# uci-rendering/psdr-cuda

Measured on AMD Instinct MI355X. Metric: Mpath-samples/s renderC+renderD, cbox 512x512 spp=64; grad rel-L2 vs ref, higher is better.
Workload: dtype f32; 1 GPU; cbox 512x512 spp=64/GPU PathTracer(max_depth=3): renderC + configure + renderD + enoki.forward w.r.t. diffuse albedo, through the psdr_cuda surface; triangles=12, global_spp=64, world_size=1, device=AMD Radeon Graphics, local_rank=0

## Files before the change

### __graft_entry__.py

```python
import os
import subprocess
import sys

ROOT = os.path.dirname(os.path.abspath(__file__))
PKG = os.path.join(ROOT, "psdr-cuda_amd")
for p in (PKG, os.path.join(ROOT, "oracle"), os.path.join(ROOT, "tests")):
    if p not in sys.path:
        sys.path.insert(0, p)

HIPCC_FLAGS = ["--offload-arch=gfx950", "-O3", "-std=c++17", "-fPIC", "-munsafe-fp-atomics",
               "-fno-hip-fp32-correctly-rounded-divide-sqrt", "-fgpu-flush-denormals-to-zero", "-fno-slp-vectorize",
               "-freciprocal-math", "-fapprox-func"]
VARIANTS = (0, 1, 2, 3, 4, 6, 8, 10)


def _stale(target, sources):
    return (not os.path.exists(target)) or any(os.path.getmtime(s) > os.path.getmtime(target) for s in sources)


TESTS = os.path.join(ROOT, "tests")
CSRC = os.path.join(PKG, "csrc")
HC_DIR = os.path.join(TESTS, "hostcheck")
HOST_FLAGS = ["-O2", "-std=c++17", "-pthread"]


def _product_and_harness():
    return ([os.path.join(CSRC, f) for f in sorted(os.listdir(CSRC))] + [os.path.join(ROOT, "include", "psdr_hip.h")] +
            [os.path.join(HC_DIR, f) for f in sorted(os.listdir(HC_DIR)) if f.endswith(".h")])


TEST_LIBS = {
    "hostcheck": ("hostcheck/hostcheck.cpp", "hostcheck/libhostcheck.so", _product_and_harness, HOST_FLAGS),
    "path_sedge": ("hostcheck/hostcheck_path_sedge.cpp", "hostcheck/libhostcheck_path_sedge.so", _product_and_harness, HOST_FLAGS),
    "path_guide": ("hostcheck/hostcheck_path_guide.cpp", "hostcheck/libhostcheck_path_guide.so", _product_and_harness, HOST_FLAGS),
    "collocated": ("hostcheck/hostcheck_collocated.cpp", "hostcheck/libhostcheck_collocated.so", _product_and_harness, HOST_FLAGS),
    "pointlight": ("hostcheck/hostcheck_pointlight.cpp", "hostcheck/libhostcheck_pointlight.so", _product_and_harness, HOST_FLAGS),
    "lightstage": ("hostcheck/hostcheck_lightstage.cpp", "hostcheck/libhostcheck_lightstage.so", _product_and_harness, HOST_FLAGS),
    "distantlight": ("hostcheck/hostcheck_distantlight.cpp", "hostcheck/libhostcheck_distantlight.so", _product_and_harness, HOST_FLAGS),
    "plan": ("hostcheck/hostcheck_plan.cpp", "hostcheck/libhostcheck_plan.so", _product_and_harness, HOST_FLAGS),
    "smooth": ("hostcheck/hostcheck_smooth.cpp", "hostcheck/libhostcheck_smooth.so", lambda: [os.path.join(CSRC, "psdr_smooth.h")], HOST_FLAGS),
    "poison": ("poison/poison.hip", "poison/libpoison.so", lambda: [], ["-O1"]),
}


def testlib_deps(name):
    return [os.path.join(TESTS, TEST_LIBS[name][0])] + TEST_LIBS[name][2]()


def build_testlib(name):
    so = os.path.join(TESTS, TEST_LIBS[name][1])
    if _stale(so, testlib_deps(name)):
        subprocess.check_call(["hipcc", "--offload-arch=gfx950", "-fPIC", "-shared"] + TEST_LIBS[name][3] + [os.path.join(TESTS, TEST_LIBS[name][0]), "-o", so])
    return so


def build():
    csrc = os.path.join(PKG, "csrc")
    srcs = [os.path.join(csrc, f) for f in os.listdir(csrc)] + [os.path.join(ROOT, "include", "psdr_hip.h")]
    lib = os.path.join(PKG, "lib", "libpsdr_hip.so")
    os.makedirs(os.path.dirname(lib), exist_ok=True)
    defect_job = None
    if _stale(lib, srcs):
        obj_dir = os.path.join(PKG, "lib", "obj")
        os.makedirs(obj_dir, exist_ok=True)
        jobs, objs, unit_cmds = [], [], {}
        for v in VARIANTS:
            o = os.path.join(obj_dir, "variant%d.o" % v)
            objs.append(o)
            unit_cmds[o] = ["hipcc"] + HIPCC_FLAGS + ["-DPSDR_VARIANT_FLAGS=%d" % v, "-c", os.path.join(csrc, "psdr_variant.hip"), "-o", o]
            jobs.append(subprocess.Popen(unit_cmds[o]))
            o = os.path.join(obj_dir, "path_sedge%d.o" % v)
            objs.append(o)
            unit_cmds[o] = ["hipcc"] + HIPCC_FLAGS + ["-DPSDR_VARIANT_FLAGS=%d" % v, "-c", os.path.join(csrc, "psdr_path_sedge.hip"), "-o", o]
            jobs.append(subprocess.Popen(unit_cmds[o]))
            o = os.path.join(obj_dir, "collocated%d.o" % v)
            objs.append(o)
            unit_cmds[o] = ["hipcc"] + HIPCC_FLAGS + ["-DPSDR_VARIANT_FLAGS=%d" % v, "-c", os.path.join(csrc, "psdr_collocated.hip"), "-o", o]
            jobs.append(subprocess.Popen(unit_cmds[o]))
            o = os.path.join(obj_dir, "pointlight%d.o" % v)
            objs.append(o)
            unit_cmds[o] = ["hipcc"] + HIPCC_FLAGS + ["-DPSDR_VARIANT_FLAGS=%d" % v, "-c", os.path.join(csrc, "psdr_pointlight.hip"), "-o", o]
            jobs.append(subprocess.Popen(unit_cmds[o]))
            o = os.path.join(obj_dir, "lightstage%d.o" % v)
            objs.append(o)
            unit_cmds[o] = ["hipcc"] + HIPCC_FLAGS + ["-DPSDR_VARIANT_FLAGS=%d" % v, "-c", os.path.join(csrc, "psdr_lightstage.hip"), "-o", o]
            jobs.append(subprocess.Popen(unit_cmds[o]))
        o = os.path.join(obj_dir, "logd_lean.o")
        objs.append(o)
        unit_cmds[o] = ["hipcc"] + HIPCC_FLAGS + ["-c", os.path.join(csrc, "psdr_logd_lean.hip"), "-o", o]
        jobs.append(subprocess.Popen(unit_cmds[o]))
        o = os.path.join(obj_dir, "host.o")
        objs.append(o)
        unit_cmds[o] = ["hipcc"] + HIPCC_FLAGS + ["-c", os.path.join(csrc, "psdr_hip.hip"), "-o", o]
        jobs.append(subprocess.Popen(unit_cmds[o]))
        o = os.path.join(obj_dir, "tables.o")
        objs.append(o)
        unit_cmds[o] = ["hipcc"] + HIPCC_FLAGS + ["-c", os.path.join(csrc, "psdr_tables.hip"), "-o", o]
        jobs.append(subprocess.Popen(unit_cmds[o]))
        o = os.path.join(obj_dir, "smooth.o")
        objs.append(o)
        unit_cmds[o] = ["hipcc"] + HIPCC_FLAGS + ["-c", os.path.join(csrc, "psdr_smooth.hip"), "-o", o]
        jobs.append(subprocess.Popen(unit_cmds[o]))
        defect_job = _start_defect_object(csrc, obj_dir)
        if any(j.wait() != 0 for j in jobs):
            raise RuntimeError("hipcc failed")
        sys.path.insert(0, os.path.join(ROOT, "tools"))
        import check_spill_exec
        fallbacks = (["-mllvm", "-amdgpu-opt-exec-mask-pre-ra=0"], ["-mllvm", "-amdgpu-spill-sgpr-to-vgpr=0"])
        from concurrent.futures import ThreadPoolExecutor
        with ThreadPoolExecutor(max_workers=8) as pool:
            first = dict(zip(unit_cmds, pool.map(lambda o_: check_spill_exec.check_library(o_, verbose=True, min_code_objects=1), list(unit_cmds))))
        for o, cmd in list(unit_cmds.items()):
            hits = first[o]
            for extra in fallbacks:
                if not hits:
                    break
                print("build(): %s trips the spill guard -- rebuilding it with %s" % (os.path.basename(o), " ".join(extra)))
                subprocess.check_call(cmd[:1] + cmd[1:-4] + extra + cmd[-4:])
                hits = check_spill_exec.check_library(o, verbose=True, min_code_objects=1)
            if hits:
                raise RuntimeError("%s: %d kernel(s) spill in front of an exec restore with every fallback (tools/check_spill_exec.py)" % (os.path.basename(o), len(hits)))
        subprocess.check_call(["hipcc", "--offload-arch=gfx950", "-shared", "-fPIC"] + objs + ["-o", lib])
        if len(check_spill_exec.code_objects(lib)) < len(objs):
            raise RuntimeError("the linked library holds fewer gfx code objects than translation units: the spill guard cannot see all of it")
    subprocess.check_call(["make", "-C", os.path.join(ROOT, "oracle"), "-s"])
    for name in TEST_LIBS:
        build_testlib(name)
    try:
        build_defect_lib(defect_job)
    except Exception as e:
        print("build(): tests/poison/libpsdr_hip_defect.so not built (%s) -- only tests/test_rough_rev_order_gpu.py uses it" % e)
    import psdr_cuda
    from psdr_cuda import _abi
    _abi.load_hip()
    import oracle
    oracle.load_oracle()


def _defect_object_cmd(csrc, obj_dir):
    return ["hipcc"] + HIPCC_FLAGS + ["-DPSDR_VARIANT_FLAGS=10", "-DPSDR_SINK_REG_PRIV_ROUGH=1", "-DPSDR_DPP_ALWAYS=1", "-c",
                                      os.path.join(csrc, "psdr_variant.hip"), "-o", os.path.join(obj_dir, "variant10_defect.o")]


def _start_defect_object(csrc, obj_dir):
    try:
        return subprocess.Popen(_defect_object_cmd(csrc, obj_dir), stdout=subprocess.DEVNULL, stderr=subprocess.DEVNULL)
    except Exception:
        return None


def build_defect_lib(object_job=None):
    csrc = os.path.join(PKG, "csrc")
    srcs = [os.path.join(csrc, f) for f in os.listdir(csrc)] + [os.path.join(ROOT, "include", "psdr_hip.h")]
    obj_dir = os.path.join(PKG, "lib", "obj")
    defect_lib = os.path.join(ROOT, "tests", "poison", "libpsdr_hip_defect.so")
    objs = [os.path.join(obj_dir, "%s%d.o" % (unit, v)) for v in VARIANTS for unit in ("variant", "path_sedge", "collocated", "pointlight", "lightstage")] + [os.path.join(obj_dir, "logd_lean.o"), os.path.join(obj_dir, "host.o"), os.path.join(obj_dir, "tables.o"), os.path.join(obj_dir, "smooth.o")]
    if not all(os.path.exists(o) for o in objs):
        return None
    if object_job is not None and object_job.wait() != 0:
        object_job = None
    if _stale(defect_lib, srcs + objs):
        defect_obj = os.path.join(obj_dir, "variant10_defect.o")
        if object_job is None:
            subprocess.check_call(_defect_object_cmd(csrc, obj_dir))
        subprocess.check_call(["hipcc", "--offload-arch=gfx950", "-shared", "-fPIC"] + [defect_obj if o.endswith("variant10.o") else o for o in objs] + ["-o", defect_lib])
    return defect_lib


def smoke():
    import numpy as np
    import torch
    assert torch.cuda.is_available(), "smoke() needs a GPU"
    torch.cuda.set_device(0)
    import oracle
    from helpers import GpuScene, load_scene, rel_l2, tangents_wrt
    from psdr_cuda import _abi
    sc, P = load_scene("cbox", res=32, spp=8, sppe=4, sppse=4, translate=(0, (1.0, 0.0, 0.0)))
    tb = sc.tables(0)
    g = GpuScene(tb)
    o = _abi.make_opts(integrator=_abi.INTEGRATOR_PATH, max_depth=3, spp=8)
    img = g.render_c(o)
    ref = oracle.render(tb, o)
    assert np.isfinite(img).all() and rel_l2(img, ref) < 1e-4, rel_l2(img, ref)
    o = _abi.make_opts(spp=8, sppe=4, sppse=4)
    tan = tangents_wrt(tb, P)
    img, dimg = g.render_d_fwd(o, [tan])
    rimg, rd = oracle.render(tb, o, mode=1, tangents=tan)
    assert rel_l2(img, rimg) < 1e-4 and rel_l2(dimg[0], rd) < 1e-3, (rel_l2(img, rimg), rel_l2(dimg[0], rd))
    import psdr_cuda
    from psdr_cuda.fixtures import scene_path
    s2 = psdr_cuda.Scene()
    s2.load_file(scene_path("cbox"), False)
# ... 15 lines not shown
```

### include/psdr_hip.h

```cpp
#ifndef PSDR_HIP_H
#define PSDR_HIP_H

#include <stdint.h>

#ifdef __cplusplus
extern "C" {
#endif

#define PSDR_TRI_STRIDE   24
#define PSDR_TRIUV_STRIDE  8
#define PSDR_SEDGE_STRIDE 16
#define PSDR_PEDGE_STRIDE  8
#define PSDR_BSDF_STRIDE  16
#define PSDR_EMITTER_F_STRIDE 8
#define PSDR_EMITTER_I_STRIDE 4
#define PSDR_CAM_WORDS    64
#define PSDR_ENV_WORDS    32

#define PSDR_TRI_FACE_NORMALS 0x40000000

#define PSDR_BSDF_DIFFUSE        0
#define PSDR_BSDF_ROUGHCONDUCTOR 1
#define PSDR_BSDF_MICROFACET     2
#define PSDR_BSDF_MICROFACET_NORMAL 3
// ... 70 lines not shown
    const int32_t *sec_edge_faces;
    const float   *prim_edge_z;
} psdr_scene_desc;

#define PSDR_FLAG_FUSED     1
#define PSDR_FLAG_WAVEFRONT 2
#define PSDR_FLAG_LITERAL_FORMS 4
#define PSDR_FLAG_KEEP_RECORDS 8
#define PSDR_FLAG_PATH_SEDGES 16
#define PSDR_PATH_SEDGES_MAX_DEPTH 8

typedef struct psdr_render_opts {
    int32_t integrator;
    int32_t bsdf_samples, light_samples;
    int32_t max_depth;
    int32_t hide_emitters;
    int32_t field;
    int32_t spp, sppe, sppse;
    int32_t spp_begin, spp_end;
    int32_t sppe_begin, sppe_end;
    int32_t sppse_begin, sppse_end;
    int32_t flags;
    uint64_t rng_offset[3];
} psdr_render_opts;

typedef struct psdr_tangents {
    const float *d_tri_info;
    const float *d_texels;
    const float *d_emitter_rad;
    const float *d_cam_to_world;
    const float *d_sec_edge;
    const float *d_prim_edge;
    const float *d_env_f;
} psdr_tangents;

typedef struct psdr_grads {
    float *g_tri_info;
    float *g_texels;
    float *g_emitter_rad;
    float *g_cam_to_world;
    float *g_sec_edge;
    float *g_prim_edge;
    float *g_env_f;
} psdr_grads;

typedef struct psdr_scene_s *psdr_scene_t;

const char *psdr_last_error(void);
const char *psdr_version(void);
int psdr_abi_struct_sizes(int32_t out[4]);

int psdr_scene_create(psdr_scene_t *out);
int psdr_scene_destroy(psdr_scene_t h);
int psdr_scene_set_option(psdr_scene_t h, const char *name, double value);

int psdr_scene_set_tables(psdr_scene_t h, const psdr_scene_desc *desc);

int psdr_bvh_build(psdr_scene_t h, void *stream);
int psdr_bvh_stats(psdr_scene_t h, int32_t out[4]);
int psdr_scene_info(psdr_scene_t h, int32_t out[8]);

int psdr_trace(psdr_scene_t h, int32_t m,
               const float *ox, const float *oy, const float *oz,
               const float *dx, const float *dy, const float *dz,
               const float *tmax,
               int32_t *out_shape, int32_t *out_tri, float *out_u, float *out_v,
               void *stream);

int psdr_render_c(psdr_scene_t h, const psdr_render_opts *opts,
                  float *out_img, void *stream);

int psdr_render_d_fwd(psdr_scene_t h, const psdr_render_opts *opts,
                      int32_t K, const psdr_tangents *tangents,
                      float *out_img, float *out_dimg, void *stream);

int psdr_render_d_rev(psdr_scene_t h, const psdr_render_opts *opts,
                      const float *adj_img, float *out_img,
                      const psdr_grads *grads, void *stream);

int psdr_guide_build(psdr_scene_t h, const psdr_render_opts *opts,
                     const int32_t reso[4], int32_t nrounds,
                     float *out_mass, void *stream);

int psdr_scene_set_path_guide(psdr_scene_t h, const int32_t reso[3], const float *cmf, const float *pmf, float sum);
int psdr_scene_set_point_light(psdr_scene_t h, const float pos[3], int32_t K, const float *d_pos, float *g_pos);
int psdr_scene_set_point_lights(psdr_scene_t h, int32_t L, const float *pos, int32_t K, const float *d_pos, float *g_pos);
int psdr_scene_set_light(psdr_scene_t h, int32_t kind, const float v[3], int32_t K, const float *d_v, float *g_v);
int psdr_scene_set_lights(psdr_scene_t h, int32_t L, const int32_t *kinds, const float *v, int32_t K, const float *d_v, float *g_v);
int psdr_path_guide_build(psdr_scene_t h, const psdr_render_opts *opts, int32_t segment,
                          const int32_t reso[4], int32_t nrounds,
                          float *out_mass, void *stream);

int psdr_cube_sample_reuse(int32_t ndim, const int32_t *reso, const float *cmf, const float *pmf, float sum,
                           int32_t n, int32_t m, float *samples, float *out_pdf, void *stream);
int psdr_sample_boundary_segment_direct(const psdr_scene_desc *desc, int32_t m, const float *sample3,
                                        const uint8_t *active, float *out_p0, float *out_edge_dir,
                                        float *out_edge2, float *out_p2, float *out_n, float *out_pdf,
                                        uint8_t *out_valid, int32_t *out_edge, float *out_s1, void *stream);

int psdr_geo_world_vertices_fwd(int32_t V, const float *v_raw, const int32_t *vmesh, const float *mats, float *v_world, void *stream);
int psdr_geo_world_vertices_rev(int32_t V, const float *v_raw, const int32_t *vmesh, const float *mats, const float *v_world, const float *a_world, float *a_raw,
                                void *stream);
int psdr_geo_world_vertices_jvp(int32_t V, const float *v_raw, const int32_t *vmesh, const float *mats, const float *v_world, const float *t_raw, const float *t_mats,
                                float *t_world, void *stream);
int psdr_geo_tri_rows_fwd(int32_t V, int32_t T, const float *v, const int32_t *faces, float *vsum, float *rows, int32_t row_stride, void *stream);
int psdr_geo_tri_rows_rev(int32_t V, int32_t T, const float *v, const int32_t *faces, const float *vsum, const float *a_rows, int32_t row_stride,
                          float *a_vsum , float *a_v, void *stream);
int psdr_geo_tri_rows_jvp(int32_t V, int32_t T, const float *v, const int32_t *faces, const float *vsum, const float *t_v, int32_t row_stride,
                          float *t_vsum , float *t_rows, void *stream);
int psdr_geo_sec_edges_fwd(int32_t E, const int32_t *edges, const float *v, const float *rows, int32_t row_stride, float *info, uint8_t *keep, void *stream);
int psdr_geo_sec_edges_rev(int32_t E, const int32_t *edges, const float *a_info, float *a_v, float *a_rows, int32_t row_stride, void *stream);
int psdr_geo_sec_edges_jvp(int32_t E, const int32_t *edges, const float *t_v, const float *t_rows, int32_t row_stride, float *t_info, void *stream);
int psdr_geo_prim_edges_fwd(int32_t E, const int32_t *edges, const uint8_t *face_normals, const float *v, const float *rows, int32_t row_stride,
                            const float *cam22, float *rows8, float *z4, uint8_t *keep, void *stream);
int psdr_geo_prim_edges_rev(int32_t E, const int32_t *edges, const float *v, const float *cam22, const float *a_rows8, float *a_v, float *a_w2s ,
                            void *stream);
int psdr_geo_prim_edges_jvp(int32_t E, const int32_t *edges, const float *v, const float *cam22, const float *t_v, const float *t_w2s , float *t_rows8,
                            void *stream);

int psdr_geo_compact_edges_fwd(int32_t E, const float *rows, int32_t S, const uint8_t *keep, int32_t w0, int32_t wn, const void *aux, int32_t aux_stride, int32_t A,
                               void *scratch, float *rows_out, void *aux_out, int32_t *pos, float *pmf, float *cmf, float *header, void *stream);
int psdr_geo_compact_edges_rev(int32_t E, int32_t S, const int32_t *pos, const float *a_rows_out, float *a_rows, void *stream);
int psdr_geo_compact_edges_jvp(int32_t E, int32_t S, const int32_t *pos, const float *t_rows, float *t_rows_out, void *stream);
int psdr_geo_emitter_tables(int32_t M, const float *rows, int32_t row_stride, const int32_t *face_offset, const int32_t *mesh_emitter, int32_t Ne, const int32_t *emitter_i,
                            const float *radiance, const float *env_weight, float *mesh_area, float *emitter_f, float *emitter_pmf, float *emitter_cmf, float *face_pmf,
                            float *face_cmf, void *stream);

typedef struct psdr_smooth_s *psdr_smooth_t;
typedef struct psdr_smooth_info_s {
    int32_t iterations;
    int32_t converged;
    int32_t form;
    int32_t launches;
    float rel_residual[3];
    int32_t one_workgroup_limit;
    int32_t one_workgroup_default;
    int32_t num_vertices;
    int32_t num_entries;
    int32_t long_rows;
} psdr_smooth_info_t;
int psdr_smooth_create(int32_t V, int32_t F, const int32_t *faces, psdr_smooth_t *out);
void psdr_smooth_destroy(psdr_smooth_t h);
int psdr_smooth_set_option(psdr_smooth_t h, const char *name, int value);
int psdr_smooth_apply(psdr_smooth_t h, float lambda, const float *x, float *u, void *stream);
int psdr_smooth_solve(psdr_smooth_t h, float lambda, const float *b, const float *x0, float *x, float tol, int32_t max_iter, void *stream);
int psdr_smooth_info(psdr_smooth_t h, psdr_smooth_info_t *out);

int psdr_scene_rev_layout(psdr_scene_t h, int32_t out[16]);

int psdr_scene_seed_info(psdr_scene_t h, int64_t out[4]);

int psdr_scene_logd_info(psdr_scene_t h, int64_t out[4]);

int psdr_get_counters(psdr_scene_t h, uint64_t out[4]);

#ifdef __cplusplus
}
#endif
#endif
```

### psdr-cuda_amd/csrc/psdr_hip.hip

```cpp
#define PSDR_WIDE_TREE 2
#include "psdr_host.h"
#include "psdr_bvh_build.h"

#include <cstdlib>
#include <cstring>
#include <rocprim/rocprim.hpp>

namespace {
__global__ __launch_bounds__(kBlock) void k_trace(LaunchCtx cx, int m, const float *__restrict__ ox, const float *__restrict__ oy,
                                                  const float *__restrict__ oz, const float *__restrict__ dx,
                                                  const float *__restrict__ dy, const float *__restrict__ dz,
                                                  const float *__restrict__ tmax, int32_t *__restrict__ out_shape,
                                                  int32_t *__restrict__ out_tri, float *__restrict__ out_u, float *__restrict__ out_v) {
    TraversalStack st; setup_lds(cx, st);
    const SceneView &sc = cx.sc;
    for (int i = blockIdx.x * kBlock + threadIdx.x; i < m; i += gridDim.x * kBlock) {
        const Hit h = closest_hit<false, -1>(sc, st, Vec3f{ox[i], oy[i], oz[i]}, Vec3f{dx[i], dy[i], dz[i]}, tmax[i]);
        out_tri[i] = h.tri;
        out_shape[i] = h.tri >= 0 ? (sc.d.tri_mesh[h.tri] & ~PSDR_TRI_FACE_NORMALS) : -1;
        out_u[i] = h.u; out_v[i] = h.v;
    }
}


// ... 548 lines not shown
    if (int rc = device_grow(h->d_lbvh, h->lbvh_bytes, need, 1)) return rc;
    const LbvhScratch L = lbvh_layout(h->d_lbvh, T, sort_tmp);
    if (int rc = grow_tree(h, (size_t) T, (size_t) T * 3)) return rc;
    const dim3 gT((T + kBlock - 1) / kBlock), blk(kBlock);
    HIP_TRY(hipMemsetAsync(L.info, 0, sizeof(LbvhInfo), s));
    HIP_TRY(hipMemsetAsync(L.bounds, 0xff, 3 * 4, s));
    HIP_TRY(hipMemsetAsync(L.bounds + 3, 0, 3 * 4, s));
    hipLaunchKernelGGL(k_lbvh_bounds, gT, blk, 0, s, h->desc.tri_info, T, L.bounds, L.info);
    hipLaunchKernelGGL(k_lbvh_codes, gT, blk, 0, s, h->desc.tri_info, T, L.bounds, L.keys, L.vals, L.info);
    HIP_TRY(hipGetLastError());
    size_t tmp_bytes = L.sort_tmp_bytes;
    HIP_TRY(rocprim::radix_sort_pairs(L.sort_tmp, tmp_bytes, L.keys, L.keys2, L.vals, L.vals2, (size_t) T, 0, 30, s));
    HIP_TRY(hipMemsetAsync(L.leaf_parent, 0xff, (size_t) T * 4, s));
    hipLaunchKernelGGL(k_lbvh_tris, gT, blk, 0, s, h->desc.tri_info, T, L.vals2, h->d_btris);
    hipLaunchKernelGGL(k_lbvh_hierarchy, gT, blk, 0, s, L.keys2, T, h->d_nodes, L.node_parent, L.leaf_parent);
    HIP_TRY(hipGetLastError());
    LbvhInfo info{};
    HIP_TRY(hipMemcpyAsync(&info, L.info, sizeof(info), hipMemcpyDeviceToHost, s));
    HIP_TRY(hipStreamSynchronize(s));
    if (info.bad) return fail("psdr_bvh_build: non-finite vertex");
    if (int rc = lbvh_fit(h, L, info.pad, s)) return rc;
    hipLaunchKernelGGL(k_lbvh_depth, gT, blk, 0, s, T, L.node_parent, L.leaf_parent, L.info);
    hipLaunchKernelGGL(k_lbvh_area_keys, gT, blk, 0, s, h->desc.tri_info, T, L.keys, L.vals);
    HIP_TRY(hipGetLastError());
    tmp_bytes = L.sort_tmp_bytes;
    HIP_TRY(rocprim::radix_sort_pairs_desc(L.sort_tmp, tmp_bytes, L.keys, L.keys2, L.vals, L.vals2, (size_t) T, 0, 32, s));
    float area = 0.f;
    const int top = std::min(T, kMaxHotRows);
    std::vector<int32_t> by_area((size_t) top);
    HIP_TRY(hipMemcpyAsync(&info, L.info, sizeof(info), hipMemcpyDeviceToHost, s));
    HIP_TRY(hipMemcpyAsync(&area, h->d_refit_area, sizeof(float), hipMemcpyDeviceToHost, s));
    HIP_TRY(hipMemcpyAsync(by_area.data(), L.vals2, (size_t) top * 4, hipMemcpyDeviceToHost, s));
    if (int rc = fetch_emitters(h, s)) return rc;
    HIP_TRY(hipStreamSynchronize(s));
    if (info.depth > kBvhStack - 2) { fallback = true; return 0; }
    if (int rc = upload_hot_rows(h, T, hot_row_list(T, false, h->emitter_i, h->desc.num_emitters, by_area.data(), top), s)) return rc;
    h->hot_identity = false;
    h->root = 0; h->bvh_depth = info.depth; h->num_nodes = T - 1; h->num_btris = T;
    reset_top(h);
    if (use_wide_tree(h, false)) {
        std::vector<BvhNode> host_nodes((size_t) T - 1);
        HIP_TRY(hipMemcpyAsync(host_nodes.data(), h->d_nodes, host_nodes.size() * sizeof(BvhNode), hipMemcpyDeviceToHost, s));
        HIP_TRY(hipStreamSynchronize(s));
        if (int rc = bvh4_build(h, host_nodes, std::vector<int32_t>{0}, false, s)) return rc;
    } else { h->wide = false; h->num_nodes4 = 0; h->stack_need4 = 0; }
    h->level_start.clear();
    finish_build(h, T, info.pad, area, true, true);
    return 0;
}

int bvh4_refill(psdr_scene_s *h, hipStream_t s) {
    if (h->num_nodes4 <= 0) return 0;
    hipLaunchKernelGGL(k_bvh4_fill, dim3((h->num_nodes4 + kBlock - 1) / kBlock), dim3(kBlock), 0, s, h->d_nodes4, h->d_nodes, h->d_topo4,
                       h->d_topo4 + (size_t) h->num_nodes4 * 4, h->num_nodes4);
    HIP_TRY(hipGetLastError());
    return 0;
}
int bvh4_build(psdr_scene_s *h, const std::vector<BvhNode> &nodes, const std::vector<int32_t> &roots2, bool forest, hipStream_t s) {
    h->wide = use_wide_tree(h, forest);
    if (!h->wide && !forest) { h->num_nodes4 = 0; h->stack_need4 = 0; return 0; }
    Bvh4Topology tp;
    collapse_bvh4(nodes, roots2, tp);
    h->num_nodes4 = tp.n4; h->stack_need4 = tp.stack_need;
    h->root4 = roots2.size() == 1 ? tp.roots[0] : 0;
    for (size_t k = 0; k < roots2.size() && k < (size_t) kMaxBlas; ++k) h->blas_root4[k] = tp.roots[k];
    if (tp.n4 == 0) return 0;
    if (int rc = device_grow(h->d_nodes4, h->cap_nodes4, (size_t) tp.n4, sizeof(Bvh4Node), &h->d_topo4, 8 * sizeof(int32_t))) return rc;
    HIP_TRY(hipMemcpyAsync(h->d_topo4, tp.child.data(), (size_t) tp.n4 * 4 * sizeof(int32_t), hipMemcpyHostToDevice, s));
    HIP_TRY(hipMemcpyAsync(h->d_topo4 + (size_t) tp.n4 * 4, tp.src.data(), (size_t) tp.n4 * 4 * sizeof(int32_t), hipMemcpyHostToDevice, s));
    if (int rc = bvh4_refill(h, s)) return rc;
    HIP_TRY(hipStreamSynchronize(s));
    return 0;
}

int launch_wf_trace(psdr_scene_s *h, const float4 *req, const int32_t *count, long long sub_cap, float4 *hit, hipStream_t s, bool ign) {
    TraceArgs a{};
    a.sec_edge_faces = h->desc.sec_edge_faces;
    if (ign && !a.sec_edge_faces) ign = false;
    pack_blas_boxes(h, a.blas_lo, a.blas_hi);
    a.nodes4 = h->d_nodes4; a.btris = h->d_btris; a.req = req; a.count = count; a.hit = hit; a.sub_cap = sub_cap; a.n_blas = h->n_blas;
    const TracePlan p = plan_wf_trace(h, sub_cap);
    a.n_lnodes = p.n_lnodes; a.off_stack = p.off_stack; a.stack_entries = p.stack_entries; a.ovf_stride = p.ovf_stride;
    if (p.ovf) {
        if (int rc = scratch_reserve(reinterpret_cast<void **>(&h->d_trace_ovf), &h->trace_ovf_bytes, p.ovf_bytes, s, "trace kernel's overflow stack columns")) return rc;
        a.ovf = h->d_trace_ovf;
    }
    const bool wg2 = p.wg2, ovf = p.ovf;
    const int grid = p.grid, dyn = p.dyn;
#define PSDR_LAUNCH_TRACE_I(MULTI, OVF, IGN, WPE)                                                                                                           \
    do { static bool attr_set = false;                                                                                                                      \
         if (!attr_set) { if (int rc = allow_dynamic_lds(&k_wf_trace<MULTI, OVF, IGN, WPE>, 160 * 1024 - 1024)) return rc; attr_set = true; }                     \
         hipLaunchKernelGGL(HIP_KERNEL_NAME(k_wf_trace<MULTI, OVF, IGN, WPE>), dim3(grid), dim3(kTraceBlock), dyn, s, a); } while (0)
#define PSDR_LAUNCH_TRACE(MULTI, OVF) do { if (ign) { if (wg2) PSDR_LAUNCH_TRACE_I(MULTI, OVF, true, 8); else PSDR_LAUNCH_TRACE_I(MULTI, OVF, true, 4); } else if (wg2) PSDR_LAUNCH_TRACE_I(MULTI, OVF, false, 8); else PSDR_LAUNCH_TRACE_I(MULTI, OVF, false, 4); } while (0)
    if (h->n_blas > 1) { if (ovf) PSDR_LAUNCH_TRACE(true, true); else PSDR_LAUNCH_TRACE(true, false); }
    else { if (ovf) PSDR_LAUNCH_TRACE(false, true); else PSDR_LAUNCH_TRACE(false, false); }
#undef PSDR_LAUNCH_TRACE_I
#undef PSDR_LAUNCH_TRACE
    HIP_TRY(hipGetLastError());
    return 0;
}

int probe_buffers(psdr_scene_s *h, long long slots, int rays_per_slot, ProbeBuffers &pb, hipStream_t s, int per_cu) {
    const ProbePlan pl = plan_probe_buffers(h, slots, rays_per_slot, per_cu);
    pb.sub_cap = pl.sub_cap;
    if (int rc = scratch_reserve(&h->d_probe, &h->probe_bytes, pl.total, s, "probe buffers (hit rows, masks, trace requests)")) return rc;
    char *p = reinterpret_cast<char *>(h->d_probe);
    pb.count = reinterpret_cast<int32_t *>(p); p += pl.cnt_bytes;
    pb.hit = reinterpret_cast<float4 *>(p); p += pl.hit_bytes;
    pb.mask = reinterpret_cast<uint32_t *>(p); p += pl.mask_bytes;
    pb.req = reinterpret_cast<float4 *>(p);
    HIP_TRY(hipMemsetAsync(pb.count, 0, pl.cnt_bytes, s));
    return 0;
}

#define PSDR_OPS_OF(OPS)                                                                                                              \
    switch (scene_flag_set(h)) {                                                                                                      \
        case 0: return OPS##0(); case 1: return OPS##1(); case 2: return OPS##2(); case 3: return OPS##3();                          \
        case 4: return OPS##4(); case 8: return OPS##8(); case 10: return OPS##10();                                                 \
        default: return OPS##6();                       \
    }
const VariantOps *variant_of(const psdr_scene_s *h) { PSDR_OPS_OF(variant_ops_) }
const PathSedgeOps *path_sedge_of(const psdr_scene_s *h) { PSDR_OPS_OF(path_sedge_ops_) }
const CollocatedOps *collocated_of(const psdr_scene_s *h) { PSDR_OPS_OF(collocated_ops_) }
const PointLightOps *point_light_of(const psdr_scene_s *h) { PSDR_OPS_OF(point_light_ops_) }
const LightStageOps *light_stage_of(const psdr_scene_s *h) { PSDR_OPS_OF(light_stage_ops_) }
const char *const kDistantInEnv = "a distant light cannot reach a scene inside an environment map's bounding mesh (env_emitter >= 0)";
int check_point_light(const psdr_scene_s *h, const psdr_render_opts *o) {
    if (o->integrator == PSDR_INTEGRATOR_POINT && !h->have_point) return fail("PointLightIntegrator: no light set (psdr_scene_set_point_light)");
    if (o->integrator == PSDR_INTEGRATOR_POINT_STACK && h->stack_pos.empty()) return fail("LightStageIntegrator: no lights set (psdr_scene_set_point_lights)");
    if (h->desc.env_emitter >= 0) {
        const bool distant = o->integrator == PSDR_INTEGRATOR_POINT ? h->point_kind == PSDR_LIGHT_DISTANT
                           : o->integrator == PSDR_INTEGRATOR_POINT_STACK && std::find(h->stack_kind.begin(), h->stack_kind.end(), PSDR_LIGHT_DISTANT) != h->stack_kind.end();
        if (distant) return fail(kDistantInEnv);
    }
    return 0;
}
#undef PSDR_OPS_OF
}
using namespace psdr_host;

extern "C" {

const char *psdr_last_error(void) { return g_err.c_str(); }
const char *psdr_version(void) { return "psdr-hip 0.1 gfx950"; }
int psdr_abi_struct_sizes(int32_t out[4]) {
    out[0] = (int32_t) sizeof(psdr_scene_desc); out[1] = (int32_t) sizeof(psdr_render_opts);
    out[2] = (int32_t) sizeof(psdr_tangents); out[3] = (int32_t) sizeof(psdr_grads);
    return 0;
}

int psdr_scene_create(psdr_scene_t *out) {
    if (!out) return fail("psdr_scene_create: null output");
    psdr_scene_s *h = new psdr_scene_s();
    hipError_t e = hipMalloc(&h->d_counters, sizeof(unsigned long long) * kRayCounters * kRayCounterStride);
    if (e != hipSuccess) { delete h; return fail(std::string("hipMalloc: ") + hipGetErrorString(e)); }
    int dev = 0; hipDeviceProp_t prop;
    if (hipGetDevice(&dev) == hipSuccess && hipGetDeviceProperties(&prop, dev) == hipSuccess) {
        h->num_cus = prop.multiProcessorCount;
        h->lds_limit = (int) std::min<size_t>(prop.sharedMemPerBlock, 160 * 1024);
    }
    *out = h;
    return 0;
}

int psdr_scene_set_option(psdr_scene_t h, const char *name, double value) {
    if (!h || !name) return fail("psdr_scene_set_option: null argument");
    const std::string n(name);
    const int iv = (int) value;
    if (n == "bvh_refit") h->refit_enabled = iv != 0;
    else if (n == "forest_min_inline") { h->forest_min_inline = iv; h->have_bvh = false; }
    else if (n == "scratch_plain") g_scratch_plain = iv;
    else if (n == "own_pixels") h->opt.own_pixels = iv;
    else if (n == "emitter_pretest") h->opt.emitter_pretest = iv;
    else if (n == "occ_rows") { h->opt.occ_rows = iv; h->have_bvh = false; }
    else if (n == "aa_prims") { h->aa_enabled = iv != 0; h->have_bvh = false; }
    else if (n == "tiny_scene") h->tiny_enabled = iv != 0;
    else if (n == "two_level") h->two_level_enabled = iv != 0;
    else if (n == "wf_binned") h->wf_binned = iv != 0;
    else if (n == "wf_traced") h->traced_enabled = iv != 0;
    else if (n == "bvh_build") h->bvh_device_mode = iv;
    else if (n == "sort_edges") h->sort_edges = iv != 0;
    else if (n == "blocks_per_cu") h->opt.blocks_per_cu = iv;
    else if (n == "camera_blocks") h->opt.camera_blocks = iv;
    else if (n == "tiny_variants") h->opt.tiny_variants = iv;
    else if (n == "wide") h->opt.wide = iv;
    else if (n == "lds_budget") h->opt.lds_budget = iv;
    else if (n == "sink_rep") h->opt.sink_rep = std::max(1, std::min(16, iv));
    else if (n == "sink_private") h->opt.sink_private = iv;
    else if (n == "rev_split") h->opt.rev_split = iv;
    else if (n == "tangent_live") h->opt.tangent_live = iv;
    else if (n == "wf_geo") h->opt.wf_geo = iv;
    else if (n == "logd") h->opt.logd = iv;
    else if (n == "seed_cache") h->opt.seed_cache = iv;
    else if (n == "logd_park") h->opt.logd_park = iv;
    else if (n == "seed_cache_log2") h->opt.seed_cache_log2 = std::max(0, std::min(40, iv));
    else if (n == "keep_records") h->opt.keep_records = iv;
    else if (n == "rev_sorted") h->opt.rev_sorted = iv;
    else if (n == "sedge_split") h->opt.sedge_split = iv;
    else if (n == "pt_sedge") h->opt.pt_sedge = iv & 3;
    else if (n == "pt_sedge_walk") h->opt.pt_sedge_walk = iv;
    else if (n == "probe") h->opt.probe = iv;
    else if (n == "trace_wg2") h->opt.trace_wg2 = iv;
    else if (n == "chunk_log2") h->opt.chunk_log2 = std::max(0, std::min(30, iv));
    else if (n == "bvh_maxleaf") h->opt.bvh_maxleaf = std::max(1, std::min(8, iv));
    else if (n == "bvh_tcost") h->opt.bvh_tcost = (float) value;
    else return fail("psdr_scene_set_option: unknown option '" + n + "'");
    h->kept.valid = false;
    if (n == "tiny_scene" || n == "two_level" || n == "bvh_build" || n == "wide" || n == "bvh_maxleaf" || n == "bvh_tcost" || n == "tiny_variants") h->have_bvh = false;
    return 0;
}

int psdr_scene_destroy(psdr_scene_t h) {
    if (!h) return 0;
    if (h->d_nodes) (void) hipFree(h->d_nodes);
    if (h->d_stack_lights) (void) hipFree(h->d_stack_lights);
    if (h->d_btris) (void) hipFree(h->d_btris);
    if (h->d_counters) (void) hipFree(h->d_counters);
    if (h->d_refit_area) (void) hipFree(h->d_refit_area);
    if (h->d_sort) (void) hipFree(h->d_sort);
    if (h->d_ws) (void) hipFree(h->d_ws);
    if (h->d_live) (void) hipFree(h->d_live);
    if (h->d_logd_bad) (void) hipFree(h->d_logd_bad);
    if (h->d_seed) (void) hipFree(h->d_seed);
    if (h->seed_event) (void) hipEventDestroy(h->seed_event);
    if (h->d_hot_map) (void) hipFree(h->d_hot_map);
    if (h->d_hot_tris) (void) hipFree(h->d_hot_tris);
    if (h->d_occ) (void) hipFree(h->d_occ);
    if (h->d_top) (void) hipFree(h->d_top);
    if (h->d_inline_ids) (void) hipFree(h->d_inline_ids);
    if (h->d_lbvh) (void) hipFree(h->d_lbvh);
    if (h->d_nodes4) (void) hipFree(h->d_nodes4);
    if (h->d_topo4) (void) hipFree(h->d_topo4);
    if (h->d_rev) (void) hipFree(h->d_rev);
    if (h->d_se_list) (void) hipFree(h->d_se_list);
    if (h->d_rev_deep) (void) hipFree(h->d_rev_deep);
    if (h->d_pe_rep) (void) hipFree(h->d_pe_rep);
    if (h->d_trace_ovf) (void) hipFree(h->d_trace_ovf);
    if (h->d_probe) (void) hipFree(h->d_probe);
    delete h;
    return 0;
}

int psdr_scene_set_tables(psdr_scene_t h, const psdr_scene_desc *desc) {
    if (!h || !desc) return fail("psdr_scene_set_tables: null argument");
    psdr_scene_desc d = *desc;
    if (d.num_tris <= 0 || !d.tri_info || !d.tri_mesh) return fail("Missing meshes!");
    if (!d.cam) return fail("Missing sensor!");
    if (reinterpret_cast<uintptr_t>(d.tri_info) & 15) return fail("psdr_scene_set_tables: tri_info must be 16-byte aligned");
    if (d.width <= 0 || d.height <= 0) return fail("Invalid film resolution");
    if (d.num_meshes <= 0 || !d.mesh_bsdf || !d.mesh_emitter) return fail("psdr_scene_set_tables: mesh_bsdf / mesh_emitter missing");
    if (d.num_bsdfs > 0 && (!d.bsdf_rec || !d.texels)) return fail("psdr_scene_set_tables: bsdf_rec / texels missing");
    if (d.num_emitters > 0 && (!d.emitter_f || !d.emitter_i)) return fail("psdr_scene_set_tables: emitter tables missing");
    if (d.num_emitters > 1 && (!d.emitter_cmf || !d.emitter_pmf)) return fail("psdr_scene_set_tables: emitter distribution missing");
    if (d.num_sec_edges > 0 && (!d.sec_edge || !d.sec_cmf || !d.sec_pmf)) return fail("psdr_scene_set_tables: secondary-edge tables missing");
    if (d.num_prim_edges > 0 && (!d.prim_edge || !d.prim_cmf || !d.prim_pmf)) return fail("psdr_scene_set_tables: primary-edge tables missing");
    if (d.num_prim_edges <= 0) d.prim_edge_z = nullptr;
    if (d.num_guide_cells > 0 && (!d.guide_cmf || !d.guide_pmf)) return fail("psdr_scene_set_tables: guiding tables missing");
    if (!d.env_f) d.env_emitter = -1;
    if (d.env_emitter >= 0) {
        if (d.env_emitter >= d.num_emitters || !d.env_cmf || !d.env_pmf || d.env_reso[0] <= 0 || d.env_reso[1] <= 0 || d.env_tex[1] < 2 ||
            d.env_tex[2] < 2)
            return fail("psdr_scene_set_tables: inconsistent environment-map record");
    }
    if (h->have_tables && (d.tri_info != h->desc.tri_info || d.num_tris != h->desc.num_tris)) h->have_bvh = false;
    if (h->have_tables && (d.emitter_i != h->desc.emitter_i || d.num_emitters != h->desc.num_emitters)) h->have_bvh = false;
    if (!h->have_tables || std::memcmp(&h->desc, &d, sizeof(d)) != 0) { ++h->tables_gen; h->kept.valid = false; }
    h->desc = d;
    h->has_microfacet = (d.material_mask & ((1u << PSDR_BSDF_MICROFACET) | (1u << PSDR_BSDF_MICROFACET_NORMAL) | (1u << PSDR_BSDF_MICROFACET_HEIGHT))) != 0;
    h->has_rough = d.material_mask == 0 || (d.material_mask & (1u << PSDR_BSDF_ROUGHCONDUCTOR)) != 0 || h->has_microfacet;
    h->have_tables = true;
    h->pg_cmf = h->pg_pmf = nullptr; h->pg_sum = 0.f;
    return 0;
}

int psdr_scene_set_path_guide(psdr_scene_t h, const int32_t reso[3], const float *cmf, const float *pmf, float sum) {
    if (!h) return fail("psdr_scene_set_path_guide: null argument");
    if (!cmf) { h->pg_cmf = h->pg_pmf = nullptr; h->pg_sum = 0.f; return 0; }
    if (!reso || !pmf) return fail("psdr_scene_set_path_guide: null argument");
    if (reso[0] <= 0 || reso[1] <= 0 || reso[2] <= 0 || (long long) reso[0] * reso[1] * reso[2] > 0x7fffffffLL) return fail("psdr_scene_set_path_guide: invalid resolution");
    for (int i = 0; i < 3; ++i) h->pg_reso[i] = reso[i];
    h->pg_cmf = cmf; h->pg_pmf = pmf; h->pg_sum = sum;
    return 0;
}

static hipError_t copy_on_stream(void *dst, const void *src, size_t bytes, hipMemcpyKind kind, hipStream_t s) {
    if (hipError_t e = hipMemcpyAsync(dst, src, bytes, kind, s)) return e;
    return hipStreamSynchronize(s);
}
static void update_emit_rows(psdr_scene_s *h) {
    h->emit_rows = 0;
    if (h->n_tiny > 0 && emit_rows_wanted(h))
        h->emit_rows = tiny_emitter_rows(h->tiny_meta, h->n_tiny, h->aa_cnt, emitter_triangle_mask(h->emitter_i, h->desc.num_emitters, h->desc.num_tris));
}

static void refit_done(psdr_scene_s *h) { h->refits_since_build++; h->num_refits++; h->have_bvh = true; }
static int emitters_unchanged(psdr_scene_s *h, hipStream_t s, bool &same) {
    same = (size_t) std::max(h->desc.num_emitters, 0) * PSDR_EMITTER_I_STRIDE == h->emitter_i.size();
    if (!same || h->emitter_i.empty()) return 0;
    same = h->desc.emitter_i != nullptr;
    if (!same) return 0;
    std::vector<int32_t> now(h->emitter_i.size());
    HIP_TRY(copy_on_stream(now.data(), h->desc.emitter_i, now.size() * sizeof(int32_t), hipMemcpyDeviceToHost, s));
    same = std::memcmp(now.data(), h->emitter_i.data(), now.size() * sizeof(int32_t)) == 0;
    return 0;
}
static int host_tree_refit(psdr_scene_s *h, hipStream_t s, bool &fits) {
    fits = true;
    HIP_TRY(hipMemsetAsync(h->d_refit_area, 0, sizeof(float), s));
    hipLaunchKernelGGL(k_refit_leaves, dim3((h->num_btris + kBlock - 1) / kBlock), dim3(kBlock), 0, s, h->d_btris, h->desc.tri_info, h->num_btris);
    for (int l = (int) h->level_start.size() - 2; l >= 0; --l) {
        const int first = h->level_start[l], count = h->level_start[l + 1] - first;
        hipLaunchKernelGGL(k_refit_level, dim3((count + kBlock - 1) / kBlock), dim3(kBlock), 0, s, h->d_nodes, h->d_btris, first, count, h->bvh_pad, h->d_refit_area);
    }
    HIP_TRY(hipGetLastError());
    if (int rc = bvh4_refill(h, s)) return rc;
    if (h->n_blas == 0) return 0;
    float4 top[kMaxInlineTris * 3 + 2 * kMaxBlas];
    hipLaunchKernelGGL(k_gather_top, dim3(1), dim3(64), 0, s, h->d_top, h->d_nodes, h->desc.tri_info, h->d_inline_ids, h->n_inline, h->n_blas);
    HIP_TRY(hipMemcpyAsync(top, h->d_top, sizeof(top), hipMemcpyDeviceToHost, s));
    HIP_TRY(hipStreamSynchronize(s));
    std::vector<float4> tris(top, top + 3 * (size_t) h->n_inline), prims;
    pack_tiny_prims(tris, prims);
    fits = refit_inline_fits((int) prims.size() / 3);
    if (!fits) return 0;
    h->n_tiny = tiny_plane_form(prims, h->tiny, h->tiny_meta, &h->aa_cnt, h->aa_enabled);
    update_emit_rows(h);
    for (int k = 0; k < h->n_blas; ++k) {
        const float w = h->blas_lo[k].w;
        h->blas_lo[k] = top[kMaxInlineTris * 3 + k]; h->blas_lo[k].w = w;
        h->blas_hi[k] = top[kMaxInlineTris * 3 + kMaxBlas + k];
    }
    return 0;
}
static int try_refit(psdr_scene_s *h, int T, bool tiny, hipStream_t s, bool &done) {
    done = false;
    if (!refit_candidate(h, T, tiny)) return 0;
    bool emitters_same = false;
    if (int rc = emitters_unchanged(h, s, emitters_same)) return rc;
    const bool stands = forest_stands(h);
    if (refit_choice(h, emitters_same, stands, h->built_area) == kRefitNone) return 0;
    float prev_area = h->built_area;
    if (h->refits_since_build > 0) {
        HIP_TRY(hipMemcpyAsync(&prev_area, h->d_refit_area, sizeof(float), hipMemcpyDeviceToHost, h->refit_stream));
        HIP_TRY(hipStreamSynchronize(h->refit_stream));
    }
    const RefitKind kind = refit_choice(h, emitters_same, stands, prev_area);
// ... 229 lines not shown
    if (pos == nullptr || L == 0) return 0;
    if (int rc = device_grow(h->d_stack_lights, h->cap_stack_lights, (size_t) L, sizeof(float) * 13)) return rc;
    h->stack_pos.assign(pos, pos + 3 * (size_t) L);
    h->stack_kind.assign((size_t) L, PSDR_LIGHT_POINT);
    if (d_pos != nullptr && K > 0) { h->stack_K = K; h->stack_dpos.assign(d_pos, d_pos + 3 * (size_t) L * K); }
    h->stack_gpos = g_pos;
    return 0;
}

static int check_light_vector(const char *fn, int kind, const float *v, const std::string &which) {
    if (kind != PSDR_LIGHT_POINT && kind != PSDR_LIGHT_DISTANT) return fail(std::string(fn) + ": unknown light kind " + std::to_string(kind) + which + " (PSDR_LIGHT_POINT or PSDR_LIGHT_DISTANT)");
    if (kind != PSDR_LIGHT_DISTANT || v == nullptr) return 0;
    if (!(std::isfinite(v[0]) && std::isfinite(v[1]) && std::isfinite(v[2]))) return fail(std::string(fn) + ": the direction" + which + " is not finite");
    if (v[0] == 0.f && v[1] == 0.f && v[2] == 0.f) return fail(std::string(fn) + ": the direction" + which + " is all zero");
    return 0;
}

int psdr_scene_set_light(psdr_scene_t h, int32_t kind, const float v[3], int32_t K, const float *d_v, float *g_v) {
    if (!h) return fail("psdr_scene_set_light: null handle");
    if (int rc = check_light_vector("psdr_scene_set_light", kind, v, "")) return rc;
    if (int rc = psdr_scene_set_point_light(h, v, K, d_v, g_v)) return rc;
    if (v != nullptr) h->point_kind = kind;
    return 0;
}

int psdr_scene_set_lights(psdr_scene_t h, int32_t L, const int32_t *kinds, const float *v, int32_t K, const float *d_v, float *g_v) {
    if (!h) return fail("psdr_scene_set_lights: null handle");
    const bool some = v != nullptr && L != 0;
    if (some && kinds == nullptr) return fail("psdr_scene_set_lights: null kinds");
    if (some && L >= 1 && L <= PSDR_POINT_LIGHTS_MAX)
        for (int l = 0; l < L; ++l)
            if (int rc = check_light_vector("psdr_scene_set_lights", kinds[l], v + 3 * l, " of light " + std::to_string(l))) return rc;
    if (int rc = psdr_scene_set_point_lights(h, L, v, K, d_v, g_v)) return rc;
    if (some) h->stack_kind.assign(kinds, kinds + L);
    return 0;
}

int psdr_guide_build(psdr_scene_t h, const psdr_render_opts *o, const int32_t reso[4], int32_t nrounds, float *out_mass, void *stream) {
    if (!h || !o || !reso || !out_mass) return fail("psdr_guide_build: null argument");
    if (int rc = check_microfacet(h, o)) return rc;
    if (nrounds <= 0) return fail("psdr_guide_build: nrounds must be positive");
    if (h->desc.num_sec_edges <= 0) return fail("psdr_guide_build: scene has no secondary edges");
    hipStream_t s = (hipStream_t) stream;
    if (int rc = begin_call(h, s)) return rc;
    LaunchCtx cx;
    if (int rc = make_ctx(h, o, 2, cx)) return rc;
    cx.sc.d.guide_cmf = nullptr; cx.sc.d.num_guide_cells = 0;
    const long long cells = (long long) reso[0] * reso[1] * reso[2];
    const long long n = cells * reso[3];
    if (n <= 0 || n > 0x7fffffffLL) return fail("psdr_guide_build: invalid resolution");
    HIP_TRY(hipMemsetAsync(out_mass, 0, sizeof(float) * cells, s));
    return variant_of(h)->guide(h, cx, reso, nrounds, n, out_mass, s);
}

int psdr_path_guide_build(psdr_scene_t h, const psdr_render_opts *o, int32_t segment, const int32_t reso[4], int32_t nrounds, float *out_mass, void *stream) {
    if (!h || !o || !reso || !out_mass) return fail("psdr_path_guide_build: null argument");
    if (int rc = check_microfacet(h, o)) return rc;
    if (nrounds <= 0) return fail("psdr_path_guide_build: nrounds must be positive");
    if (o->integrator != PSDR_INTEGRATOR_PATH) return fail("psdr_path_guide_build: the integrator must be PSDR_INTEGRATOR_PATH");
    if (o->max_depth < 1) return fail("psdr_path_guide_build: max_depth must be at least 1");
    if (o->max_depth > PSDR_PATH_SEDGES_MAX_DEPTH) return fail("psdr_path_guide_build: PathTracer max_depth > 8 is not supported for the secondary-edge term");
    if (segment != 1 && segment != 2) return fail("psdr_path_guide_build: segment must be 1 (direct source) or 2 (indirect source)");
    if (segment == 2 && o->max_depth < 2) return fail("psdr_path_guide_build: segment 2 needs max_depth >= 2");
    if (!h->have_tables) return fail("Scene not loaded yet!");
    if (h->desc.num_sec_edges <= 0) return fail("psdr_path_guide_build: scene has no secondary edges");
    if (reso[0] <= 0 || reso[1] <= 0 || reso[2] <= 0 || reso[3] <= 0) return fail("psdr_path_guide_build: invalid resolution");
    const long long cells = (long long) reso[0] * reso[1] * reso[2];
    if (cells > 0x7fffffffLL || cells * reso[3] > 0x7fffffffLL || cells * reso[3] * (long long) nrounds > 0x7fffffffLL)
        return fail("psdr_path_guide_build: more than 2^31 (stream, round) slots");
    hipStream_t s = (hipStream_t) stream;
    if (int rc = begin_call(h, s)) return rc;
    HIP_TRY(hipMemsetAsync(out_mass, 0, sizeof(float) * cells, s));
    return path_sedge_of(h)->guide(h, o, segment, reso, nrounds, out_mass, s);
}

int psdr_cube_sample_reuse(int32_t ndim, const int32_t *reso, const float *cmf, const float *pmf, float sum, int32_t n, int32_t m, float *samples,
                           float *out_pdf, void *stream) {
    if (!reso || !cmf || !pmf || !samples || !out_pdf) return fail("psdr_cube_sample_reuse: null argument");
    if (ndim != 2 && ndim != 3) return fail("psdr_cube_sample_reuse: ndim must be 2 or 3");
    long long cells = 1;
    for (int d = 0; d < ndim; ++d) {
        if (reso[d] <= 0) return fail("psdr_cube_sample_reuse: invalid resolution");
        cells *= reso[d];
    }
    if (cells != (long long) n) return fail("psdr_cube_sample_reuse: n must be the product of the resolution");
    if (m < 0) return fail("psdr_cube_sample_reuse: negative sample count");
    if (m == 0) return 0;
    const dim3 grid((unsigned) ((m + kBlock - 1) / kBlock));
    hipStream_t s = (hipStream_t) stream;
    if (ndim == 2)
        hipLaunchKernelGGL(k_cube_sample_reuse<2>, grid, dim3(kBlock), 0, s, m, cmf, pmf, sum, n, reso[0], reso[1], 1, samples, out_pdf);
    else
        hipLaunchKernelGGL(k_cube_sample_reuse<3>, grid, dim3(kBlock), 0, s, m, cmf, pmf, sum, n, reso[0], reso[1], reso[2], samples, out_pdf);
    HIP_TRY(hipGetLastError());
    return 0;
}

int psdr_sample_boundary_segment_direct(const psdr_scene_desc *desc, int32_t m, const float *sample3, const uint8_t *active, float *out_p0,
                                        float *out_edge_dir, float *out_edge2, float *out_p2, float *out_n, float *out_pdf, uint8_t *out_valid,
                                        int32_t *out_edge, float *out_s1, void *stream) {
    if (!desc || !sample3 || !out_p0 || !out_edge_dir || !out_edge2 || !out_p2 || !out_n || !out_pdf || !out_valid || !out_edge || !out_s1)
        return fail("psdr_sample_boundary_segment_direct: null argument");
    const psdr_scene_desc &d = *desc;
    if (d.num_sec_edges <= 0 || !d.sec_edge || !d.sec_cmf || !d.sec_pmf) return fail("Scene has no secondary edges");
    if (d.num_emitters <= 0 || !d.emitter_f || !d.emitter_i) return fail("No Emitter!");
    if (d.num_emitters > 1 && (!d.emitter_cmf || !d.emitter_pmf)) return fail("psdr_sample_boundary_segment_direct: emitter distribution missing");
    const bool env = d.env_f != nullptr && d.env_emitter >= 0;
    if (env && (d.env_emitter >= d.num_emitters || !d.env_cmf || !d.env_pmf || d.env_reso[0] <= 0 || d.env_reso[1] <= 0))
        return fail("psdr_sample_boundary_segment_direct: inconsistent environment-map record");
    if (d.num_emitters > (env ? 1 : 0) && (d.num_tris <= 0 || !d.tri_info || !d.face_cmf || !d.face_pmf))
        return fail("psdr_sample_boundary_segment_direct: area-light tables missing");
    if (m < 0) return fail("psdr_sample_boundary_segment_direct: negative sample count");
    if (m == 0) return 0;
    SceneView sc{};
    sc.d = d;
    if (!env) sc.d.env_emitter = -1;
    const dim3 grid((unsigned) ((m + kBlock - 1) / kBlock));
    hipStream_t s = (hipStream_t) stream;
    if (env)
        hipLaunchKernelGGL(k_boundary_segment_direct<kSceneEnv>, grid, dim3(kBlock), 0, s, sc, m, sample3, active, out_p0, out_edge_dir, out_edge2, out_p2, out_n,
                           out_pdf, out_valid, out_edge, out_s1);
    else
        hipLaunchKernelGGL(k_boundary_segment_direct<0>, grid, dim3(kBlock), 0, s, sc, m, sample3, active, out_p0, out_edge_dir, out_edge2, out_p2, out_n,
                           out_pdf, out_valid, out_edge, out_s1);
    HIP_TRY(hipGetLastError());
    return 0;
}

int psdr_bvh_stats(psdr_scene_t h, int32_t out[4]) {
    if (!h || !out) return fail("psdr_bvh_stats: null argument");
    out[0] = h->num_builds; out[1] = h->num_refits; out[2] = h->num_nodes; out[3] = h->bvh_depth;
    return 0;
}

int psdr_scene_info(psdr_scene_t h, int32_t out[8]) {
    if (!h || !out) return fail("psdr_scene_info: null argument");
    const int n_slab = (h->aa_cnt & 255) + ((h->aa_cnt >> 8) & 255) + (h->aa_cnt >> 16);
    out[0] = h->n_tiny - (h->aa_cnt != 0 ? kAaSlots - n_slab : 0); out[1] = h->n_blas; out[2] = h->n_inline; out[3] = h->num_btris; out[4] = h->lbvh ? 1 : 0;
    out[5] = n_slab; out[6] = h->have_occ ? 1 : 0; out[7] = h->have_occ ? h->occ_max_rows : 0;
    return 0;
}

int psdr_scene_rev_layout(psdr_scene_t h, int32_t out[16]) {
    if (!h || !out) return fail("psdr_scene_rev_layout: null argument");
    std::copy(std::begin(h->rev_layout), std::end(h->rev_layout), out);
    return 0;
}

int psdr_scene_logd_info(psdr_scene_t h, int64_t out[4]) {
    if (!h || !out) return fail("psdr_scene_logd_info: null argument");
    out[0] = h->logd_launches; out[1] = h->logd_lean_launches; out[2] = h->logd_lean_seeded; out[3] = (int64_t) h->logd_lean_lds + h->logd_lean_park;
    return 0;
}
int psdr_scene_seed_info(psdr_scene_t h, int64_t out[4]) {
    if (!h || !out) return fail("psdr_scene_seed_info: null argument");
    out[0] = h->seed_valid ? h->seed_key[0] * h->seed_key[3] : 0; out[1] = (int64_t) (h->seed_cap * sizeof(ulonglong2)); out[2] = h->seed_fills; out[3] = h->seed_launches;
    return 0;
}

int psdr_get_counters(psdr_scene_t h, uint64_t out[4]) {
    if (!h || !out) return fail("psdr_get_counters: null argument");
    unsigned long long all[kRayCounters * kRayCounterStride], c[1] = {0};
    HIP_TRY(hipMemcpyAsync(all, h->d_counters, sizeof(all), hipMemcpyDeviceToHost, h->last_stream));
    HIP_TRY(hipStreamSynchronize(h->last_stream));
    for (int i = 0; i < kRayCounters; ++i) c[0] += all[i * kRayCounterStride];
#ifdef PSDR_STAGE_CLOCKS
    {
        unsigned long long ph[12] = {0};
        for (int i = 0; i < kRayCounters; ++i) for (int k = 0; k < 12; ++k) ph[k] += all[i * kRayCounterStride + 1 + k];
        std::fprintf(stderr, "stage clocks:");
        for (int k = 0; k < 12; ++k) std::fprintf(stderr, " %llu", ph[k]);
        std::fprintf(stderr, "\n");
    }
#endif
    out[0] = c[0]; out[1] = h->slots[0]; out[2] = h->slots[1]; out[3] = h->slots[2];
    return 0;
}

}
```

### psdr-cuda_amd/csrc/psdr_host.h

```cpp
#pragma once
#include "psdr_device.h"
#include "psdr_reverse.h"

#include <algorithm>
#include <type_traits>
#include <cmath>
#include <cstdio>
#include <cstdlib>
#include <cstring>
#include <string>
#include <vector>

using namespace psdr;

struct LaunchCtx {
    SceneView sc;
    LiParams lp;
    RngJump jump;
    int32_t off_stack;
    int32_t off_pathrec;
    int32_t off_sink;
    int32_t off_park;
};

static_assert(offsetof(LaunchCtx, sc) == 0, "closest_hit reads SceneView::tiny through the kernel-argument segment pointer: LaunchCtx (SceneView first) must be the first kernel argument");

__device__ __forceinline__ void setup_lds(const LaunchCtx &cx, TraversalStack &st) {
#if defined(__HIP_DEVICE_COMPILE__)
    const SceneView &sc = cx.sc;
    float4 *dst = reinterpret_cast<float4 *>(psdr_dyn_lds);
    const float4 *src = sc.nodes4 != nullptr ? reinterpret_cast<const float4 *>(sc.nodes4) : reinterpret_cast<const float4 *>(sc.nodes);
    for (int i = threadIdx.x; i < sc.n_lnodes * 4; i += kBlock) dst[sc.off_lnodes / 16 + (i >> 2) * (kLdsNodeStride / 16) + (i & 3)] = src[i];
    for (int i = threadIdx.x; i < sc.n_lbtris * 3; i += kBlock) dst[sc.off_lbtris / 16 + i] = sc.btris[i];
    src = reinterpret_cast<const float4 *>(sc.d.tri_info);
    for (int i = threadIdx.x; i < sc.n_ltri * 6; i += kBlock) dst[sc.off_ltri / 16 + i] = src[i];
    {
        float *m = reinterpret_cast<float *>(psdr_dyn_lds + sc.off_lprim);
#pragma unroll 1
        for (int i = 0; i < sc.n_tiny; ++i) {
            int32_t tri; float k[6];
            const int w = threadIdx.x & 7;
            const float4 Sm = sc.tiny[i * 4 + 2];
            const float S[4] = {Sm.x, Sm.y, Sm.z, Sm.w};
            tiny_hit_row(sc.tiny_meta + i * 4, (threadIdx.x >> 3) & 1, tri, k, (sc.aa_cnt != 0 && i < kAaSlots) ? S : nullptr);
            const float val = w == 0 ? __int_as_float(tri) : (w == 1 ? k[0] : w == 2 ? k[1] : w == 3 ? k[2] : w == 4 ? k[3] : w == 5 ? k[4] : w == 6 ? k[5] : 0.f);
            if (threadIdx.x < kTinyHitWords) m[i * kTinyHitWords + threadIdx.x] = val;
        }
    }
    if (sc.lt_meshbsdf >= 0) {
        auto stage = [&](int off, const void *table, int words) {
            if (off < 0 || table == nullptr) return;
            const uint32_t *g = static_cast<const uint32_t *>(table);
            uint32_t *l = reinterpret_cast<uint32_t *>(psdr_dyn_lds + off);
#pragma unroll 1
            for (int i = threadIdx.x; i < words; i += kBlock) l[i] = g[i];
        };
        stage(sc.lt_trimesh, sc.d.tri_mesh, sc.d.num_tris);
        stage(sc.lt_meshbsdf, sc.d.mesh_bsdf, sc.d.num_meshes);
        stage(sc.lt_meshemitter, sc.d.mesh_emitter, sc.d.num_meshes);
        stage(sc.lt_bsdf, sc.d.bsdf_rec, sc.d.num_bsdfs * PSDR_BSDF_STRIDE);
        stage(sc.lt_emf, sc.d.emitter_f, sc.d.num_emitters * PSDR_EMITTER_F_STRIDE);
        stage(sc.lt_emi, sc.d.emitter_i, sc.d.num_emitters * PSDR_EMITTER_I_STRIDE);
        stage(sc.lt_ecmf, sc.d.emitter_cmf, sc.d.num_emitters);
        stage(sc.lt_epmf, sc.d.emitter_pmf, sc.d.num_emitters);
        stage(sc.lt_fcmf, sc.d.face_cmf, sc.lt_nfaces);
        stage(sc.lt_fpmf, sc.d.face_pmf, sc.lt_nfaces);
        stage(sc.lt_uv, sc.d.tri_uv, sc.d.num_tris * PSDR_TRIUV_STRIDE);
        stage(sc.lt_tex, sc.d.texels, sc.d.num_texels);
        stage(sc.lt_occ, sc.occ, sc.d.num_tris * sc.d.num_tris);
    }
    st.base = reinterpret_cast<int32_t *>(psdr_dyn_lds + cx.off_stack) + threadIdx.x;
    __syncthreads();
#else
    (void) cx; (void) st;
#endif
}
template <class TVT> __device__ __forceinline__ void setup_lds(const LaunchCtx &cx, TraversalStack &st, const TVT &tv) {
    setup_lds(cx, st);
#if defined(__HIP_DEVICE_COMPILE__)
    if constexpr (Tab<TVT::flags>::lds_small && TVT::k > 0) {
        constexpr int K = TVT::k;
        static_assert(K <= 3, "plan_lds reserves three tangent texel pools");
        if (cx.sc.lt_tex >= 0) {
            float *l = reinterpret_cast<float *>(psdr_dyn_lds + cx.sc.lt_tex);
            const int nt = cx.sc.d.num_texels;
            for (int k = 0; k < K; ++k) {
                const float *g = tv.t[k].d_texels;
                for (int i = threadIdx.x; i < nt; i += kBlock) l[(k + 1) * nt + i] = g ? g[i] : 0.f;
            }
            __syncthreads();
        }
    }
#endif
}

constexpr int kSinkCacheWords = 6144;
struct SinkLayout {
    int tex_off, tex_n;
    int rad_off, rad_n;
    int cam_off;
    int env_off, env_n;
    int hot_off, hot_rows;
    const int32_t *hot_map, *hot_tris;
    int total;
    int rep, stride;
    int priv_off, priv_rows;
    int priv_tri[2], priv_slot[2], priv_emitter;
    int priv_regs;
    int pend_off, pend_rows;
};
constexpr int kPendWords = 10;
constexpr int kPrivRowWords = 13;
constexpr int kPrivWords = 2 * kPrivRowWords + 3;

struct psdr_scene_options {
    int blocks_per_cu = 0;
    int camera_blocks = 0;
    int tiny_variants = 1;
    int wide = -1;
    int lds_budget = 0;
    int sink_rep = 4;
    int sink_private = 1;
    int rev_split = -1;
    int tangent_live = 1;
    int wf_geo = 1;
    int own_pixels = 1;
    int emitter_pretest = 1;
    int occ_rows = 1;
    int logd = 1;
    int keep_records = 1;
    int rev_sorted = 1;
    int pt_sedge = 3;
    int pt_sedge_walk = 1;
    int sedge_split = -1;
    int chunk_log2 = 0;
    int probe = 1;
    int trace_wg2 = -1;
    int seed_cache = 1;
    int seed_cache_log2 = 25;
    int logd_park = 1;
    int bvh_maxleaf = 4;
    float bvh_tcost = 2.0f;
};

struct psdr_scene_s {
    psdr_scene_options opt;
    psdr_scene_desc desc{};
    bool have_tables = false;
    bool has_rough = true;
    int num_cus = 256;
    int lds_limit = 64 * 1024;

    BvhNode *d_nodes = nullptr;
    float4 *d_btris = nullptr;
    size_t cap_nodes = 0, cap_btris = 0;
    int32_t root = 0;
    bool have_bvh = false;
    int bvh_depth = 0, num_nodes = 0, num_btris = 0;
    Bvh4Node *d_nodes4 = nullptr;
    int32_t *d_topo4 = nullptr;
    size_t cap_nodes4 = 0;
    int num_nodes4 = 0, stack_need4 = 0;
    bool wide = false;
    int32_t *d_trace_ovf = nullptr;
    size_t trace_ovf_bytes = 0;
    bool traced_enabled = true;
    int32_t root4 = 0, blas_root4[kMaxBlas] = {};
    bool refit_enabled = true;
    int tree_tris = -1, refits_since_build = 0, num_builds = 0, num_refits = 0;
    std::vector<int> level_start;
    float bvh_pad = 0.f, built_area = 0.f;
    float *d_refit_area = nullptr;

    int bvh_device_mode = -1;
    bool lbvh = false;
    int lbvh_leaves = 0;
    void *d_lbvh = nullptr;
    size_t lbvh_bytes = 0;

    bool tiny_enabled = true, aa_enabled = true;
    int n_tiny = 0, aa_cnt = 0;
    float4 tiny[kTinyRows * 4] = {};
    int32_t tiny_meta[kTinyRows * 4] = {};
    bool two_level_enabled = true, refit_ok = true, wf_binned = true;
    int n_blas = 0, n_inline = 0;
    float4 blas_lo[kMaxBlas] = {}, blas_hi[kMaxBlas] = {};
    float4 *d_top = nullptr;
    int32_t *d_inline_ids = nullptr;

    unsigned long long *d_counters = nullptr;
    hipStream_t last_stream = nullptr;
    hipStream_t refit_stream = nullptr;
    uint64_t slots[3] = {0, 0, 0};
    int last_path_depth = 0;
    int32_t rev_layout[16] = {};

    std::vector<int32_t> emitter_i;
    int32_t *d_hot_map = nullptr, *d_hot_tris = nullptr;
    uint32_t *d_occ = nullptr; size_t occ_cap = 0; bool have_occ = false; int occ_max_rows = 0;
    int hot_rows = 0;
    bool hot_identity = false;
    size_t hot_cap = 0;

    bool sort_edges = true;
    void *d_sort = nullptr;
    size_t sort_bytes = 0;

    void *d_pe_rep = nullptr;
    size_t pe_rep_bytes = 0;

    void *d_rev_deep = nullptr;
    size_t rev_deep_bytes = 0;

    void *d_se_list = nullptr;
    size_t se_list_bytes = 0;

    void *d_rev = nullptr;
    size_t rev_bytes = 0;
    void *d_logd_bad = nullptr; size_t logd_bad_bytes = 0;
    struct KeptRecords { bool valid = false; psdr_render_opts o{}; uint64_t gen = 0; long long n = 0; int kind = 0; } kept;
    uint64_t tables_gen = 0;

    void *d_seed = nullptr;
    size_t seed_cap = 0;
    long long seed_key[4] = {0, 0, 0, 0};
    bool seed_valid = false;
    hipStream_t seed_stream = nullptr;
    hipEvent_t seed_event = nullptr;
    long long seed_fills = 0, seed_launches = 0;
    long long logd_launches = 0, logd_lean_launches = 0, logd_lean_seeded = 0;
    int logd_lean_lds = 0, logd_lean_park = 0;
    void *d_ws = nullptr;
    size_t ws_bytes = 0;
    void *d_live = nullptr;
    size_t live_bytes = 0;
    void *d_probe = nullptr;
    size_t probe_bytes = 0;
    uint32_t emit_rows = 0;
    int forest_min_inline = 0;
    int32_t pg_reso[3] = {1, 1, 1};
    const float *pg_cmf = nullptr, *pg_pmf = nullptr;
    float pg_sum = 0.f;
    bool has_microfacet = false;
    bool have_point = false;
    float point_pos[3] = {0.f, 0.f, 0.f}, point_dpos[3][3] = {};
    int point_K = 0;
    float *point_gpos = nullptr;
    int point_kind = PSDR_LIGHT_POINT;
    std::vector<float> stack_pos, stack_dpos;
    int stack_K = 0;
    float *stack_gpos = nullptr;
    std::vector<int32_t> stack_kind;
    float *d_stack_lights = nullptr;
    size_t cap_stack_lights = 0;
};

constexpr int kRayCounters = 64, kRayCounterStride = 16;
constexpr int kWfSub = 64, kWfCountStride = 32;
constexpr int kTraceBlock = 1024, kTraceNodeStride = 80, kTraceStackMax = 16;

#define HIP_TRY(expr)                                                                              \
    do { hipError_t e_ = (expr); if (e_ != hipSuccess) return psdr_host::fail(std::string(#expr) + ": " + hipGetErrorString(e_)); } while (0)
namespace psdr_host {
int fail(const std::string &m);
template <class Kernel> int allow_dynamic_lds(Kernel *kernel, int bytes) {
    if (bytes > 48 * 1024) HIP_TRY(hipFuncSetAttribute(reinterpret_cast<const void *>(kernel), hipFuncAttributeMaxDynamicSharedMemorySize, bytes));
    return 0;
}
int scratch_reserve(void **buf, size_t *have, size_t need, hipStream_t s, const char *what);
long long fit_chunk(long long chunk, size_t bytes_per_slot, size_t fixed_bytes, size_t have);
inline int workspace_reserve(psdr_scene_s *h, size_t need, hipStream_t s) { return scratch_reserve(&h->d_ws, &h->ws_bytes, need, s, "wavefront workspace (path-state streams + trace requests)"); }
void fill_top(const psdr_scene_s *h, SceneView &sc);
constexpr int kMaxInlineTris = 2 * kTinyTris;
int make_ctx(psdr_scene_s *h, const psdr_render_opts *o, int sampler, LaunchCtx &cx);
int launch_wf_trace(psdr_scene_s *h, const float4 *req, const int32_t *count, long long sub_cap, float4 *hit, hipStream_t s, bool ign = false);
struct ProbeBuffers { float4 *hit; uint32_t *mask; float4 *req; int32_t *count; long long sub_cap; };
int probe_buffers(psdr_scene_s *h, long long slots, int rays_per_slot, ProbeBuffers &pb, hipStream_t s, int per_cu = 16);
inline int sink_bytes_base(const SinkLayout &L) { return (L.priv_rows > 0 && !L.priv_regs) ? (L.priv_off + kPrivWords * kBlock) * 4 : (L.rep * L.stride * 4 + 15) / 16 * 16; }
inline int sink_bytes(const SinkLayout &L) { return L.pend_rows > 0 ? (L.pend_off + L.pend_rows * kPendWords * kBlock) * 4 : sink_bytes_base(L); }
inline void sink_reserve_pending(SinkLayout &L, int rows) { L.pend_rows = 0; L.pend_off = (sink_bytes_base(L) / 4 + 3) / 4 * 4; L.pend_rows = rows; }
int check_counts(const psdr_scene_s *h, const psdr_render_opts *o);
int check_microfacet(const psdr_scene_s *h, const psdr_render_opts *o);
int begin_call(psdr_scene_s *h, hipStream_t s);
int primary_edge_order(psdr_scene_s *h, const LaunchCtx &cx, long long i0, long long n, const uint32_t **order, hipStream_t s);
constexpr int kMaxRefits = 64;
constexpr float kRefitAreaGrowth = 1.3f;
constexpr int kLbvhAutoTris = 1 << 18;

struct VariantOps {
    int (*render_c)(psdr_scene_s *h, const psdr_render_opts *o, float *img, hipStream_t s);
    int (*render_fwd)(psdr_scene_s *h, const psdr_render_opts *o, int K, const psdr_tangents *tangents, float *img, float *dimg, hipStream_t s);
    int (*render_rev)(psdr_scene_s *h, const psdr_render_opts *o, const float *adj_img, float *out_img, const psdr_grads *grads, hipStream_t s);
    int (*guide)(psdr_scene_s *h, LaunchCtx &cx, const int32_t reso[4], int nrounds, long long n, float *out_mass, hipStream_t s);
};
struct PathSedgeOps {
    int (*fwd)(psdr_scene_s *h, const psdr_render_opts *o, int K, const psdr_tangents *tangents, float *dimg, hipStream_t s);
    int (*rev)(psdr_scene_s *h, const psdr_render_opts *o, const float *adj_img, const psdr_grads *grads, hipStream_t s);
    int (*guide)(psdr_scene_s *h, const psdr_render_opts *o, int segment, const int32_t reso[4], int nrounds, float *out_mass, hipStream_t s);
};
const PathSedgeOps *path_sedge_ops_0();
const PathSedgeOps *path_sedge_ops_1();
const PathSedgeOps *path_sedge_ops_2();
const PathSedgeOps *path_sedge_ops_3();
const PathSedgeOps *path_sedge_ops_4();
const PathSedgeOps *path_sedge_ops_6();
const PathSedgeOps *path_sedge_ops_8();
const PathSedgeOps *path_sedge_ops_10();
struct CollocatedOps {
    int (*render_c)(psdr_scene_s *h, const psdr_render_opts *o, float *img, hipStream_t s);
    int (*render_fwd)(psdr_scene_s *h, const psdr_render_opts *o, int K, const psdr_tangents *tangents, float *img, float *dimg, hipStream_t s);
    int (*render_rev)(psdr_scene_s *h, const psdr_render_opts *o, const float *adj_img, float *out_img, const psdr_grads *grads, hipStream_t s);
};
const CollocatedOps *collocated_ops_0();
const CollocatedOps *collocated_ops_1();
const CollocatedOps *collocated_ops_2();
const CollocatedOps *collocated_ops_3();
const CollocatedOps *collocated_ops_4();
const CollocatedOps *collocated_ops_6();
const CollocatedOps *collocated_ops_8();
const CollocatedOps *collocated_ops_10();
struct PointLightOps {
    int (*render_c)(psdr_scene_s *h, const psdr_render_opts *o, float *img, hipStream_t s);
    int (*render_fwd)(psdr_scene_s *h, const psdr_render_opts *o, int K, const psdr_tangents *tangents, float *img, float *dimg, hipStream_t s);
    int (*render_rev)(psdr_scene_s *h, const psdr_render_opts *o, const float *adj_img, float *out_img, const psdr_grads *grads, hipStream_t s);
    int (*edges_fwd)(psdr_scene_s *h, const psdr_render_opts *o, int K, const psdr_tangents *tangents, int kind, const float *pos, const float *d_pos, float *dimg, long long plane, hipStream_t s);
    int (*edges_rev)(psdr_scene_s *h, const psdr_render_opts *o, const float *adj_img, const psdr_grads *grads, int kind, const float *pos, float *g_pos, hipStream_t s);
};
const PointLightOps *point_light_ops_0();
const PointLightOps *point_light_ops_1();
const PointLightOps *point_light_ops_2();
const PointLightOps *point_light_ops_3();
const PointLightOps *point_light_ops_4();
const PointLightOps *point_light_ops_6();
const PointLightOps *point_light_ops_8();
const PointLightOps *point_light_ops_10();
struct LightStageOps {
    int (*render_c)(psdr_scene_s *h, const psdr_render_opts *o, float *img, hipStream_t s);
    int (*render_fwd)(psdr_scene_s *h, const psdr_render_opts *o, int K, const psdr_tangents *tangents, float *img, float *dimg, const PointLightOps *point, hipStream_t s);
    int (*render_rev)(psdr_scene_s *h, const psdr_render_opts *o, const float *adj_img, float *out_img, const psdr_grads *grads, const PointLightOps *point, hipStream_t s);
};
const LightStageOps *light_stage_ops_0();
const LightStageOps *light_stage_ops_1();
const LightStageOps *light_stage_ops_2();
const LightStageOps *light_stage_ops_3();
const LightStageOps *light_stage_ops_4();
const LightStageOps *light_stage_ops_6();
const LightStageOps *light_stage_ops_8();
const LightStageOps *light_stage_ops_10();
int logd_lean_launch_8(psdr_scene_s *h, const psdr_render_opts *o, const LaunchCtx &cx, const psdr::TangentView<1, psdr::kSceneTiny> &tv, float *img, float *dimg, hipStream_t s, bool *ran);
const VariantOps *variant_ops_0();
const VariantOps *variant_ops_1();
const VariantOps *variant_ops_2();
const VariantOps *variant_ops_3();
const VariantOps *variant_ops_4();
const VariantOps *variant_ops_6();
const VariantOps *variant_ops_8();
const VariantOps *variant_ops_10();
}

#include "psdr_plan.h"
#include "psdr_tree_plan.h"
```

### psdr-cuda_amd/csrc/psdr_kernels.h

```cpp
#pragma once
#include "psdr_host.h"

namespace {
using namespace psdr_host;

__device__ __forceinline__ float wave_shfl_down(float v, int off) { return __shfl_down(v, off, 64); }

template <int CTRL, int ROW_MASK> __device__ __forceinline__ float dpp_add(float v) {
    return v + __int_as_float(__builtin_amdgcn_update_dpp(0, __float_as_int(v), CTRL, ROW_MASK, 0xf, true));
}
__device__ __forceinline__ float wave_total(float v) {
    v = dpp_add<0x111, 0xf>(v); v = dpp_add<0x112, 0xf>(v); v = dpp_add<0x114, 0xf>(v); v = dpp_add<0x118, 0xf>(v);
    v = dpp_add<0x142, 0xa>(v); v = dpp_add<0x143, 0xc>(v);
    return __int_as_float(__builtin_amdgcn_readlane(__float_as_int(v), 63));
}
#ifndef PSDR_DPP_ALWAYS
#define PSDR_DPP_ALWAYS 0
#endif
template <int N, bool DPP = (N <= 6 || PSDR_DPP_ALWAYS)> __device__ __forceinline__ bool wave_segmented_sum(int key, float (&v)[N]) {
    const int lane = threadIdx.x & 63;
    if (DPP && __ballot(key != __builtin_amdgcn_readfirstlane(key)) == 0ull) {
#pragma unroll
        for (int i = 0; i < N; ++i) v[i] = wave_total(v[i]);
        return lane == 0;
    }
#pragma unroll
    for (int off = 1; off < 64; off <<= 1) {
        const int okey = __shfl_down(key, off, 64);
        const bool take = (lane + off < 64) && (okey == key);
#pragma unroll
        for (int i = 0; i < N; ++i) {
            const float o = wave_shfl_down(v[i], off);
            if (take) v[i] += o;
        }
    }
    const int pkey = __shfl_up(key, 1, 64);
    return lane == 0 || pkey != key;
}

template <int N, bool DPP = (N <= 6 || PSDR_DPP_ALWAYS)> __device__ __forceinline__ bool wave_run_sum(int key, float (&v)[N]) {
    const int lane = threadIdx.x & 63;
    const int prev = __shfl_up(key, 1, 64);
    const bool head = lane == 0 || prev != key;
    const unsigned long long heads = __ballot(head);
    const int seg = __popcll(heads & (~0ull >> (63 - lane)));
    wave_segmented_sum<N, DPP>(seg, v);
    return head;
}

__device__ __forceinline__ float *dyn_lds_floats(int byte_offset) {
#if defined(__HIP_DEVICE_COMPILE__)
    return reinterpret_cast<float *>(psdr_dyn_lds + byte_offset);
#else
    (void) byte_offset; return nullptr;
#endif
}
__device__ __forceinline__ void count_rays(unsigned long long *counters, uint32_t nrays) {
    uint32_t s = nrays;
#pragma unroll
    for (int off = 32; off > 0; off >>= 1) s += __shfl_down(s, off, 64);
    if ((threadIdx.x & 63) == 0 && s) atomicAdd(counters + (blockIdx.x % kRayCounters) * kRayCounterStride, (unsigned long long) s);
}

struct ProbeView { const float4 *hit; const uint32_t *mask; };
template <int NR>
__device__ __forceinline__ void probe_load(TraversalStack &st, const ProbeView &pv, long long slot, uint32_t m) {
#pragma unroll
    for (int r = 0; r < NR; ++r) {
        st.pre[r].tri = -1;
        if ((m >> r) & 1u) { const float4 h = pv.hit[slot * NR + r]; st.pre[r] = Hit{__float_as_int(h.x), h.y, h.z, h.w}; }
    }
}

struct SlotDiv {
    uint32_t d, m; int sh;
    SlotDiv() = default;
    SlotDiv(int nsp) : d((uint32_t) nsp) {
        int l = 0;
        while ((1u << l) < d) ++l;
        m = (uint32_t) ((1ull << (31 + l)) / d + 1ull); sh = 31 + l;
    }
};
PSDR_HD void slot_to_pixel(long long j, const SlotDiv &nsp, int &pixel, int &s) {
    const uint32_t ju = (uint32_t) j, q = (uint32_t) (((uint64_t) ju * nsp.m) >> nsp.sh);
    pixel = (int) q; s = (int) (ju - q * nsp.d);
}
#ifndef PSDR_WAVES_C
#define PSDR_WAVES_C 4
#endif
#ifndef PSDR_WAVES_DM
#define PSDR_WAVES_DM 3
#endif
#ifndef PSDR_WAVES_C_NOTREE
#define PSDR_WAVES_C_NOTREE 6
#endif
#ifndef PSDR_WAVES_DG
#define PSDR_WAVES_DG 2
#endif
#ifndef PSDR_LOGD
#define PSDR_LOGD 1
#endif
#ifndef PSDR_LOGD_WAVES_K1
#define PSDR_LOGD_WAVES_K1 6
#endif
template <class G, class R, int INTEG, int FL, bool NOTREE = false> constexpr int camera_waves() {
    constexpr bool lean = (FL & (kSceneEnv | kSceneRough)) == 0;
    if (!is_ad<R>()) return lean ? ((NOTREE && INTEG == PSDR_INTEGRATOR_PATH) ? PSDR_WAVES_C_NOTREE : PSDR_WAVES_C + 1) : PSDR_WAVES_C;
    constexpr bool rough_path_notree = NOTREE && (FL & kSceneRough) != 0 && INTEG == PSDR_INTEGRATOR_PATH;
    if (is_ad<G>()) return ad_traits<G>::K == 1 ? (rough_path_notree ? 2 : 3) : PSDR_WAVES_DG;
    if (rough_path_notree && ad_traits<R>::K == 3) return 2;
    if (lean && NOTREE && INTEG == PSDR_INTEGRATOR_PATH) return ad_traits<R>::K == 1 ? PSDR_WAVES_DM + 2 : PSDR_WAVES_DM + 1;
    return (lean && INTEG == PSDR_INTEGRATOR_PATH && ad_traits<R>::K == 1) ? PSDR_WAVES_DM + 1 : PSDR_WAVES_DM;
}
constexpr int kLogdGateWord = kRayCounterStride - 1;
template <class G, class R, int INTEG, int FL> constexpr bool logd_instance() {
    return PSDR_LOGD && !is_ad<G>() && is_ad<R>() && INTEG == PSDR_INTEGRATOR_PATH && (FL & (kSceneRough | kSceneEnv | kScenePre)) == 0;
}
__global__ __launch_bounds__(kBlock) void k_seed_fill(ulonglong2 *__restrict__ seed, long long n, int spp, int s_begin, SlotDiv nsp) {
    const long long j = (long long) blockIdx.x * kBlock + threadIdx.x;
    if (j >= n) return;
    int pixel, s_in;
    slot_to_pixel(j, nsp, pixel, s_in);
    Rng rng; rng.seed((uint64_t) pixel * (uint64_t) spp + (uint64_t) (s_begin + s_in));
    seed[j] = ulonglong2{rng.state, rng.inc};
}
__device__ __forceinline__ Rng seeded_rng(const ulonglong2 &sd, const RngJump &jump) { Rng rng; rng.init_seeded(sd.x, sd.y, jump); return rng; }
#define PSDR_CAMERA_KERNEL_BODY(SEED_LOAD, SAMPLE) \
    constexpr int K = ad_traits<R>::K; \
    constexpr int NV = 3 * (1 + K); \
    if constexpr (logd_instance<G, R, INTEG, FL>()) { if (counters[kLogdGateWord] == 1ull) return; } \
    TraversalStack st; setup_lds(cx, st, tv); \
    uint32_t nrays = 0; \
    const long long nceil = (n + kBlock - 1) / kBlock * kBlock; \
    for (long long j = (long long) blockIdx.x * kBlock + threadIdx.x; j < nceil; j += (long long) gridDim.x * kBlock) { \
        const bool in = j < n; \
        SEED_LOAD \
        int pixel = 0x7fffffff, s_in = 0; \
        if (in) slot_to_pixel(j0 + j, nsp, pixel, s_in); \
        float v[NV]; \
_Pragma("unroll") \
        for (int i = 0; i < NV; ++i) v[i] = 0.f; \
        if constexpr ((FL & kScenePre) != 0) { if (in) probe_load<3>(st, pv, j, pv.mask[j]); } \
        if (in) { \
            const int s = s_begin + s_in; \
            const uint64_t slot = (uint64_t) pixel * (uint64_t) spp + (uint64_t) s; \
            const Vec3<R> r = SAMPLE; \
            v[0] = val(r.x) * inv_spp; v[1] = val(r.y) * inv_spp; v[2] = val(r.z) * inv_spp; \
_Pragma("unroll") \
            for (int k = 0; k < K; ++k) { \
                v[3 + 3 * k] = tangent(r.x, k) * inv_spp; v[4 + 3 * k] = tangent(r.y, k) * inv_spp; v[5 + 3 * k] = tangent(r.z, k) * inv_spp; \
            } \
        } \
        const bool head = wave_segmented_sum<NV>(pixel, v); \
        if (head && in) { \
            float *p = img + (size_t) pixel * 3; \
            if (own) { \
                p[0] = v[0]; p[1] = v[1]; p[2] = v[2]; \
_Pragma("unroll") \
                for (int k = 0; k < K; ++k) { float *q = dimg + (size_t) k * plane + (size_t) pixel * 3; q[0] = v[3 + 3 * k]; q[1] = v[4 + 3 * k]; q[2] = v[5 + 3 * k]; } \
            } else { \
                if (v[0] != 0.f) atomicAdd(p, v[0]); \
                if (v[1] != 0.f) atomicAdd(p + 1, v[1]); \
                if (v[2] != 0.f) atomicAdd(p + 2, v[2]); \
_Pragma("unroll") \
                for (int k = 0; k < K; ++k) { \
                    float *q = dimg + (size_t) k * plane + (size_t) pixel * 3; \
                    if (v[3 + 3 * k] != 0.f) atomicAdd(q, v[3 + 3 * k]); \
                    if (v[4 + 3 * k] != 0.f) atomicAdd(q + 1, v[4 + 3 * k]); \
                    if (v[5 + 3 * k] != 0.f) atomicAdd(q + 2, v[5 + 3 * k]); \
                } \
            } \
        } \
    } \
    count_rays(counters, nrays);
#define PSDR_SEED_LOAD_NONE
#define PSDR_SEED_LOAD const ulonglong2 sd = in ? seed[j] : ulonglong2{0ull, 0ull};
template <class G, class R, int INTEG, int FL, bool NOTREE = false>
__global__ __launch_bounds__(kBlock, (camera_waves<G, R, INTEG, FL, NOTREE>())) void k_camera(LaunchCtx cx, TV<R, FL> tv, int spp, int s_begin, SlotDiv nsp, long long n, float inv_spp,
                                                   float *__restrict__ img, float *__restrict__ dimg, long long plane,
                                                   unsigned long long *counters, long long j0, ProbeView pv, int own) {
    PSDR_CAMERA_KERNEL_BODY(PSDR_SEED_LOAD_NONE, (camera_sample<G, R, INTEG>(cx.sc, tv, st, cx.lp, cx.jump, pixel, slot, nrays)))
}
template <class G, class R, int INTEG, int FL, bool NOTREE = false>
__global__ __launch_bounds__(kBlock, (camera_waves<G, R, INTEG, FL, NOTREE>())) void k_camera_seeded(LaunchCtx cx, TV<R, FL> tv, int spp, int s_begin, SlotDiv nsp, long long n, float inv_spp,
                                                   float *__restrict__ img, float *__restrict__ dimg, long long plane,
                                                   unsigned long long *counters, int own, const ulonglong2 *__restrict__ seed) {
    static_assert((FL & kScenePre) == 0, "seeded launches have no probe rows");
    constexpr long long j0 = 0;
    const ProbeView pv{nullptr, nullptr};
    PSDR_CAMERA_KERNEL_BODY(PSDR_SEED_LOAD, (((void) slot), camera_sample<G, R, INTEG>(cx.sc, tv, st, cx.lp, seeded_rng(sd, cx.jump), pixel, nrays)))
}
#undef PSDR_CAMERA_KERNEL_BODY
#undef PSDR_SEED_LOAD
#undef PSDR_SEED_LOAD_NONE

template <int K>
__global__ __launch_bounds__(kBlock) void k_logd_check(const float *__restrict__ texels, TangentView<K, 0> tv, int n, unsigned long long *counters, int *bad) {
    const int i = blockIdx.x * kBlock + threadIdx.x;
    bool b = false;
    if (i < n) {
        bool moved = false;
#pragma unroll
        for (int k = 0; k < K; ++k) moved = moved || tv.t[k].d_texels[i] != 0.f;
        b = moved && !(fabsf(texels[i]) > 1e-20f);
    }
    if (__ballot(b) != 0ull && (threadIdx.x & 63) == 0) atomicOr(bad, 1);
}
__global__ void k_logd_gate(unsigned long long *counters, const int *bad) { if (threadIdx.x == 0 && blockIdx.x == 0) counters[kLogdGateWord] = *bad ? 0ull : 1ull; }
template <int K, int FL, bool NOTREE>
__global__ __launch_bounds__(kBlock, ((PSDR_LOGD_WAVES_K1 > 0 && K == 1 && NOTREE) ? PSDR_LOGD_WAVES_K1 : camera_waves<float, Dual<K>, PSDR_INTEGRATOR_PATH, FL, NOTREE>())) void k_camera_logd(LaunchCtx cx, TV<Dual<K>, FL> tv, int spp, int s_begin, SlotDiv nsp,
                                                   long long n, float inv_spp, float *__restrict__ img, float *__restrict__ dimg, long long plane, unsigned long long *counters, int own) {
    constexpr int NV = 3 * (1 + K);
    if (counters[kLogdGateWord] != 1ull) return;
    TraversalStack st; setup_lds(cx, st, tv);
    uint32_t nrays = 0;
    const long long nceil = (n + kBlock - 1) / kBlock * kBlock;
    for (long long j = (long long) blockIdx.x * kBlock + threadIdx.x; j < nceil; j += (long long) gridDim.x * kBlock) {
        const bool in = j < n;
        int pixel = 0x7fffffff, s_in = 0;
        if (in) slot_to_pixel(j, nsp, pixel, s_in);
        float v[NV];
#pragma unroll
        for (int i = 0; i < NV; ++i) v[i] = 0.f;
        if (in) {
            const uint64_t slot = (uint64_t) pixel * (uint64_t) spp + (uint64_t) (s_begin + s_in);
            const Vec3<Dual<K>> r = camera_sample_logd<K>(cx.sc, tv, st, cx.lp, cx.jump, pixel, slot, nrays);
            v[0] = r.x.v * inv_spp; v[1] = r.y.v * inv_spp; v[2] = r.z.v * inv_spp;
#pragma unroll
            for (int k = 0; k < K; ++k) { v[3 + 3 * k] = r.x.d[k] * inv_spp; v[4 + 3 * k] = r.y.d[k] * inv_spp; v[5 + 3 * k] = r.z.d[k] * inv_spp; }
        }
        const bool head = wave_segmented_sum<NV>(pixel, v);
        if (head && in) {
            float *p = img + (size_t) pixel * 3;
            if (own) {
                p[0] = v[0]; p[1] = v[1]; p[2] = v[2];
#pragma unroll
                for (int k = 0; k < K; ++k) { float *q = dimg + (size_t) k * plane + (size_t) pixel * 3; q[0] = v[3 + 3 * k]; q[1] = v[4 + 3 * k]; q[2] = v[5 + 3 * k]; }
            } else {
                if (v[0] != 0.f) atomicAdd(p, v[0]);
                if (v[1] != 0.f) atomicAdd(p + 1, v[1]);
                if (v[2] != 0.f) atomicAdd(p + 2, v[2]);
#pragma unroll
                for (int k = 0; k < K; ++k) {
                    float *q = dimg + (size_t) k * plane + (size_t) pixel * 3;
                    if (v[3 + 3 * k] != 0.f) atomicAdd(q, v[3 + 3 * k]);
                    if (v[4 + 3 * k] != 0.f) atomicAdd(q + 1, v[4 + 3 * k]);
                    if (v[5 + 3 * k] != 0.f) atomicAdd(q + 2, v[5 + 3 * k]);
                }
            }
        }
    }
    count_rays(counters, nrays);
}

constexpr int kWfGroups = 16, kWfClasses = 4, kWfGrab = 8;
constexpr int kWfStageInts = (kWfSub + 1) * kWfCountStride;
struct PathStream {
    int32_t *pixel; uint32_t *slot; int32_t *tri; float *hu, *hv; float *dir; float *beta;
    float *acc;
    long long cap;
    int32_t *count;
    long long sub_cap;
    int32_t binned;
    float4 *hit;
    float *prev_t;
};
constexpr int kWfClsShift = 29;
constexpr int32_t kWfTriMask = (1 << kWfClsShift) - 1;
struct TraceQueue {
    float4 *req;
    int32_t *count;
    long long sub_cap;
};
struct WfRec {
    float *disk; long long stride;
    int spp, s_begin, nsp; long long j0;
    int stage;
    __device__ __forceinline__ long long column(int pixel, uint32_t slot) const {
        return (long long) pixel * nsp + (long long) (slot - (uint32_t) pixel * (uint32_t) spp - (uint32_t) s_begin) - j0;
    }
};

template <class M>
__device__ __forceinline__ void stream_write(const PathStream &out, long long i, int pixel, uint32_t slot, const Its<float> &next, const Vec3f &dir, const Vec3<M> &beta,
                                             const Vec3<M> &acc, int cls = 0) {
    constexpr int K = ad_traits<M>::K;
    out.pixel[i] = pixel; out.slot[i] = slot; out.tri[i] = next.tri | (cls << kWfClsShift); out.hu[i] = next.hu; out.hv[i] = next.hv;
    out.dir[i] = dir.x; out.dir[out.cap + i] = dir.y; out.dir[2 * out.cap + i] = dir.z;
    out.beta[i] = val(beta.x); out.beta[out.cap + i] = val(beta.y); out.beta[2 * out.cap + i] = val(beta.z);
    out.acc[i] = val(acc.x); out.acc[out.cap + i] = val(acc.y); out.acc[2 * out.cap + i] = val(acc.z);
#pragma unroll
    for (int k = 0; k < K; ++k) {
        out.beta[(3 + 3 * k) * out.cap + i] = tangent(beta.x, k); out.beta[(4 + 3 * k) * out.cap + i] = tangent(beta.y, k);
        out.beta[(5 + 3 * k) * out.cap + i] = tangent(beta.z, k);
        out.acc[(3 + 3 * k) * out.cap + i] = tangent(acc.x, k); out.acc[(4 + 3 * k) * out.cap + i] = tangent(acc.y, k);
        out.acc[(5 + 3 * k) * out.cap + i] = tangent(acc.z, k);
    }
}

template <class M>
__device__ __forceinline__ void stream_push(const PathStream &out, bool alive, int pixel, uint32_t slot, const Its<float> &next,
                                            const Vec3f &dir, const Vec3<M> &beta, const Vec3<M> &acc) {
    const unsigned long long mask = __ballot(alive);
    if (mask == 0ull) return;
    const int lane = threadIdx.x & 63, sub = blockIdx.x % kWfSub;
    int base = 0;
    if (lane == __ffsll((long long) mask) - 1) base = atomicAdd(out.count + sub * kWfCountStride, (int) __popcll(mask));
    base = __shfl(base, __ffsll((long long) mask) - 1, 64);
    if (!alive) return;
    const long long i = (long long) sub * out.sub_cap + base + __popcll(mask & ((1ull << lane) - 1ull));
    stream_write<M>(out, i, pixel, slot, next, dir, beta, acc);
}

template <bool TRACED = false, class TVT>
__device__ __forceinline__ int classify_next(const SceneView &sc, const TVT &, Rng rng, const Its<float> &next, const Vec3f &,
                                             Vec3f *d_bsdf = nullptr, Vec3f *d_light = nullptr, bool emitter_only = false, TraversalStack *stp = nullptr) {
    const TangentView<0, TVT::flags> tv0{};
    const Its<float> &its = next;
    const int bsdf_id = Tab<TVT::flags>::mesh_bsdf(sc, its.mesh);
    if (bsdf_id < 0) return 0;
    auto enters = [&](const Vec3f &o, const Vec3f &d, float tmax) {
        const Vec3f inv{1.f / d.x, 1.f / d.y, 1.f / d.z};
        bool any = false;
        for (int k = 0; k < sc.n_blas; ++k) { float te; any = any || blas_box(sc, k, o, inv, tmax, te); }
        return any;
    };
    const float s[3] = {rng.next(), rng.next(), rng.next()};
    const float s0 = rng.next(), s1 = rng.next();
    int cls = 0;
    const Bsdf<float, float> bsdf(sc, tv0, bsdf_id);
    Vec3f wo_s; float pdf_s;
    if (bsdf.sample(sc, tv0, its, s, true, wo_s, pdf_s)) {
        const Vec3f d1 = its.sh.s * wo_s.x + its.sh.t * wo_s.y + its.sh.n * wo_s.z;
        bool wanted = true;
        if constexpr (!TVT::has_env && TVT::forest && PSDR_EMITTER_PRETEST) {
            if (emitter_only && sc.emit_rows != 0u && stp != nullptr) wanted = closest_hit<false, 2, true>(sc, *stp, its.p, d1, INFINITY, -1, -1, 0, sc.emit_rows).tri >= 0;
        }
        if (wanted && enters(its.p, d1, INFINITY)) cls |= 1;
        if (TRACED) *d_bsdf = d1;
    }
    const PosSample<float> ps = sample_emitter_position<float>(sc, tv0, its.p, s0, s1, false);
    if (ps.valid) {
        Vec3f wo = ps.p - its.p;
        const float dist = sqrtf(fmaxf(dot(wo, wo), 0.f));
        wo = wo / dist;
        const bool lit = PSDR_SKIP_UNLIT ? (its.sh.to_local(wo).z > 0.f && its.wi.z > 0.f) : true;
        if (lit && enters(its.p, wo, TRACED ? INFINITY : dist)) cls |= 2;
// ... 1100 lines not shown
__global__ __launch_bounds__(kBlock) void k_sum_replicas(float *__restrict__ dst, const float *__restrict__ rep, long long n, int reps) {
    const long long i = (long long) blockIdx.x * kBlock + threadIdx.x;
    if (i >= n) return;
    float s = 0.f;
    for (int r = 0; r < reps; ++r) s += rep[(size_t) r * n + i];
    if (s != 0.f) dst[i] += s;
}
template <int FL, int INTEG>
__global__ __launch_bounds__(kBlock, PSDR_WAVES_PE) void k_primary_edge_rev(LaunchCtx cx, PrimaryEdgeSink<FL> sink, long long i0, long long n, float inv_sppe,
                                                                            const float *__restrict__ adj_img, unsigned long long *counters,
                                                                            const uint32_t *__restrict__ order) {
    TraversalStack st; setup_lds(cx, st);
    uint32_t nrays = 0;
    const long long nceil = (n + kBlock - 1) / kBlock * kBlock;
    for (long long j = (long long) blockIdx.x * kBlock + threadIdx.x; j < nceil; j += (long long) gridDim.x * kBlock) {
        float w[4] = {0.f, 0.f, 0.f, 0.f};
        int edge = -1;
        if (j < n)
            edge = primary_edge_reverse_values<INTEG, FL>(cx.sc, st, cx.lp, cx.jump, (uint64_t) (i0 + (order ? (long long) order[j] : j)), inv_sppe, adj_img,
                                                          nrays, w);
        const bool head = wave_run_sum<4>(edge, w);
        if (head && edge >= 0) {
#pragma unroll
            for (int i = 0; i < 4; ++i) sink.add_pedge(edge, i, w[i]);
        }
    }
    count_rays(counters, nrays);
}

template <int FL>
__global__ __launch_bounds__(kBlock) void k_secondary_edge_rev(LaunchCtx cx, DeviceSink<FL> sink, long long i0, long long n, float inv_sppse,
                                                               const float *__restrict__ adj_img, unsigned long long *counters,
                                                               const uint32_t *__restrict__ list, const int *__restrict__ list_n) {
    TraversalStack st; setup_lds(cx, st);
    sink.begin(dyn_lds_floats(cx.off_sink));
    uint32_t nrays = 0;
    const bool guided = cx.sc.d.guide_cmf != nullptr && cx.sc.d.num_guide_cells > 0;
    if (list != nullptr) n = *list_n;
    for (long long jj = (long long) blockIdx.x * kBlock + threadIdx.x; jj < n; jj += (long long) gridDim.x * kBlock) {
        const long long j = list != nullptr ? (long long) list[jj] : jj;
        Rng rng; rng.init((uint64_t) (i0 + j), cx.jump);
        float s3[3] = {rng.next(), rng.next(), rng.next()};
        const float pdf0 = guided ? guide_sample_reuse(cx.sc, s3) : 1.f;
        secondary_edge_reverse(sink, cx.sc, st, s3, (pdf0 > kEpsilon ? 1.f / pdf0 : 1.f) * inv_sppse, adj_img, nrays, list == nullptr);
    }
    sink.end();
    count_rays(counters, nrays);
}


template <int FL> int make_device_sink(const psdr_scene_s *h, const psdr_grads *grads, DeviceSink<FL> &sink) {
    sink.g = *grads; sink.L = make_sink_layout(h, grads);
    if ((FL & kSceneTiny) != 0 && PSDR_TINY_DIRECT_ROWS && grads->g_tri_info != nullptr && !(h->hot_identity && sink.L.hot_rows == h->desc.num_tris))
        return fail("psdr_render_d_rev: the gradient cache of a scene without a tree does not hold every triangle row");
    return 0;
}
inline bool tangents_move_geometry(const psdr_tangents *tangents, int K) {
    bool geo = false;
    for (int k = 0; k < K; ++k) geo = geo || tangents[k].d_tri_info || tangents[k].d_cam_to_world;
    return geo;
}
struct EdgeLaunch { LaunchCtx cx; long long i0, n; const uint32_t *order; };
inline int begin_edge_term(psdr_scene_s *h, const psdr_render_opts *o, int sampler, EdgeLaunch &e, hipStream_t s) {
    if (int rc = make_ctx(h, o, sampler, e.cx)) return rc;
    const long long WH = (long long) h->desc.width * h->desc.height;
    const int begin = sampler == 1 ? o->sppe_begin : o->sppse_begin, end = sampler == 1 ? o->sppe_end : o->sppse_end;
    e.i0 = WH * begin; e.n = WH * (end - begin);
    h->slots[sampler] += (uint64_t) e.n;
    e.order = nullptr;
    return sampler == 1 ? primary_edge_order(h, e.cx, e.i0, e.n, &e.order, s) : 0;
}
template <int FL> int begin_pe_replicas(psdr_scene_s *h, const psdr_grads *grads, const EdgeLaunch &e, PrimaryEdgeSink<FL> &pe_sink, hipStream_t s) {
    const long long pe_words = (long long) h->desc.num_prim_edges * PSDR_PEDGE_STRIDE;
    const int reps = primary_edge_replicas(pe_words, e.n);
    if (reps > 1) {
        const size_t need = (size_t) reps * pe_words * sizeof(float);
        if (int rc = scratch_reserve(&h->d_pe_rep, &h->pe_rep_bytes, need, s, "primary-edge gradient replicas")) return rc;
        HIP_TRY(hipMemsetAsync(h->d_pe_rep, 0, need, s));
    }
    pe_sink = PrimaryEdgeSink<FL>{reps > 1 ? reinterpret_cast<float *>(h->d_pe_rep) : grads->g_prim_edge, pe_words, reps};
    h->rev_layout[9] = reps; h->rev_layout[15] = e.order != nullptr ? 1 : 0;
    return 0;
}
template <int FL> int end_pe_replicas(psdr_scene_s *h, const psdr_grads *grads, const PrimaryEdgeSink<FL> &pe_sink, hipStream_t s) {
    if (pe_sink.reps > 1) {
        hipLaunchKernelGGL(k_sum_replicas, dim3((unsigned) ((pe_sink.rep_stride + kBlock - 1) / kBlock)), dim3(kBlock), 0, s, grads->g_prim_edge,
                           reinterpret_cast<const float *>(h->d_pe_rep), pe_sink.rep_stride, pe_sink.reps);
        HIP_TRY(hipGetLastError());
    }
    return 0;
}
template <int FL> int probe_and_trace(psdr_scene_s *h, const psdr_render_opts *o, const LaunchCtx &cx, long long c0, long long nc, ProbeBuffers &pb, hipStream_t s) {
    const int probe_per_cu = big_launch_per_cu(h, nc);
    if (int rc = probe_buffers(h, nc, 3, pb, s, probe_per_cu)) return rc;
    const TraceQueue tq{pb.req, pb.count, pb.sub_cap};
    const int blocks = (launch_blocks(h, nc, probe_per_cu) + kWfSub - 1) / kWfSub * kWfSub;
    hipLaunchKernelGGL(k_direct_probe<FL>, dim3(blocks), dim3(kBlock), lds_bytes(cx, h), s, cx, TangentView<0, FL>{}, o->spp, o->spp_begin, SlotDiv(o->spp_end - o->spp_begin), c0, nc, tq,
                       pb.hit, pb.mask, make_rng_jump(o->rng_offset[0] + 2));
    HIP_TRY(hipGetLastError());
    return launch_wf_trace(h, pb.req, pb.count, pb.sub_cap, pb.hit, s);
}
inline const ulonglong2 *seed_table(psdr_scene_s *h, const psdr_render_opts *o, long long WH, int nsp, long long n, hipStream_t s) {
    if (h->opt.seed_cache == 0 || n <= 0 || n > (1ll << std::max(0, std::min(40, h->opt.seed_cache_log2)))) return nullptr;
    const long long key[4] = {WH, (long long) o->spp, (long long) o->spp_begin, (long long) nsp};
    if (h->d_seed != nullptr && h->seed_valid && std::equal(key, key + 4, h->seed_key)) {
        if (s != h->seed_stream && h->seed_event != nullptr && hipStreamWaitEvent(s, h->seed_event, 0) != hipSuccess) { (void) hipGetLastError(); return nullptr; }
        return reinterpret_cast<const ulonglong2 *>(h->d_seed);
    }
    h->seed_valid = false;
    if ((size_t) n > h->seed_cap) {
        if (h->d_seed) { (void) hipFreeAsync(h->d_seed, s); h->d_seed = nullptr; h->seed_cap = 0; }
        void *nb = nullptr;
        if (hipMallocAsync(&nb, (size_t) n * sizeof(ulonglong2), s) != hipSuccess) { (void) hipGetLastError(); return nullptr; }
        h->d_seed = nb; h->seed_cap = (size_t) n;
    }
    if (h->seed_event == nullptr && hipEventCreateWithFlags(&h->seed_event, hipEventDisableTiming) != hipSuccess) { (void) hipGetLastError(); h->seed_event = nullptr; return nullptr; }
    hipLaunchKernelGGL(k_seed_fill, dim3((unsigned) ((n + kBlock - 1) / kBlock)), dim3(kBlock), 0, s, reinterpret_cast<ulonglong2 *>(h->d_seed), n, o->spp, o->spp_begin, SlotDiv(nsp));
    if (hipGetLastError() != hipSuccess || hipEventRecord(h->seed_event, s) != hipSuccess) { (void) hipGetLastError(); return nullptr; }
    std::copy(key, key + 4, h->seed_key);
    h->seed_valid = true; h->seed_stream = s; h->seed_fills++;
    return reinterpret_cast<const ulonglong2 *>(h->d_seed);
}
template <class G, class R, int FL> constexpr bool seeded_render_c() { return (FL & kSceneTiny) != 0 && (FL & kScenePre) == 0 && std::is_same<G, float>::value && std::is_same<R, float>::value; }
template <class G, class R, int FL>
int run_camera(psdr_scene_s *h, const psdr_render_opts *o, const TV<R, FL> &tv, float *img, float *dimg, hipStream_t s) {
    const long long WH = (long long) h->desc.width * h->desc.height;
    const int nsp = o->spp_end - o->spp_begin;
    if (o->spp <= 0 || nsp <= 0) return 0;
    LaunchCtx cx;
    if (int rc = make_ctx(h, o, 0, cx)) return rc;
    const long long n = WH * nsp;
    h->slots[0] += (uint64_t) n;
    if constexpr ((FL & kSceneForest) != 0) {
        if (o->integrator == PSDR_INTEGRATOR_DIRECT && probe_direct(h, o, n)) {
            TV<R, FL | kScenePre> tvp;
            for (int k = 0; k < (ad_traits<R>::K > 0 ? ad_traits<R>::K : 1); ++k) tvp.t[k] = tv.t[k];
            tvp.live = tv.live;
            LaunchCtx cxp = cx;
            plan_lds_no_walk(h, cxp);
            const long long chunk = std::min<long long>(n, launch_chunk(h, 25));
            const int own = wave_owns_pixels(h, nsp, chunk);
            for (long long c0 = 0; c0 < n; c0 += chunk) {
                const long long nc = std::min(chunk, n - c0);
                ProbeBuffers pb;
                if (int rc = probe_and_trace<FL>(h, o, cx, c0, nc, pb, s)) return rc;
                hipLaunchKernelGGL(HIP_KERNEL_NAME(k_camera<G, R, PSDR_INTEGRATOR_DIRECT, FL | kScenePre, false>), dim3(launch_blocks(h, nc, camera_blocks_per_cu(h, nc))), dim3(kBlock), cxp.off_stack, s,
                                   cxp, tvp, o->spp, o->spp_begin, SlotDiv(nsp), nc, 1.f / (float) o->spp, img, dimg, WH * 3, h->d_counters, c0, ProbeView{pb.hit, pb.mask}, own);
                HIP_TRY(hipGetLastError());
            }
            return 0;
        }
    }
    const int own = wave_owns_pixels(h, nsp, n);
    bool gated = false;
    if constexpr (logd_instance<G, R, PSDR_INTEGRATOR_PATH, FL>()) {
        constexpr int K = ad_traits<R>::K;
        bool texels_only = o->integrator == PSDR_INTEGRATOR_PATH && h->opt.logd != 0 && h->desc.num_texels > 0 && h->desc.texels != nullptr;
        for (int k = 0; k < K && texels_only; ++k) {
            const psdr_tangents &t = tv.t[k];
            texels_only = t.d_texels != nullptr && !t.d_tri_info && !t.d_emitter_rad && !t.d_cam_to_world && !t.d_sec_edge && !t.d_prim_edge && !t.d_env_f;
        }
        if (texels_only) {
            if (int rc = scratch_reserve(&h->d_logd_bad, &h->logd_bad_bytes, sizeof(int), s, "log-derivative gate")) return rc;
            int *bad = reinterpret_cast<int *>(h->d_logd_bad);
            HIP_TRY(hipMemsetAsync(bad, 0, sizeof(int), s));
            TangentView<K, 0> tvk;
            for (int k = 0; k < K; ++k) tvk.t[k] = tv.t[k];
            hipLaunchKernelGGL(k_logd_check<K>, dim3((unsigned) ((h->desc.num_texels + kBlock - 1) / kBlock)), dim3(kBlock), 0, s, h->desc.texels, tvk, h->desc.num_texels, h->d_counters, bad);
            hipLaunchKernelGGL(k_logd_gate, dim3(1), dim3(64), 0, s, h->d_counters, bad);
            bool lean = false;
            if constexpr (K == 1 && FL == kSceneTiny) { if (int rc = logd_lean_launch_8(h, o, cx, tv, img, dimg, s, &lean)) return rc; }
            if (!lean)
                hipLaunchKernelGGL(HIP_KERNEL_NAME(k_camera_logd<K, FL, ((FL & kSceneTiny) != 0)>), dim3(launch_blocks(h, n, camera_blocks_per_cu(h, n))), dim3(kBlock), lds_bytes(cx, h), s, cx, tv,
                                   o->spp, o->spp_begin, SlotDiv(nsp), n, 1.f / (float) o->spp, img, dimg, WH * 3, h->d_counters, own);
            HIP_TRY(hipGetLastError());
            h->logd_launches++;
            gated = true;
        }
    }
#define PSDR_LAUNCH_CAMERA_T(INTEG, NOTREE)                                                                                        \
    hipLaunchKernelGGL(HIP_KERNEL_NAME(k_camera<G, R, INTEG, FL, NOTREE>), dim3(launch_blocks(h, n, camera_blocks_per_cu(h, n))), dim3(kBlock), lds_bytes(cx, h), s, cx, tv, o->spp, \
                       o->spp_begin, nsp, n, 1.f / (float) o->spp, img, dimg, WH * 3, h->d_counters, 0ll, ProbeView{nullptr, nullptr}, own)
#define PSDR_LAUNCH_CAMERA(INTEG) PSDR_LAUNCH_CAMERA_T(INTEG, ((FL & kSceneTiny) != 0))
    if constexpr (seeded_render_c<G, R, FL>()) {
        if (o->integrator == PSDR_INTEGRATOR_PATH) {
            if (const ulonglong2 *seed = seed_table(h, o, WH, nsp, n, s)) {
                hipLaunchKernelGGL(HIP_KERNEL_NAME(k_camera_seeded<G, R, PSDR_INTEGRATOR_PATH, FL, true>), dim3(launch_blocks(h, n, camera_blocks_per_cu(h, n))), dim3(kBlock), lds_bytes(cx, h), s, cx, tv,
                                   o->spp, o->spp_begin, SlotDiv(nsp), n, 1.f / (float) o->spp, img, dimg, WH * 3, h->d_counters, own, seed);
                HIP_TRY(hipGetLastError());
                h->seed_launches++;
                return 0;
            }
        }
    }
    switch (o->integrator) {
        case PSDR_INTEGRATOR_DIRECT: PSDR_LAUNCH_CAMERA(PSDR_INTEGRATOR_DIRECT); break;
        case PSDR_INTEGRATOR_PATH: PSDR_LAUNCH_CAMERA(PSDR_INTEGRATOR_PATH); break;
        case PSDR_INTEGRATOR_FIELD: PSDR_LAUNCH_CAMERA(PSDR_INTEGRATOR_FIELD); break;
        default: return fail("Unknown integrator");
    }
#undef PSDR_LAUNCH_CAMERA
#undef PSDR_LAUNCH_CAMERA_T
    HIP_TRY(hipGetLastError());
    if (gated) HIP_TRY(hipMemsetAsync(h->d_counters + kLogdGateWord, 0, sizeof(unsigned long long), s));
    return 0;
}


constexpr int kWfMaxDepth = 256;
struct WfRecArgs { float *disk; long long stride, c0, nc; };
template <class M, int FL>
int run_camera_wavefront(psdr_scene_s *h, const psdr_render_opts *o, const TV<M, FL> &tv, float *img, float *dimg, hipStream_t s, const WfRecArgs *rec = nullptr) {
    constexpr int K = ad_traits<M>::K;
    const long long WH = (long long) h->desc.width * h->desc.height;
    const int nsp = o->spp_end - o->spp_begin;
    if (o->spp <= 0 || nsp <= 0) return 0;
    const long long n_all = WH * nsp;
    const long long n = rec ? rec->nc : n_all;
    bool traced = false;
    if constexpr ((FL & kSceneForest) != 0) traced = traced_wavefront(h);
    const bool binned = !traced && (FL & kSceneForest) != 0 && h->n_blas > 0 && h->wf_binned;
    const int depth = o->max_depth;
    const size_t words = 8 + 6 * (1 + K) + (traced ? 8 : 0);
    const long long cap = rec ? n : std::min(n, fit_chunk(binned ? launch_chunk(h, 24) : launch_chunk(h, traced ? 26 : 25), 2 * words * 4 * 5 / 4 + (traced ? 80 : 0), 64u << 20, h->ws_bytes));
    const auto wf_per_cu = [&](long long slots) { return traced ? big_launch_per_cu(h, slots) : 16; };
    const long long max_blocks = ((long long) launch_blocks(h, cap, wf_per_cu(cap)) + kWfSub - 1) / kWfSub * kWfSub;
    const long long binned_sub_cap = (((cap + kBlock - 1) / kBlock + kWfSub) / kWfGroups + 2) * kBlock;
    const long long cap_alloc = ((binned ? binned_sub_cap * kWfSub : cap + max_blocks * kBlock) + 63) / 64 * 64;
    const size_t cnt_ints = (size_t) (kWfMaxDepth + 1) * kWfStageInts + (traced ? (size_t) (kWfMaxDepth + 1) * kWfSub * kWfCountStride : 0);
    const size_t cnt_bytes = cnt_ints * sizeof(int32_t);
    const size_t req_bytes = traced ? (size_t) 2 * cap_alloc * 2 * sizeof(float4) : 0;
    const size_t need = 2 * words * 4 * (size_t) cap_alloc + cnt_bytes + req_bytes;
    if (int rc = workspace_reserve(h, need, s)) return rc;
    int32_t *cnt = reinterpret_cast<int32_t *>(h->d_ws);
    int32_t *req_cnt = cnt + (size_t) (kWfMaxDepth + 1) * kWfStageInts;
    PathStream st[2];
    for (int i = 0; i < 2; ++i) {
        float *b = reinterpret_cast<float *>(reinterpret_cast<char *>(h->d_ws) + cnt_bytes) + (size_t) i * words * cap_alloc;
        const long long c = cap_alloc;
        st[i].cap = c;
        st[i].pixel = reinterpret_cast<int32_t *>(b); st[i].slot = reinterpret_cast<uint32_t *>(b + c); st[i].tri = reinterpret_cast<int32_t *>(b + 2 * c);
        st[i].hu = b + 3 * c; st[i].hv = b + 4 * c; st[i].dir = b + 5 * c; st[i].beta = b + 8 * c; st[i].acc = b + (8 + 3 * (1 + K)) * c;
        st[i].hit = traced ? reinterpret_cast<float4 *>(b + (8 + 6 * (1 + K)) * c) : nullptr;
        st[i].prev_t = nullptr;
        st[i].binned = binned ? 1 : 0;
    }
    TraceQueue tq{};
    tq.req = traced ? reinterpret_cast<float4 *>(reinterpret_cast<char *>(h->d_ws) + cnt_bytes + 2 * words * 4 * (size_t) cap_alloc) : nullptr;
    if (!rec) h->slots[0] += (uint64_t) n;
    const float inv_spp = 1.f / (float) o->spp;
    const long long j_first = rec ? rec->c0 : 0;
    for (long long j0 = j_first; j0 < j_first + n; j0 += cap) {
        const long long cn = std::min(cap, j_first + n - j0);
        LaunchCtx cx;
        if (int rc = make_ctx(h, o, 0, cx)) return rc;
        HIP_TRY(hipMemsetAsync(cnt, 0, (size_t) (std::min(depth, kWfMaxDepth) + 1) * kWfStageInts * sizeof(int32_t), s));
        if (traced) HIP_TRY(hipMemsetAsync(req_cnt, 0, (size_t) (std::min(depth, kWfMaxDepth) + 1) * kWfSub * kWfCountStride * sizeof(int32_t), s));
        const int blocks = (launch_blocks(h, cn, wf_per_cu(cn)) + kWfSub - 1) / kWfSub * kWfSub;
        const long long trips = (cn + (long long) blocks * kBlock - 1) / ((long long) blocks * kBlock);
        st[0].sub_cap = st[1].sub_cap = binned ? binned_sub_cap : (blocks / kWfSub) * trips * kBlock;
        st[0].count = cnt;
        if constexpr ((FL & kSceneForest) != 0) {
            if (traced) {
                tq.sub_cap = 2 * st[0].sub_cap;
                tq.count = req_cnt;
                LaunchCtx cxp = cx;
                plan_lds(h, cxp, 1 << 30);
                cxp.sc.n_lnodes = cxp.sc.n_lbtris = cxp.sc.n_ltri = 0;
                const int dyn_p = cxp.off_stack;
                WfRec wr{};
                bool recording = false;
                if constexpr (K == 0) {
                    if (rec) { recording = true; wr = WfRec{rec->disk + (j0 - rec->c0), rec->stride, o->spp, o->spp_begin, nsp, j0, 0}; }
                }
                if (recording) {
                    if constexpr (K == 0)
                        hipLaunchKernelGGL(HIP_KERNEL_NAME(k_wf_camera<M, FL, true, true>), dim3(blocks), dim3(kBlock), lds_bytes(cx, h), s, cx, tv, o->spp, o->spp_begin, nsp, j0, cn,
                                           inv_spp, img, dimg, WH * 3, st[0], 1 | (depth == 1 ? 2 : 0), h->d_counters, make_rng_jump(o->rng_offset[0] + 2), tq, wr);
                } else
                hipLaunchKernelGGL(HIP_KERNEL_NAME(k_wf_camera<M, FL, true>), dim3(blocks), dim3(kBlock), lds_bytes(cx, h), s, cx, tv, o->spp, o->spp_begin, nsp, j0, cn,
                                   inv_spp, img, dimg, WH * 3, st[0], 1 | (depth == 1 ? 2 : 0), h->d_counters, make_rng_jump(o->rng_offset[0] + 2), tq, wr);
                HIP_TRY(hipGetLastError());
                for (int k = 0; k < depth; ++k) {
                    if (int rc = launch_wf_trace(h, tq.req, tq.count, tq.sub_cap, st[k & 1].hit, s)) return rc;
                    st[(k + 1) & 1].count = cnt + (size_t) (k + 1) * kWfStageInts;
                    tq.count = req_cnt + (size_t) (k + 1) * kWfSub * kWfCountStride;
                    cxp.jump = make_rng_jump(o->rng_offset[0] + 2 + 5 * (uint64_t) k);
                    wr.stage = k;
                    if (recording) {
                        if constexpr (K == 0)
                            hipLaunchKernelGGL(HIP_KERNEL_NAME(k_wf_bounce<M, FL, true, true>), dim3(blocks), dim3(kBlock), dyn_p, s, cxp, tv, inv_spp, img, dimg, WH * 3,
                                               st[k & 1], st[(k + 1) & 1], (k + 1 < depth ? 1 : 0) | (k + 2 == depth ? 2 : 0), h->d_counters, make_rng_jump(o->rng_offset[0] + 2 + 5 * (uint64_t) (k + 1)), tq, wr);
                    } else
                    hipLaunchKernelGGL(HIP_KERNEL_NAME(k_wf_bounce<M, FL, true>), dim3(blocks), dim3(kBlock), dyn_p, s, cxp, tv, inv_spp, img, dimg, WH * 3,
                                       st[k & 1], st[(k + 1) & 1], (k + 1 < depth ? 1 : 0) | (k + 2 == depth ? 2 : 0), h->d_counters, make_rng_jump(o->rng_offset[0] + 2 + 5 * (uint64_t) (k + 1)), tq, wr);
                    HIP_TRY(hipGetLastError());
                }
                continue;
            }
        }
        if (binned) {
            hipLaunchKernelGGL(HIP_KERNEL_NAME(k_wf_camera<M, FL>), dim3(blocks), dim3(kBlock), lds_bytes(cx, h), s, cx, tv, o->spp, o->spp_begin, nsp, j0, cn,
                               inv_spp, img, dimg, WH * 3, st[0], 1 | (depth == 1 ? 2 : 0), h->d_counters, make_rng_jump(o->rng_offset[0] + 2), tq, WfRec{});
            HIP_TRY(hipGetLastError());
            for (int k = 0; k < depth; ++k) {
                st[(k + 1) & 1].count = cnt + (size_t) (k + 1) * kWfStageInts;
                cx.jump = make_rng_jump(o->rng_offset[0] + 2 + 5 * (uint64_t) k);
                hipLaunchKernelGGL(HIP_KERNEL_NAME(k_wf_bounce<M, FL>), dim3(blocks), dim3(kBlock), lds_bytes(cx, h), s, cx, tv, inv_spp, img, dimg, WH * 3,
                                   st[k & 1], st[(k + 1) & 1], (k + 1 < depth ? 1 : 0) | (k + 2 == depth ? 2 : 0), h->d_counters, make_rng_jump(o->rng_offset[0] + 2 + 5 * (uint64_t) (k + 1)), tq, WfRec{});
                HIP_TRY(hipGetLastError());
            }
            continue;
        }
        hipLaunchKernelGGL(HIP_KERNEL_NAME(k_wf_camera<M, FL>), dim3(blocks), dim3(kBlock), lds_bytes(cx, h), s, cx, tv, o->spp, o->spp_begin, nsp, j0, cn,
                           inv_spp, img, dimg, WH * 3, st[0], (depth > 1 ? 1 : 0) | (depth == 2 ? 2 : 0), h->d_counters, make_rng_jump(o->rng_offset[0] + 2 + 5), tq, WfRec{});
        HIP_TRY(hipGetLastError());
        for (int k = 1; k < depth; ++k) {
            st[k & 1].count = cnt + (size_t) k * kWfStageInts;
            cx.jump = make_rng_jump(o->rng_offset[0] + 2 + 5 * (uint64_t) k);
            hipLaunchKernelGGL(HIP_KERNEL_NAME(k_wf_bounce<M, FL>), dim3(blocks), dim3(kBlock), lds_bytes(cx, h), s, cx, tv, inv_spp, img, dimg, WH * 3,
                               st[(k - 1) & 1], st[k & 1], (k + 1 < depth ? 1 : 0) | (k + 2 == depth ? 2 : 0), h->d_counters, make_rng_jump(o->rng_offset[0] + 2 + 5 * (uint64_t) (k + 1)), tq, WfRec{});
            HIP_TRY(hipGetLastError());
        }
    }
    return 0;
}

template <int K, int FL>
int run_camera_wavefront_geo(psdr_scene_s *h, const psdr_render_opts *o, const TangentView<K, FL> &tv, float *img, float *dimg, hipStream_t s) {
    const long long WH = (long long) h->desc.width * h->desc.height;
    const int nsp = o->spp_end - o->spp_begin;
    if (o->spp <= 0 || nsp <= 0) return 0;
    const long long n = WH * nsp;
    const int depth = o->max_depth;
    const size_t words = 8 + 6 * (1 + K) + 3 * K + 8;
    const long long cap = std::min(n, fit_chunk(launch_chunk(h, 26), 2 * words * 4 * 5 / 4 + 80, 64u << 20, h->ws_bytes));
    const auto wf_per_cu = [&](long long slots) { return big_launch_per_cu(h, slots); };
    const long long max_blocks = ((long long) launch_blocks(h, cap, wf_per_cu(cap)) + kWfSub - 1) / kWfSub * kWfSub;
    const long long cap_alloc = ((cap + max_blocks * kBlock) + 63) / 64 * 64;
    const size_t cnt_ints = (size_t) (kWfMaxDepth + 1) * kWfStageInts + (size_t) (kWfMaxDepth + 1) * kWfSub * kWfCountStride;
    const size_t cnt_bytes = cnt_ints * sizeof(int32_t);
    const size_t req_bytes = (size_t) 2 * cap_alloc * 2 * sizeof(float4);
    const size_t need = 2 * words * 4 * (size_t) cap_alloc + cnt_bytes + req_bytes;
// ... 350 lines not shown
```

### psdr-cuda_amd/csrc/psdr_logd_lean.hip

```cpp
#define PSDR_WIDE_TREE 0
#define PSDR_LEAF_PAIR 0
#include "psdr_kernels.h"
#include "psdr_logd_lean.h"

namespace {

constexpr int kLeanFlags = kSceneTiny;

template <int K, int FL, bool SEEDED>
__global__ __launch_bounds__(kBlock, PSDR_LOGD_WAVES_K1) void k_camera_logd_lean(LaunchCtx cx, TV<Dual<K>, FL> tv, int spp, int s_begin, SlotDiv nsp, long long n, float inv_spp,
                                                                                  float *__restrict__ img, float *__restrict__ dimg, long long plane, unsigned long long *counters, int own,
                                                                                  const ulonglong2 *__restrict__ seed) {
    constexpr int NV = 3 * (1 + K);
    if (counters[kLogdGateWord] != 1ull) return;
    TraversalStack st; setup_lds(cx, st, tv);
    Park pk{nullptr};
#if defined(__HIP_DEVICE_COMPILE__)
    pk.base = reinterpret_cast<float *>(psdr_dyn_lds + cx.off_park) + threadIdx.x;
#endif
    uint32_t nrays = 0;
    const long long nceil = (n + kBlock - 1) / kBlock * kBlock;
    for (long long jb = (long long) blockIdx.x * kBlock; jb < nceil; jb += (long long) gridDim.x * kBlock) {
        const long long j = jb + threadIdx.x;
        const bool in = j < n;
        int pixel = 0x7fffffff, s_in = 0;
        if (in) slot_to_pixel(j, nsp, pixel, s_in);
        Rng rng;
        if constexpr (SEEDED) {
            const ulonglong2 sd = in ? seed[j] : ulonglong2{0ull, 0ull};
            rng.init_seeded(sd.x, sd.y, cx.jump);
        } else {
            rng.init((uint64_t) pixel * (uint64_t) spp + (uint64_t) (s_begin + s_in), cx.jump);
        }
        const float j0 = rng.next(), j1 = rng.next();
        const int W = cx.sc.d.width;
        const float sx = ((float) (pixel % W) + j0) / (float) W, sy = ((float) (pixel / W) + j1) / (float) cx.sc.d.height;
        const TangentView<0, FL> tv0{};
        const RayT<float> ray = primary_ray<float>(cx.sc, tv0, sx, sy);
        const Vec3<Dual<K>> r = zero_nonfinite(li_path_logd_lean<K>(cx.sc, tv, st, cx.lp, rng, ray, in, nrays, pk));
        float v[NV];
        v[0] = in ? r.x.v * inv_spp : 0.f; v[1] = in ? r.y.v * inv_spp : 0.f; v[2] = in ? r.z.v * inv_spp : 0.f;
#pragma unroll
        for (int k = 0; k < K; ++k) { v[3 + 3 * k] = in ? r.x.d[k] * inv_spp : 0.f; v[4 + 3 * k] = in ? r.y.d[k] * inv_spp : 0.f; v[5 + 3 * k] = in ? r.z.d[k] * inv_spp : 0.f; }
        const bool head = wave_segmented_sum<NV>(pixel, v);
        if (head && in) {
            float *p = img + (size_t) pixel * 3;
            if (own) {
                p[0] = v[0]; p[1] = v[1]; p[2] = v[2];
#pragma unroll
                for (int k = 0; k < K; ++k) { float *q = dimg + (size_t) k * plane + (size_t) pixel * 3; q[0] = v[3 + 3 * k]; q[1] = v[4 + 3 * k]; q[2] = v[5 + 3 * k]; }
            } else {
                if (v[0] != 0.f) atomicAdd(p, v[0]);
                if (v[1] != 0.f) atomicAdd(p + 1, v[1]);
                if (v[2] != 0.f) atomicAdd(p + 2, v[2]);
#pragma unroll
                for (int k = 0; k < K; ++k) {
                    float *q = dimg + (size_t) k * plane + (size_t) pixel * 3;
                    if (v[3 + 3 * k] != 0.f) atomicAdd(q, v[3 + 3 * k]);
                    if (v[4 + 3 * k] != 0.f) atomicAdd(q + 1, v[4 + 3 * k]);
                    if (v[5 + 3 * k] != 0.f) atomicAdd(q + 2, v[5 + 3 * k]);
                }
            }
        }
    }
    count_rays(counters, nrays);
}

}

namespace psdr_host {
int logd_lean_launch_8(psdr_scene_s *h, const psdr_render_opts *o, const LaunchCtx &cx0, const psdr::TangentView<1, psdr::kSceneTiny> &tv, float *img, float *dimg, hipStream_t s, bool *ran) {
    *ran = false;
    if (h->opt.logd_park == 0) return 0;
    constexpr int kCuLds = 160 * 1024, park = ParkLayout<1>::cols * kBlock * 4;
    const int lds = (lds_bytes(cx0, h) + 15) / 16 * 16;
    const int limit = h->opt.lds_budget > 0 ? std::min(h->opt.lds_budget, kCuLds / PSDR_LOGD_WAVES_K1) : kCuLds / PSDR_LOGD_WAVES_K1;
    if (lds + park > limit) return 0;
    LaunchCtx cx = cx0;
    cx.off_park = lds;
    const long long WH = (long long) h->desc.width * h->desc.height;
    const int nsp = o->spp_end - o->spp_begin;
    const long long n = WH * nsp;
    const int own = wave_owns_pixels(h, nsp, n);
    const dim3 grid(launch_blocks(h, n, camera_blocks_per_cu(h, n)));
    const ulonglong2 *seed = seed_table(h, o, WH, nsp, n, s);
    if (seed != nullptr)
        hipLaunchKernelGGL(HIP_KERNEL_NAME(k_camera_logd_lean<1, kLeanFlags, true>), grid, dim3(kBlock), lds + park, s, cx, tv, o->spp, o->spp_begin, SlotDiv(nsp), n, 1.f / (float) o->spp, img, dimg,
                           WH * 3, h->d_counters, own, seed);
    else
        hipLaunchKernelGGL(HIP_KERNEL_NAME(k_camera_logd_lean<1, kLeanFlags, false>), grid, dim3(kBlock), lds + park, s, cx, tv, o->spp, o->spp_begin, SlotDiv(nsp), n, 1.f / (float) o->spp, img, dimg,
                           WH * 3, h->d_counters, own, seed);
    h->logd_lean_launches++;
    if (seed != nullptr) { h->logd_lean_seeded++; h->seed_launches++; }
    h->logd_lean_lds = lds; h->logd_lean_park = park;
    *ran = true;
    return 0;
}
}
```

### psdr-cuda_amd/csrc/psdr_plan.h

```cpp
#pragma once

namespace psdr_host {
inline int launch_blocks(const psdr_scene_s *h, long long n, int per_cu = 16) {
    const int forced = h->opt.blocks_per_cu;
    const long long need = (n + kBlock - 1) / kBlock;
    const long long cap = (long long) h->num_cus * (forced ? forced : per_cu);
    return (int) std::max(1LL, std::min(need, cap));
}

constexpr int kLdsBudget = 40 * 1024;
inline bool tiny_only(const psdr_scene_s *h) { return h->n_tiny > 0 && h->n_blas == 0; }
inline int emitter_faces(const psdr_scene_s *h) {
    int n = 0;
    for (int e = 0; e < h->desc.num_emitters && (size_t) (e + 1) * PSDR_EMITTER_I_STRIDE <= h->emitter_i.size(); ++e)
        n = std::max(n, h->emitter_i[(size_t) e * PSDR_EMITTER_I_STRIDE + 3] + h->emitter_i[(size_t) e * PSDR_EMITTER_I_STRIDE + 2]);
    return n;
}
constexpr int kLdsTexels = 256, kLdsTexelTangents = 3;
inline bool small_tables_fit(const psdr_scene_s *h) {
    const psdr_scene_desc &d = h->desc;
    return d.env_emitter < 0 && d.num_meshes <= 64 && d.num_bsdfs <= 32 && d.num_emitters >= 0 && d.num_emitters <= 8 &&
           (d.num_emitters == 0 || (d.face_cmf && d.face_pmf)) && emitter_faces(h) <= 64;
}
inline bool tiny_tables_ok(const psdr_scene_s *h) {
    return h->opt.tiny_variants != 0 && tiny_only(h) && small_tables_fit(h);
}
inline int scene_flag_set(const psdr_scene_s *h) {
    return (h->desc.env_emitter >= 0 ? kSceneEnv : 0) | (h->has_rough ? kSceneRough : 0) | (h->n_blas > 0 ? kSceneForest : 0) | (tiny_tables_ok(h) ? kSceneTiny : 0);
}
inline bool forest_tables(const psdr_scene_s *h) { return PSDR_FOREST_LDS_TABLES && h->n_blas > 0; }

inline int stack_entries_of(const psdr_scene_s *h) { return tiny_only(h) ? 0 : (h->wide ? h->stack_need4 + 1 : std::min(kBvhStack, h->bvh_depth + 2)); }
inline int staged_nodes_of(const psdr_scene_s *h) { return h->wide ? h->num_nodes4 : h->num_nodes; }
inline int plan_lds(const psdr_scene_s *h, LaunchCtx &cx, int reserved = 0) {
    const int forced = h->opt.lds_budget;
    const bool lean = !h->has_rough && h->desc.env_emitter < 0;
    const int budget = forced ? forced : (lean ? 28 * 1024 : kLdsBudget);
    const int stack_bytes = stack_entries_of(h) * kBlock * 4;
    int room = std::max(0, budget - reserved - stack_bytes);
    if (tiny_only(h)) room = std::max(room, staged_nodes_of(h) * kLdsNodeStride + h->num_btris * 48 + h->desc.num_tris * 96);
    SceneView &sc = cx.sc;
    int off = 0;
    sc.n_lnodes = std::min(staged_nodes_of(h), room / kLdsNodeStride); sc.off_lnodes = off; off += sc.n_lnodes * kLdsNodeStride; room -= sc.n_lnodes * kLdsNodeStride;
    sc.n_lbtris = (sc.n_lnodes == staged_nodes_of(h)) ? std::min(h->num_btris, room / 48) : 0;
    sc.off_lbtris = off; off += sc.n_lbtris * 48; room -= sc.n_lbtris * 48;
    sc.n_ltri = (sc.n_lbtris == h->num_btris) ? std::min(h->desc.num_tris, room / 96) : 0;
    sc.off_ltri = off; off += sc.n_ltri * 96;
    sc.off_lprim = off; off += h->n_tiny * kTinyHitWords * 4;
    sc.lt_trimesh = sc.lt_meshbsdf = sc.lt_meshemitter = sc.lt_bsdf = sc.lt_emf = sc.lt_emi = sc.lt_fcmf = sc.lt_fpmf = sc.lt_uv = sc.lt_tex = sc.lt_ecmf = sc.lt_epmf = -1;
    sc.lt_nfaces = 0; sc.lt_occ = -1; sc.occ = nullptr;
    const bool all_tables = tiny_tables_ok(h);
    if (all_tables || forest_tables(h)) {
        auto take = [&](int words) { const int o = off; off += (words * 4 + 15) / 16 * 16; return o; };
        const psdr_scene_desc &d = h->desc;
        sc.lt_nfaces = emitter_faces(h);
        if (all_tables) sc.lt_trimesh = take(d.num_tris);
        sc.lt_meshbsdf = take(d.num_meshes); sc.lt_meshemitter = take(d.num_meshes);
        sc.lt_bsdf = take(std::max(d.num_bsdfs, 1) * PSDR_BSDF_STRIDE);
        sc.lt_emf = take(d.num_emitters * PSDR_EMITTER_F_STRIDE); sc.lt_emi = take(d.num_emitters * PSDR_EMITTER_I_STRIDE);
        sc.lt_fcmf = take(sc.lt_nfaces); sc.lt_fpmf = take(sc.lt_nfaces);
        if (d.num_emitters > 1 && d.emitter_cmf && d.emitter_pmf) { sc.lt_ecmf = take(d.num_emitters); sc.lt_epmf = take(d.num_emitters); }
        if (all_tables && d.tri_uv) sc.lt_uv = take(d.num_tris * PSDR_TRIUV_STRIDE);
        if (d.num_texels > 0 && d.num_texels <= kLdsTexels) sc.lt_tex = take(d.num_texels * (1 + kLdsTexelTangents));
        if (all_tables && h->have_occ && h->d_occ != nullptr) { sc.occ = h->d_occ; sc.lt_occ = take(d.num_tris * d.num_tris); }
    }
    sc.lt_end = off;
    cx.off_stack = off;
    return off + stack_bytes;
}
inline int lds_bytes(const LaunchCtx &cx, const psdr_scene_s *h) { return cx.off_stack + stack_entries_of(h) * kBlock * 4; }
inline int plan_lds_no_walk(const psdr_scene_s *h, LaunchCtx &cx) {
    const int with_stacks = plan_lds(h, cx, 1 << 30);
    cx.sc.n_lnodes = cx.sc.n_lbtris = cx.sc.n_ltri = 0;
    return with_stacks;
}

inline bool open_scene(const psdr_scene_s *h) { return !(h->n_blas > 0 || (h->n_tiny > 0 && h->n_blas == 0)); }
inline bool traced_wavefront(const psdr_scene_s *h) { return h->traced_enabled && h->n_blas > 0 && h->num_nodes4 > 0 && h->d_nodes4 != nullptr; }
inline bool use_wavefront(const psdr_scene_s *h, const psdr_render_opts *o) {
    if (o->integrator != PSDR_INTEGRATOR_PATH || o->max_depth > 250) return false;
    if (h->desc.num_tris >= (1 << 29)) return false;
    if (o->flags & PSDR_FLAG_FUSED) return false;
    if (o->flags & PSDR_FLAG_WAVEFRONT) return true;
    if (o->max_depth < 2) return false;
    if (open_scene(h)) return true;
    const long long n = (long long) h->desc.width * h->desc.height * (o->spp_end - o->spp_begin);
    if (traced_wavefront(h)) return n >= (1ll << 16);
    return h->n_blas > 0 && h->wf_binned && n >= (1ll << 25);
}

inline SinkLayout make_sink_layout(const psdr_scene_s *h, const psdr_grads *g) {
    SinkLayout L{};
    int off = 0;
    L.cam_off = off; off += 16;
    if (g->g_env_f && h->desc.env_emitter >= 0) { L.env_off = off; L.env_n = PSDR_ENV_WORDS; off += PSDR_ENV_WORDS; }
    const int nt = h->desc.num_texels, nr = h->desc.num_emitters * 3;
    if (g->g_texels && nt > 0 && nt <= 2048) { L.tex_off = off; L.tex_n = nt; off += nt; }
    if (g->g_emitter_rad && nr > 0 && nr <= 256) { L.rad_off = off; L.rad_n = nr; off += nr; }
    if (g->g_tri_info && h->hot_rows > 0) {
        const int rows = std::min(h->hot_rows, (kSinkCacheWords - off) / PSDR_TRI_STRIDE);
        if (rows > 0) { L.hot_off = off; L.hot_rows = rows; L.hot_map = h->d_hot_map; L.hot_tris = h->d_hot_tris; off += rows * PSDR_TRI_STRIDE; }
    }
    L.total = off;
    L.stride = off | 1;
    L.rep = 1;
    const int max_rep = h->opt.sink_rep;
    while (L.rep * 2 <= max_rep && L.rep * 2 * L.stride <= kSinkCacheWords) L.rep *= 2;
    const bool priv_on = h->opt.sink_private != 0;
    L.priv_tri[0] = L.priv_tri[1] = -1; L.priv_slot[0] = L.priv_slot[1] = 0; L.priv_emitter = -1;
    if (priv_on && L.hot_rows > 0 && h->desc.num_emitters > 0 && h->desc.env_emitter != 0) {
        const int32_t *ei = h->emitter_i.data();
        const int n = std::min(std::min(ei[2], 2), L.hot_rows);
        for (int r = 0; r < n; ++r) { L.priv_tri[r] = ei[1] + r; L.priv_slot[r] = h->hot_identity ? ei[1] + r : r; }
        L.priv_rows = n;
        if (n > 0) { L.priv_off = (L.rep * L.stride + 3) / 4 * 4; if (L.rad_n) L.priv_emitter = 0; }
    }
    return L;
}

inline int camera_blocks_per_cu(const psdr_scene_s *h, long long n) {
    if (h->opt.camera_blocks > 0) return h->opt.camera_blocks;
    if (h->has_rough) return 16;
    if (h->n_tiny > 0 && h->n_blas == 0) return 40;
    const long long fit = n / ((long long) kBlock * h->num_cus * 2);
    return (int) std::max(16LL, std::min(64LL, fit));
}
inline int big_launch_per_cu(const psdr_scene_s *h, long long n) { return (int) std::max(16LL, std::min(40LL, n / ((long long) kBlock * h->num_cus * 8))); }
inline long long launch_chunk(const psdr_scene_s *h, int log2_default) { return 1ll << (h->opt.chunk_log2 > 0 ? h->opt.chunk_log2 : log2_default); }
inline bool probe_direct(const psdr_scene_s *h, const psdr_render_opts *o, long long n) {
    return traced_wavefront(h) && h->opt.probe != 0 && o->bsdf_samples == 1 && o->light_samples == 1 && !(o->flags & PSDR_FLAG_FUSED) && n >= (1ll << 16);
}
inline bool wave_owns_pixels(const psdr_scene_s *h, int nsp, long long chunk) {
    return h->opt.own_pixels != 0 && nsp <= 64 && 64 % nsp == 0 && chunk % nsp == 0;
}
inline bool path_sedge_split(const psdr_scene_s *h, long long n) {
    const int split_env = h->opt.sedge_split;
    return !(split_env == 0 || (split_env < 0 && n < (1ll << 18))) && n <= 0x7fffffffLL;
}
inline long long filter_grid_slots(long long n, int divisor) { return std::max(n / divisor, 1ll << 16); }
inline int primary_edge_replicas(long long pe_words, long long n) {
    int reps = 1;
    while (reps < 64 && (long long) (reps * 2) * pe_words * 4 <= (64ll << 20)) reps *= 2;
    return n < (1ll << 18) ? 1 : reps;
}

inline bool same_camera_samples(const psdr_render_opts &a, const psdr_render_opts &b) {
    return a.integrator == b.integrator && a.max_depth == b.max_depth && a.hide_emitters == b.hide_emitters && a.spp == b.spp && a.spp_begin == b.spp_begin &&
           a.spp_end == b.spp_end && a.rng_offset[0] == b.rng_offset[0] && ((a.flags ^ b.flags) & (PSDR_FLAG_FUSED | PSDR_FLAG_WAVEFRONT)) == 0;
}
inline int rev_record_words(int depth, bool wavefront) { return kRevDiskHead + (wavefront ? kRevDiskPerVertexCf : kRevDiskPerVertex) * depth; }
inline bool rev_launch_splits(const psdr_scene_s *h, const psdr_render_opts *o, long long n) {
    const int split_env = h->opt.rev_split;
    const bool replayable = o->integrator == PSDR_INTEGRATOR_PATH || (o->integrator == PSDR_INTEGRATOR_DIRECT && o->bsdf_samples <= 1 && o->light_samples <= 1);
    const bool has_tree = h->num_nodes > 0 && (h->n_tiny == 0 || h->n_blas > 0);
    const bool worth = o->integrator == PSDR_INTEGRATOR_PATH ? o->max_depth >= 2 : h->num_nodes >= 16384;
    return replayable && split_env != 0 && (split_env == 1 || (has_tree && worth && n >= (1ll << 20)));
}
inline bool rev_wavefront_sweep(const psdr_scene_s *h, const psdr_render_opts *o) {
    return o->integrator == PSDR_INTEGRATOR_PATH && std::min(o->max_depth, kMaxRevDepthDeep) <= kMaxRevDepth && traced_wavefront(h) && use_wavefront(h, o);
}
inline bool rev_value_sweep_is_wavefront(const psdr_scene_s *h, const psdr_render_opts *o, long long n) { return rev_launch_splits(h, o, n) && rev_wavefront_sweep(h, o); }

inline void rev_layout_of_sink(psdr_scene_s *h, const SinkLayout &L, bool deep_rec) {
    int32_t *r = h->rev_layout;
    r[0] = L.tex_n; r[1] = L.rad_n; r[2] = L.env_n; r[3] = L.hot_rows; r[4] = L.rep;
    r[5] = L.priv_rows; r[6] = L.priv_regs; r[7] = L.pend_rows;
    r[10] = h->hot_identity ? 1 : 0; r[11] = deep_rec ? 1 : 0; r[12] = L.priv_slot[0]; r[13] = L.priv_slot[1]; r[14] = h->hot_rows;
}

inline int plan_rev_one_vertex(const psdr_scene_s *h, LaunchCtx &cx, SinkLayout &L, int *dyn_bytes) {
    L.priv_rows = 0; L.priv_emitter = -1; L.priv_regs = 0;
    L.pend_rows = 0; L.pend_off = 0;
    const int cache_bytes = sink_bytes(L);
    plan_lds(h, cx, cache_bytes);
    cx.off_sink = lds_bytes(cx, h);
    *dyn_bytes = cx.off_sink + cache_bytes;
    if (*dyn_bytes > h->lds_limit) return fail("psdr_render_d_rev: the launch needs " + std::to_string(*dyn_bytes) + " bytes of LDS per workgroup (traversal stacks + gradient cache), the device offers " +
                                               std::to_string(h->lds_limit));
    return 0;
}

enum RevCameraForm { kRevFused = 0, kRevSplit = 1, kRevSplitWavefront = 2, kRevKeptRecords = 3, kRevProbe = 4 };
struct RevCameraPlan {
    int form, depth, rec_bytes, cache_bytes, dyn1, dyn_bytes;
    bool geo, deep_rec, split, kept_fused, no_tree;
};
inline int plan_rev_camera(psdr_scene_s *h, const psdr_render_opts *o, const psdr_grads *grads, long long n, int fl, bool reg_priv, bool value_only, bool has_out_img,
                           SinkLayout &L, LaunchCtx &cx, LaunchCtx &cx2, RevCameraPlan &p) {
    p.depth = o->integrator == PSDR_INTEGRATOR_PATH ? std::min(o->max_depth, kMaxRevDepthDeep) : 1;
    p.deep_rec = p.depth > kMaxRevDepth;
    p.rec_bytes = p.deep_rec ? 0 : p.depth * kPathRecWords * kBlock * 4;
    p.geo = value_only || grads->g_tri_info != nullptr || grads->g_cam_to_world != nullptr;
    const int wg_per_cu = (o->integrator == PSDR_INTEGRATOR_DIRECT && !(fl & kSceneRough)) ? 3 : 2;
    p.kept_fused = !value_only && p.geo && o->integrator == PSDR_INTEGRATOR_PATH && !p.deep_rec && h->opt.rev_split != 0 && h->kept.valid && h->kept.kind == 0 &&
                   h->kept.gen == h->tables_gen && h->kept.n == n && !has_out_img && same_camera_samples(h->kept.o, *o) && n <= launch_chunk(h, 26);
    p.split = value_only || p.kept_fused || (p.geo && rev_launch_splits(h, o, n));
    L.priv_regs = (p.geo && o->integrator == PSDR_INTEGRATOR_PATH && reg_priv) ? 1 : 0;
    cx2 = cx;
    const int stacks_only = plan_lds_no_walk(h, cx2);
    const int base2 = cx2.off_stack;
    const int floor_bytes = (p.split ? base2 : stacks_only) + p.rec_bytes;
    if (!L.priv_regs && L.priv_rows > 0 && floor_bytes + sink_bytes(L) > h->lds_limit / wg_per_cu) { L.priv_rows = 0; L.priv_emitter = -1; }
    L.pend_rows = 0; L.pend_off = 0;
    if (p.geo && h->opt.rev_sorted != 0 && grads->g_tri_info != nullptr && o->integrator == PSDR_INTEGRATOR_PATH) {
        for (int rows = std::min(p.depth, 4); rows >= 1; --rows) {
            SinkLayout t = L;
            sink_reserve_pending(t, rows);
            if (floor_bytes + sink_bytes(t) <= h->lds_limit / wg_per_cu) { L = t; break; }
        }
    }
    p.cache_bytes = sink_bytes(L);
    rev_layout_of_sink(h, L, p.deep_rec);
    plan_lds(h, cx, p.split ? p.rec_bytes : p.rec_bytes + p.cache_bytes);
    cx.off_pathrec = lds_bytes(cx, h);
    cx.off_sink = cx.off_pathrec + p.rec_bytes;
    cx2.off_pathrec = base2; cx2.off_sink = base2 + p.rec_bytes;
    p.no_tree = lds_bytes(cx, h) == cx.off_stack;
    if (p.split && p.no_tree) cx2 = cx;
    p.dyn1 = cx.off_pathrec + p.rec_bytes;
    p.dyn_bytes = (p.split ? cx2.off_sink : cx.off_sink) + p.cache_bytes;
    if (std::max(p.dyn_bytes, p.split ? p.dyn1 : 0) > h->lds_limit) return fail("psdr_render_d_rev: the launch needs " + std::to_string(p.dyn_bytes) + " bytes of LDS per workgroup (path record of " +
                                              std::to_string(p.depth) + " levels + traversal stacks + gradient cache), the device offers " + std::to_string(h->lds_limit));
    const bool forest = (fl & kSceneForest) != 0;
    const bool wf_value = forest && p.split && !value_only && !p.kept_fused && !p.no_tree && rev_wavefront_sweep(h, o);
    const bool direct_probe = forest && !p.split && !p.no_tree && o->integrator == PSDR_INTEGRATOR_DIRECT && probe_direct(h, o, n);
    p.form = p.split ? (wf_value ? kRevSplitWavefront : kRevSplit) : direct_probe ? kRevProbe : kRevFused;
    if (direct_probe) p.dyn_bytes = cx2.off_sink + p.cache_bytes;
    h->rev_layout[8] = p.form;
    return 0;
}
}
```

### psdr-cuda_amd/psdr_cuda/_abi.py

```python
import ctypes as C
import os

_HERE = os.path.dirname(os.path.abspath(__file__))
PKG_ROOT = os.path.dirname(_HERE)
REPO_ROOT = os.path.dirname(PKG_ROOT)

TRI_STRIDE = 24
TRIUV_STRIDE = 8
SEDGE_STRIDE = 16
PEDGE_STRIDE = 8
BSDF_STRIDE = 16
EMITTER_F_STRIDE = 8
EMITTER_I_STRIDE = 4
CAM_WORDS = 64
ENV_WORDS = 32
TRI_FACE_NORMALS = 0x40000000

BSDF_DIFFUSE, BSDF_ROUGHCONDUCTOR, BSDF_MICROFACET, BSDF_MICROFACET_NORMAL, BSDF_MICROFACET_HEIGHT = 0, 1, 2, 3, 4
SLOT_REFLECTANCE, SLOT_ALPHA_U, SLOT_ALPHA_V, SLOT_ETA, SLOT_K = range(5)
CAM_SAMPLE_TO_CAMERA, CAM_TO_WORLD, CAM_WORLD_TO_SAMPLE, CAM_POS, CAM_DIR, CAM_INV_AREA = 0, 16, 32, 48, 51, 54
INTEGRATOR_DIRECT, INTEGRATOR_PATH, INTEGRATOR_FIELD, INTEGRATOR_COLLOCATED, INTEGRATOR_POINT, INTEGRATOR_POINT_STACK = 0, 1, 2, 3, 4, 5
POINT_LIGHTS_MAX = 256
LIGHT_POINT, LIGHT_DISTANT = 0, 1
DISTANT_IN_ENV = "a distant light cannot reach a scene inside an environment map's bounding mesh (env_emitter >= 0)"
FLAG_FUSED, FLAG_WAVEFRONT, FLAG_LITERAL_FORMS, FLAG_KEEP_RECORDS, FLAG_PATH_SEDGES = 1, 2, 4, 8, 16
MAX_PATH_SEDGE_DEPTH = 8
FIELDS = {"silhouette": 0, "position": 1, "depth": 2, "geoNormal": 3, "shNormal": 4, "uv": 5}

_fp = C.c_void_p


class SceneDesc(C.Structure):
    _fields_ = [
        ("width", C.c_int32), ("height", C.c_int32),
        ("num_tris", C.c_int32), ("num_meshes", C.c_int32), ("num_bsdfs", C.c_int32), ("num_emitters", C.c_int32),
        ("num_sec_edges", C.c_int32), ("num_prim_edges", C.c_int32), ("num_texels", C.c_int32),
        ("num_guide_cells", C.c_int32),
        ("tri_info", _fp), ("tri_uv", _fp), ("tri_mesh", _fp), ("mesh_bsdf", _fp), ("mesh_emitter", _fp),
        ("bsdf_rec", _fp), ("texels", _fp), ("emitter_f", _fp), ("emitter_i", _fp),
        ("face_cmf", _fp), ("face_pmf", _fp), ("emitter_cmf", _fp), ("emitter_pmf", _fp),
        ("emitter_sum", C.c_float),
        ("cam", _fp),
        ("sec_edge", _fp), ("sec_cmf", _fp), ("sec_pmf", _fp), ("sec_sum", C.c_float),
        ("prim_edge", _fp), ("prim_cmf", _fp), ("prim_pmf", _fp), ("prim_sum", C.c_float),
        ("guide_reso", C.c_int32 * 3),
        ("guide_cmf", _fp), ("guide_pmf", _fp), ("guide_sum", C.c_float),
        ("env_emitter", C.c_int32), ("env_tex", C.c_int32 * 3), ("env_reso", C.c_int32 * 2),
        ("env_f", _fp), ("env_cmf", _fp), ("env_pmf", _fp), ("env_sum", C.c_float),
        ("material_mask", C.c_uint32),
        ("sec_edge_faces", _fp),
        ("prim_edge_z", _fp),
    ]


class RenderOpts(C.Structure):
    _fields_ = [
        ("integrator", C.c_int32), ("bsdf_samples", C.c_int32), ("light_samples", C.c_int32),
        ("max_depth", C.c_int32), ("hide_emitters", C.c_int32), ("field", C.c_int32),
        ("spp", C.c_int32), ("sppe", C.c_int32), ("sppse", C.c_int32),
        ("spp_begin", C.c_int32), ("spp_end", C.c_int32),
        ("sppe_begin", C.c_int32), ("sppe_end", C.c_int32),
        ("sppse_begin", C.c_int32), ("sppse_end", C.c_int32),
        ("flags", C.c_int32),
        ("rng_offset", C.c_uint64 * 3),
    ]


class Tangents(C.Structure):
    _fields_ = [("d_tri_info", _fp), ("d_texels", _fp), ("d_emitter_rad", _fp), ("d_cam_to_world", _fp),
                ("d_sec_edge", _fp), ("d_prim_edge", _fp), ("d_env_f", _fp)]


class Grads(C.Structure):
    _fields_ = [("g_tri_info", _fp), ("g_texels", _fp), ("g_emitter_rad", _fp), ("g_cam_to_world", _fp),
                ("g_sec_edge", _fp), ("g_prim_edge", _fp), ("g_env_f", _fp)]


class SmoothInfo(C.Structure):
    _fields_ = [("iterations", C.c_int32), ("converged", C.c_int32), ("form", C.c_int32), ("launches", C.c_int32), ("rel_residual", C.c_float * 3),
                ("one_workgroup_limit", C.c_int32), ("one_workgroup_default", C.c_int32), ("num_vertices", C.c_int32), ("num_entries", C.c_int32),
                ("long_rows", C.c_int32)]


SMOOTH_FORMS = {-1: "none", 0: "multi_launch", 1: "one_workgroup"}

TANGENT_FIELDS = ("tri_info", "texels", "emitter_rad", "cam_to_world", "sec_edge", "prim_edge", "env_f")

HIP_SYMBOLS = (
    "psdr_last_error", "psdr_version", "psdr_abi_struct_sizes", "psdr_scene_create", "psdr_scene_destroy", "psdr_scene_set_option", "psdr_scene_set_tables",
    "psdr_bvh_build", "psdr_bvh_stats", "psdr_scene_info", "psdr_trace", "psdr_render_c", "psdr_render_d_fwd", "psdr_render_d_rev",
    "psdr_guide_build", "psdr_scene_set_point_light", "psdr_scene_set_point_lights", "psdr_scene_set_light", "psdr_scene_set_lights", "psdr_scene_set_path_guide", "psdr_path_guide_build", "psdr_get_counters", "psdr_scene_rev_layout", "psdr_scene_seed_info", "psdr_scene_logd_info",
    "psdr_geo_world_vertices_fwd", "psdr_geo_world_vertices_rev", "psdr_geo_tri_rows_fwd", "psdr_geo_tri_rows_rev", "psdr_geo_sec_edges_fwd", "psdr_geo_sec_edges_rev", "psdr_geo_prim_edges_fwd", "psdr_geo_prim_edges_rev",
    "psdr_geo_compact_edges_fwd", "psdr_geo_compact_edges_rev", "psdr_geo_emitter_tables",
    "psdr_geo_world_vertices_jvp", "psdr_geo_tri_rows_jvp", "psdr_geo_sec_edges_jvp", "psdr_geo_prim_edges_jvp", "psdr_geo_compact_edges_jvp",
    "psdr_cube_sample_reuse", "psdr_sample_boundary_segment_direct",
    "psdr_smooth_create", "psdr_smooth_destroy", "psdr_smooth_set_option", "psdr_smooth_apply", "psdr_smooth_solve", "psdr_smooth_info",
)

HIP_LIB_PATH = os.path.join(PKG_ROOT, "lib", "libpsdr_hip.so")


def use_library(path):
    global HIP_LIB_PATH
    if _hip is not None:
        raise RuntimeError("psdr_cuda._abi.use_library: the library is already loaded (%s)" % HIP_LIB_PATH)
    HIP_LIB_PATH = os.path.abspath(path)


_hip = None


def load_hip():
    global _hip
    if _hip is not None:
        return _hip
    if not os.path.exists(HIP_LIB_PATH):
        raise RuntimeError("libpsdr_hip.so not built (%s): run `python -c 'import __graft_entry__ as g; g.build()'`"
                           % HIP_LIB_PATH)
    lib = C.CDLL(HIP_LIB_PATH)
    lib.psdr_last_error.restype = C.c_char_p
    lib.psdr_version.restype = C.c_char_p
    vp, i32 = C.c_void_p, C.c_int32
    lib.psdr_scene_create.argtypes = [C.POINTER(vp)]
    lib.psdr_scene_destroy.argtypes = [vp]
    lib.psdr_scene_set_option.argtypes = [vp, C.c_char_p, C.c_double]
    lib.psdr_scene_set_tables.argtypes = [vp, C.POINTER(SceneDesc)]
    lib.psdr_bvh_build.argtypes = [vp, vp]
    lib.psdr_trace.argtypes = [vp, i32] + [vp] * 7 + [vp] * 4 + [vp]
    lib.psdr_render_c.argtypes = [vp, C.POINTER(RenderOpts), vp, vp]
    lib.psdr_render_d_fwd.argtypes = [vp, C.POINTER(RenderOpts), i32, C.POINTER(Tangents), vp, vp, vp]
    lib.psdr_render_d_rev.argtypes = [vp, C.POINTER(RenderOpts), vp, vp, C.POINTER(Grads), vp]
    lib.psdr_guide_build.argtypes = [vp, C.POINTER(RenderOpts), C.POINTER(i32), i32, vp, vp]
    lib.psdr_scene_set_point_light.argtypes = [vp, C.POINTER(C.c_float), i32, C.POINTER(C.c_float), vp]
    lib.psdr_scene_set_point_lights.argtypes = [vp, i32, C.POINTER(C.c_float), i32, C.POINTER(C.c_float), vp]
    lib.psdr_scene_set_light.argtypes = [vp, i32, C.POINTER(C.c_float), i32, C.POINTER(C.c_float), vp]
    lib.psdr_scene_set_lights.argtypes = [vp, i32, C.POINTER(C.c_int32), C.POINTER(C.c_float), i32, C.POINTER(C.c_float), vp]
    lib.psdr_scene_set_path_guide.argtypes = [vp, C.POINTER(i32), vp, vp, C.c_float]
    lib.psdr_path_guide_build.argtypes = [vp, C.POINTER(RenderOpts), i32, C.POINTER(i32), i32, vp, vp]
    lib.psdr_get_counters.argtypes = [vp, C.POINTER(C.c_uint64)]
    lib.psdr_scene_info.argtypes = [vp, C.POINTER(i32)]
    lib.psdr_scene_rev_layout.argtypes = [vp, C.POINTER(i32)]
    lib.psdr_scene_seed_info.argtypes = [vp, C.POINTER(C.c_int64)]
    lib.psdr_scene_logd_info.argtypes = [vp, C.POINTER(C.c_int64)]
    lib.psdr_geo_world_vertices_fwd.argtypes = [i32, vp, vp, vp, vp, vp]
    lib.psdr_geo_world_vertices_rev.argtypes = [i32, vp, vp, vp, vp, vp, vp, vp]
    lib.psdr_geo_tri_rows_fwd.argtypes = [i32, i32, vp, vp, vp, vp, i32, vp]
    lib.psdr_geo_tri_rows_rev.argtypes = [i32, i32, vp, vp, vp, vp, i32, vp, vp, vp]
    lib.psdr_geo_sec_edges_fwd.argtypes = [i32, vp, vp, vp, i32, vp, vp, vp]
    lib.psdr_geo_sec_edges_rev.argtypes = [i32, vp, vp, vp, vp, i32, vp]
    lib.psdr_geo_prim_edges_fwd.argtypes = [i32, vp, vp, vp, vp, i32, vp, vp, vp, vp, vp]
    lib.psdr_geo_prim_edges_rev.argtypes = [i32, vp, vp, vp, vp, vp, vp, vp]
    lib.psdr_geo_compact_edges_fwd.argtypes = [i32, vp, i32, vp, i32, i32, vp, i32, i32, vp, vp, vp, vp, vp, vp, vp, vp]
    lib.psdr_geo_compact_edges_rev.argtypes = [i32, i32, vp, vp, vp, vp]
    lib.psdr_geo_world_vertices_jvp.argtypes = [i32, vp, vp, vp, vp, vp, vp, vp, vp]
    lib.psdr_geo_tri_rows_jvp.argtypes = [i32, i32, vp, vp, vp, vp, i32, vp, vp, vp]
    lib.psdr_geo_sec_edges_jvp.argtypes = [i32, vp, vp, vp, i32, vp, vp]
    lib.psdr_geo_prim_edges_jvp.argtypes = [i32, vp, vp, vp, vp, vp, vp, vp]
    lib.psdr_geo_compact_edges_jvp.argtypes = [i32, i32, vp, vp, vp, vp]
    lib.psdr_geo_emitter_tables.argtypes = [i32, vp, i32, vp, vp, i32, vp, vp, vp, vp, vp, vp, vp, vp, vp, vp]
    lib.psdr_cube_sample_reuse.argtypes = [i32, C.POINTER(i32), vp, vp, C.c_float, i32, i32, vp, vp, vp]
    lib.psdr_sample_boundary_segment_direct.argtypes = [C.POINTER(SceneDesc), i32] + [vp] * 12
    lib.psdr_smooth_create.argtypes = [i32, i32, vp, C.POINTER(vp)]
    lib.psdr_smooth_destroy.argtypes = [vp]
    lib.psdr_smooth_destroy.restype = None
    lib.psdr_smooth_set_option.argtypes = [vp, C.c_char_p, C.c_int]
    lib.psdr_smooth_apply.argtypes = [vp, C.c_float, vp, vp, vp]
    lib.psdr_smooth_solve.argtypes = [vp, C.c_float, vp, vp, vp, C.c_float, i32, vp]
    lib.psdr_smooth_info.argtypes = [vp, C.POINTER(SmoothInfo)]
    for name in HIP_SYMBOLS:
        if name not in ("psdr_last_error", "psdr_version", "psdr_smooth_destroy"):
            getattr(lib, name).restype = C.c_int
    sizes = (C.c_int32 * 4)()
    lib.psdr_abi_struct_sizes(sizes)
    mine = (C.sizeof(SceneDesc), C.sizeof(RenderOpts), C.sizeof(Tangents), C.sizeof(Grads))
    if tuple(sizes) != mine:
        raise RuntimeError("psdr_cuda/_abi.py is out of sync with include/psdr_hip.h: %s vs %s" % (tuple(sizes), mine))
    _hip = lib
    return lib


def check(lib, rc):
    if rc != 0:
        msg = lib.psdr_last_error()
        raise RuntimeError(msg.decode() if msg else "psdr_hip call failed (rc=%d)" % rc)


def scene_stats(handle):
    lib = load_hip()
    out = (C.c_int32 * 8)()
    check(lib, lib.psdr_scene_info(handle, out))
    return {"n_tiny": out[0], "n_blas": out[1], "n_inline": out[2], "leaf_tris": out[3], "device_built": out[4], "n_slab": out[5], "occ_rows": out[6], "occ_max_rows": out[7]}


REV_LAUNCH_KINDS = {-1: "none", 0: "fused", 1: "split", 2: "split_wavefront", 3: "kept_records", 4: "probe"}


def rev_layout(handle):
    lib = load_hip()
    out = (C.c_int32 * 16)()
    check(lib, lib.psdr_scene_rev_layout(handle, out))
    return {"tex_n": out[0], "rad_n": out[1], "env_n": out[2], "hot_rows": out[3], "rep": out[4], "priv_rows": out[5], "priv_regs": out[6],
            "pend_rows": out[7], "launch": REV_LAUNCH_KINDS[out[8]], "pe_reps": out[9], "hot_identity": out[10], "deep_rec": out[11],
            "priv_slot": (out[12], out[13]), "tree_hot_rows": out[14], "pe_sorted": out[15]}


def seed_cache_info(handle):
    lib = load_hip()
    out = (C.c_int64 * 4)()
    check(lib, lib.psdr_scene_seed_info(handle, out))
    return {"slots": int(out[0]), "bytes": int(out[1]), "fills": int(out[2]), "launches": int(out[3])}


def logd_info(handle):
    lib = load_hip()
    out = (C.c_int64 * 4)()
    check(lib, lib.psdr_scene_logd_info(handle, out))
    return {"launches": int(out[0]), "lean": int(out[1]), "lean_seeded": int(out[2]), "lean_lds_bytes": int(out[3])}


def make_opts(integrator=INTEGRATOR_DIRECT, bsdf_samples=1, light_samples=1, max_depth=1, hide_emitters=False,
              field=0, spp=1, sppe=0, sppse=0, spp_range=None, sppe_range=None, sppse_range=None,
              rng_offset=(0, 0, 0), flags=0):
    o = RenderOpts()
    o.flags = flags
    o.integrator, o.bsdf_samples, o.light_samples = integrator, bsdf_samples, light_samples
    o.max_depth, o.hide_emitters, o.field = max_depth, int(bool(hide_emitters)), field
    o.spp, o.sppe, o.sppse = spp, sppe, sppse
    o.spp_begin, o.spp_end = spp_range if spp_range is not None else (0, spp)
    o.sppe_begin, o.sppe_end = sppe_range if sppe_range is not None else (0, sppe)
    o.sppse_begin, o.sppse_end = sppse_range if sppse_range is not None else (0, sppse)
    for i in range(3):
        o.rng_offset[i] = int(rng_offset[i])
    return o


def draws_per_slot(opts):
    if opts.integrator == INTEGRATOR_DIRECT:
        li = 3 * opts.bsdf_samples + 2 * opts.light_samples
    elif opts.integrator == INTEGRATOR_PATH:
        li = 5 * opts.max_depth
    else:
        li = 0
    se = 3
    if opts.integrator == INTEGRATOR_PATH and (opts.flags & FLAG_PATH_SEDGES) and opts.max_depth >= 2:
        se = 11 * opts.max_depth - 9
    return (2 + li, 1 + 2 * li, se)
```

Measured before the change: 20850 Mpath-samples/s.

## Taper camera-kernel work distribution with shrinking tail segments to cut straggler imbalance

```diff
diff --git a/__graft_entry__.py b/__graft_entry__.py
--- a/__graft_entry__.py
+++ b/__graft_entry__.py
@@ -38,6 +38,7 @@
     "lightstage": ("hostcheck/hostcheck_lightstage.cpp", "hostcheck/libhostcheck_lightstage.so", _product_and_harness, HOST_FLAGS),
     "distantlight": ("hostcheck/hostcheck_distantlight.cpp", "hostcheck/libhostcheck_distantlight.so", _product_and_harness, HOST_FLAGS),
     "plan": ("hostcheck/hostcheck_plan.cpp", "hostcheck/libhostcheck_plan.so", _product_and_harness, HOST_FLAGS),
+    "taper": ("hostcheck/hostcheck_taper.cpp", "hostcheck/libhostcheck_taper.so", _product_and_harness, HOST_FLAGS),
     "smooth": ("hostcheck/hostcheck_smooth.cpp", "hostcheck/libhostcheck_smooth.so", lambda: [os.path.join(CSRC, "psdr_smooth.h")], HOST_FLAGS),
     "poison": ("poison/poison.hip", "poison/libpoison.so", lambda: [], ["-O1"]),
 }
diff --git a/include/psdr_hip.h b/include/psdr_hip.h
--- a/include/psdr_hip.h
+++ b/include/psdr_hip.h
@@ -246,6 +246,8 @@
 
 int psdr_scene_logd_info(psdr_scene_t h, int64_t out[4]);
 
+int psdr_scene_taper_info(psdr_scene_t h, int32_t which, int32_t out[42]);
+
 int psdr_get_counters(psdr_scene_t h, uint64_t out[4]);
 
 #ifdef __cplusplus
diff --git a/psdr-cuda_amd/csrc/psdr_hip.hip b/psdr-cuda_amd/csrc/psdr_hip.hip
--- a/psdr-cuda_amd/csrc/psdr_hip.hip
+++ b/psdr-cuda_amd/csrc/psdr_hip.hip
@@ -724,8 +724,9 @@
 int psdr_scene_create(psdr_scene_t *out) {
     if (!out) return fail("psdr_scene_create: null output");
     psdr_scene_s *h = new psdr_scene_s();
-    hipError_t e = hipMalloc(&h->d_counters, sizeof(unsigned long long) * kRayCounters * kRayCounterStride);
+    hipError_t e = hipMalloc(&h->d_counters, sizeof(unsigned long long) * (kRayCounters * kRayCounterStride + kTimelineWords));
     if (e != hipSuccess) { delete h; return fail(std::string("hipMalloc: ") + hipGetErrorString(e)); }
+    if (kTimelineWords > 0) (void) hipMemset(h->d_counters, 0, sizeof(unsigned long long) * (kRayCounters * kRayCounterStride + kTimelineWords));
     int dev = 0; hipDeviceProp_t prop;
     if (hipGetDevice(&dev) == hipSuccess && hipGetDeviceProperties(&prop, dev) == hipSuccess) {
         h->num_cus = prop.multiProcessorCount;
@@ -764,6 +765,8 @@
     else if (n == "wf_geo") h->opt.wf_geo = iv;
     else if (n == "logd") h->opt.logd = iv;
     else if (n == "seed_cache") h->opt.seed_cache = iv;
+    else if (n == "taper_rounds") h->opt.taper = std::max(0, std::min(8, iv));
+    else if (n == "taper_places") h->opt.taper_places = std::max(0, iv);
     else if (n == "logd_park") h->opt.logd_park = iv;
     else if (n == "seed_cache_log2") h->opt.seed_cache_log2 = std::max(0, std::min(40, iv));
     else if (n == "keep_records") h->opt.keep_records = iv;
@@ -1299,6 +1302,25 @@
     out[0] = h->logd_launches; out[1] = h->logd_lean_launches; out[2] = h->logd_lean_seeded; out[3] = (int64_t) h->logd_lean_lds + h->logd_lean_park;
     return 0;
 }
+int psdr_scene_taper_info(psdr_scene_t h, int32_t which, int32_t out[42]) {
+    if (!h || !out || which < 0 || which > 1) return fail("psdr_scene_taper_info: null argument or unknown launch");
+    const TaperPlan &p = h->taper_last[which];
+    out[0] = p.nseg; out[1] = p.grid;
+    for (int s = 0; s < kTaperSegs; ++s) {
+        const TaperSeg &g = p.seg[s];
+        const int32_t v[5] = {g.wg0, g.wgs, g.trips, g.block0, g.stride};
+        std::copy(v, v + 5, out + 2 + 5 * s);
+    }
+    return 0;
+}
+#if PSDR_WG_TIMELINE
+extern "C" int psdr_scene_wg_timeline(psdr_scene_t h, uint64_t *out, int n_wg) {
+    if (!h || !out || n_wg < 0 || n_wg > kTimelineGrid) return fail("psdr_scene_wg_timeline: bad argument");
+    HIP_TRY(hipMemcpyAsync(out, h->d_counters + kRayCounters * kRayCounterStride, sizeof(uint64_t) * 4 * (size_t) n_wg, hipMemcpyDeviceToHost, h->last_stream));
+    HIP_TRY(hipStreamSynchronize(h->last_stream));
+    return 0;
+}
+#endif
 int psdr_scene_seed_info(psdr_scene_t h, int64_t out[4]) {
     if (!h || !out) return fail("psdr_scene_seed_info: null argument");
     out[0] = h->seed_valid ? h->seed_key[0] * h->seed_key[3] : 0; out[1] = (int64_t) (h->seed_cap * sizeof(ulonglong2)); out[2] = h->seed_fills; out[3] = h->seed_launches;
diff --git a/psdr-cuda_amd/csrc/psdr_host.h b/psdr-cuda_amd/csrc/psdr_host.h
--- a/psdr-cuda_amd/csrc/psdr_host.h
+++ b/psdr-cuda_amd/csrc/psdr_host.h
@@ -113,6 +113,10 @@
 constexpr int kPrivRowWords = 13;
 constexpr int kPrivWords = 2 * kPrivRowWords + 3;
 
+constexpr int kTaperSegs = 8;
+struct TaperSeg { int32_t wg0, wgs, trips, block0, stride; };
+struct TaperPlan { int32_t nseg, grid; TaperSeg seg[kTaperSegs]; };
+
 struct psdr_scene_options {
     int blocks_per_cu = 0;
     int camera_blocks = 0;
@@ -139,6 +143,8 @@
     int seed_cache = 1;
     int seed_cache_log2 = 25;
     int logd_park = 1;
+    int taper = 1;
+    int taper_places = 0;
     int bvh_maxleaf = 4;
     float bvh_tcost = 2.0f;
 };
@@ -230,6 +236,7 @@
     long long seed_fills = 0, seed_launches = 0;
     long long logd_launches = 0, logd_lean_launches = 0, logd_lean_seeded = 0;
     int logd_lean_lds = 0, logd_lean_park = 0;
+    TaperPlan taper_last[2] = {};
     void *d_ws = nullptr;
     size_t ws_bytes = 0;
     void *d_live = nullptr;
@@ -256,6 +263,10 @@
 };
 
 constexpr int kRayCounters = 64, kRayCounterStride = 16;
+#ifndef PSDR_WG_TIMELINE
+#define PSDR_WG_TIMELINE 0
+#endif
+constexpr int kTimelineGrid = 1 << 15, kTimelineWords = PSDR_WG_TIMELINE ? 4 * kTimelineGrid : 0;
 constexpr int kWfSub = 64, kWfCountStride = 32;
 constexpr int kTraceBlock = 1024, kTraceNodeStride = 80, kTraceStackMax = 16;
 
diff --git a/psdr-cuda_amd/csrc/psdr_kernels.h b/psdr-cuda_amd/csrc/psdr_kernels.h
--- a/psdr-cuda_amd/csrc/psdr_kernels.h
+++ b/psdr-cuda_amd/csrc/psdr_kernels.h
@@ -125,14 +125,33 @@
     seed[j] = ulonglong2{rng.state, rng.inc};
 }
 __device__ __forceinline__ Rng seeded_rng(const ulonglong2 &sd, const RngJump &jump) { Rng rng; rng.init_seeded(sd.x, sd.y, jump); return rng; }
-#define PSDR_CAMERA_KERNEL_BODY(SEED_LOAD, SAMPLE) \
+#if PSDR_WG_TIMELINE
+__device__ __forceinline__ void wg_stamp(unsigned long long *counters, int k) {
+    if (threadIdx.x == 0 && blockIdx.x < (unsigned) kTimelineGrid) counters[kRayCounters * kRayCounterStride + 4 * blockIdx.x + k] = __builtin_amdgcn_s_memrealtime();
+}
+#define PSDR_WG_STAMP(counters, k) wg_stamp(counters, k)
+#else
+#define PSDR_WG_STAMP(counters, k)
+#endif
+struct TaperRange { long long j0, step, end; };
+__device__ __forceinline__ TaperRange taper_range(const TaperPlan &tp, long long nceil) {
+    const int wg = (int) blockIdx.x;
+    unsigned s = 0;
+#pragma clang loop unroll(disable) vectorize(disable) interleave(disable)
+    for (unsigned i = 1; i < (unsigned) tp.nseg; ++i) s = wg >= tp.seg[i].wg0 ? i : s;
+    const long long end = s + 1 < (unsigned) tp.nseg ? (long long) tp.seg[s + 1].block0 * kBlock : nceil;
+    return TaperRange{((long long) tp.seg[s].block0 + (wg - tp.seg[s].wg0)) * kBlock, (long long) tp.seg[s].stride * kBlock, end};
+}
+#define PSDR_CAMERA_KERNEL_BODY(SEED_LOAD, SAMPLE, ENTRY, STAGED, SLOT_LOOP, EXIT) \
     constexpr int K = ad_traits<R>::K; \
     constexpr int NV = 3 * (1 + K); \
     if constexpr (logd_instance<G, R, INTEG, FL>()) { if (counters[kLogdGateWord] == 1ull) return; } \
+    ENTRY \
     TraversalStack st; setup_lds(cx, st, tv); \
+    STAGED \
     uint32_t nrays = 0; \
     const long long nceil = (n + kBlock - 1) / kBlock * kBlock; \
-    for (long long j = (long long) blockIdx.x * kBlock + threadIdx.x; j < nceil; j += (long long) gridDim.x * kBlock) { \
+    SLOT_LOOP \
         const bool in = j < n; \
         SEED_LOAD \
         int pixel = 0x7fffffff, s_in = 0; \
@@ -172,27 +191,39 @@
             } \
         } \
     } \
-    count_rays(counters, nrays);
+    count_rays(counters, nrays); \
+    EXIT
+#define PSDR_NOTHING
+#define PSDR_GRID_STRIDE_LOOP for (long long j = (long long) blockIdx.x * kBlock + threadIdx.x; j < nceil; j += (long long) gridDim.x * kBlock) {
+#define PSDR_TAPER_LOOP for (long long jb = tr.j0; jb < tr.end; jb += tr.step) { const long long j = jb + threadIdx.x;
 #define PSDR_SEED_LOAD_NONE
 #define PSDR_SEED_LOAD const ulonglong2 sd = in ? seed[j] : ulonglong2{0ull, 0ull};
 template <class G, class R, int INTEG, int FL, bool NOTREE = false>
 __global__ __launch_bounds__(kBlock, (camera_waves<G, R, INTEG, FL, NOTREE>())) void k_camera(LaunchCtx cx, TV<R, FL> tv, int spp, int s_begin, SlotDiv nsp, long long n, float inv_spp,
                                                    float *__restrict__ img, float *__restrict__ dimg, long long plane,
                                                    unsigned long long *counters, long long j0, ProbeView pv, int own) {
-    PSDR_CAMERA_KERNEL_BODY(PSDR_SEED_LOAD_NONE, (camera_sample<G, R, INTEG>(cx.sc, tv, st, cx.lp, cx.jump, pixel, slot, nrays)))
+    PSDR_CAMERA_KERNEL_BODY(PSDR_SEED_LOAD_NONE, (camera_sample<G, R, INTEG>(cx.sc, tv, st, cx.lp, cx.jump, pixel, slot, nrays)), PSDR_NOTHING, PSDR_NOTHING, PSDR_GRID_STRIDE_LOOP, PSDR_NOTHING)
 }
 template <class G, class R, int INTEG, int FL, bool NOTREE = false>
 __global__ __launch_bounds__(kBlock, (camera_waves<G, R, INTEG, FL, NOTREE>())) void k_camera_seeded(LaunchCtx cx, TV<R, FL> tv, int spp, int s_begin, SlotDiv nsp, long long n, float inv_spp,
                                                    float *__restrict__ img, float *__restrict__ dimg, long long plane,
-                                                   unsigned long long *counters, int own, const ulonglong2 *__restrict__ seed) {
+                                                   unsigned long long *counters, int own, const ulonglong2 *__restrict__ seed, TaperPlan tp) {
     static_assert((FL & kScenePre) == 0, "seeded launches have no probe rows");
     constexpr long long j0 = 0;
     const ProbeView pv{nullptr, nullptr};
-    PSDR_CAMERA_KERNEL_BODY(PSDR_SEED_LOAD, (((void) slot), camera_sample<G, R, INTEG>(cx.sc, tv, st, cx.lp, seeded_rng(sd, cx.jump), pixel, nrays)))
+    if constexpr (FL == kSceneTiny) {
+        PSDR_CAMERA_KERNEL_BODY(PSDR_SEED_LOAD, (((void) slot), camera_sample<G, R, INTEG>(cx.sc, tv, st, cx.lp, seeded_rng(sd, cx.jump), pixel, nrays)),
+                                PSDR_WG_STAMP(counters, 0); const TaperRange tr = taper_range(tp, (n + kBlock - 1) / kBlock * kBlock);, PSDR_WG_STAMP(counters, 1);, PSDR_TAPER_LOOP, PSDR_WG_STAMP(counters, 2);)
+    } else {
+        PSDR_CAMERA_KERNEL_BODY(PSDR_SEED_LOAD, (((void) slot), camera_sample<G, R, INTEG>(cx.sc, tv, st, cx.lp, seeded_rng(sd, cx.jump), pixel, nrays)), PSDR_NOTHING, PSDR_NOTHING, PSDR_GRID_STRIDE_LOOP, PSDR_NOTHING)
+    }
 }
 #undef PSDR_CAMERA_KERNEL_BODY
 #undef PSDR_SEED_LOAD
 #undef PSDR_SEED_LOAD_NONE
+#undef PSDR_GRID_STRIDE_LOOP
+#undef PSDR_TAPER_LOOP
+#undef PSDR_NOTHING
 
 template <int K>
 __global__ __launch_bounds__(kBlock) void k_logd_check(const float *__restrict__ texels, TangentView<K, 0> tv, int n, unsigned long long *counters, int *bad) {
@@ -1599,6 +1630,8 @@
         }
     }
     const int own = wave_owns_pixels(h, nsp, n);
+    if constexpr (seeded_render_c<G, R, FL>()) h->taper_last[0].nseg = 0;
+    if constexpr (logd_instance<G, R, PSDR_INTEGRATOR_PATH, FL>()) h->taper_last[1].nseg = 0;
     bool gated = false;
     if constexpr (logd_instance<G, R, PSDR_INTEGRATOR_PATH, FL>()) {
         constexpr int K = ad_traits<R>::K;
@@ -1632,10 +1665,13 @@
     if constexpr (seeded_render_c<G, R, FL>()) {
         if (o->integrator == PSDR_INTEGRATOR_PATH) {
             if (const ulonglong2 *seed = seed_table(h, o, WH, nsp, n, s)) {
-                hipLaunchKernelGGL(HIP_KERNEL_NAME(k_camera_seeded<G, R, PSDR_INTEGRATOR_PATH, FL, true>), dim3(launch_blocks(h, n, camera_blocks_per_cu(h, n))), dim3(kBlock), lds_bytes(cx, h), s, cx, tv,
-                                   o->spp, o->spp_begin, SlotDiv(nsp), n, 1.f / (float) o->spp, img, dimg, WH * 3, h->d_counters, own, seed);
+                const TaperPlan tp = FL == kSceneTiny ? plan_camera_launch(h, n, camera_waves<G, R, PSDR_INTEGRATOR_PATH, FL, true>())
+                                                      : taper_one_segment((n + kBlock - 1) / kBlock, launch_blocks(h, n, camera_blocks_per_cu(h, n)));
+                hipLaunchKernelGGL(HIP_KERNEL_NAME(k_camera_seeded<G, R, PSDR_INTEGRATOR_PATH, FL, true>), dim3(tp.grid), dim3(kBlock), lds_bytes(cx, h), s, cx, tv,
+                                   o->spp, o->spp_begin, SlotDiv(nsp), n, 1.f / (float) o->spp, img, dimg, WH * 3, h->d_counters, own, seed, tp);
                 HIP_TRY(hipGetLastError());
                 h->seed_launches++;
+                if (FL == kSceneTiny) h->taper_last[0] = tp;
                 return 0;
             }
         }
diff --git a/psdr-cuda_amd/csrc/psdr_logd_lean.hip b/psdr-cuda_amd/csrc/psdr_logd_lean.hip
--- a/psdr-cuda_amd/csrc/psdr_logd_lean.hip
+++ b/psdr-cuda_amd/csrc/psdr_logd_lean.hip
@@ -10,17 +10,19 @@
 template <int K, int FL, bool SEEDED>
 __global__ __launch_bounds__(kBlock, PSDR_LOGD_WAVES_K1) void k_camera_logd_lean(LaunchCtx cx, TV<Dual<K>, FL> tv, int spp, int s_begin, SlotDiv nsp, long long n, float inv_spp,
                                                                                   float *__restrict__ img, float *__restrict__ dimg, long long plane, unsigned long long *counters, int own,
-                                                                                  const ulonglong2 *__restrict__ seed) {
+                                                                                  const ulonglong2 *__restrict__ seed, TaperPlan tp) {
     constexpr int NV = 3 * (1 + K);
     if (counters[kLogdGateWord] != 1ull) return;
+    PSDR_WG_STAMP(counters, 0);
+    const TaperRange tr = taper_range(tp, (n + kBlock - 1) / kBlock * kBlock);
     TraversalStack st; setup_lds(cx, st, tv);
+    PSDR_WG_STAMP(counters, 1);
     Park pk{nullptr};
 #if defined(__HIP_DEVICE_COMPILE__)
     pk.base = reinterpret_cast<float *>(psdr_dyn_lds + cx.off_park) + threadIdx.x;
 #endif
     uint32_t nrays = 0;
-    const long long nceil = (n + kBlock - 1) / kBlock * kBlock;
-    for (long long jb = (long long) blockIdx.x * kBlock; jb < nceil; jb += (long long) gridDim.x * kBlock) {
+    for (long long jb = tr.j0; jb < tr.end; jb += tr.step) {
         const long long j = jb + threadIdx.x;
         const bool in = j < n;
         int pixel = 0x7fffffff, s_in = 0;
@@ -64,6 +66,7 @@
         }
     }
     count_rays(counters, nrays);
+    PSDR_WG_STAMP(counters, 2);
 }
 
 }
@@ -82,17 +85,19 @@
     const int nsp = o->spp_end - o->spp_begin;
     const long long n = WH * nsp;
     const int own = wave_owns_pixels(h, nsp, n);
-    const dim3 grid(launch_blocks(h, n, camera_blocks_per_cu(h, n)));
+    const TaperPlan tp = plan_camera_launch(h, n, PSDR_LOGD_WAVES_K1);
+    const dim3 grid(tp.grid);
     const ulonglong2 *seed = seed_table(h, o, WH, nsp, n, s);
     if (seed != nullptr)
         hipLaunchKernelGGL(HIP_KERNEL_NAME(k_camera_logd_lean<1, kLeanFlags, true>), grid, dim3(kBlock), lds + park, s, cx, tv, o->spp, o->spp_begin, SlotDiv(nsp), n, 1.f / (float) o->spp, img, dimg,
-                           WH * 3, h->d_counters, own, seed);
+                           WH * 3, h->d_counters, own, seed, tp);
     else
         hipLaunchKernelGGL(HIP_KERNEL_NAME(k_camera_logd_lean<1, kLeanFlags, false>), grid, dim3(kBlock), lds + park, s, cx, tv, o->spp, o->spp_begin, SlotDiv(nsp), n, 1.f / (float) o->spp, img, dimg,
-                           WH * 3, h->d_counters, own, seed);
+                           WH * 3, h->d_counters, own, seed, tp);
     h->logd_lean_launches++;
     if (seed != nullptr) { h->logd_lean_seeded++; h->seed_launches++; }
     h->logd_lean_lds = lds; h->logd_lean_park = park;
+    h->taper_last[1] = tp;
     *ran = true;
     return 0;
 }
diff --git a/psdr-cuda_amd/csrc/psdr_plan.h b/psdr-cuda_amd/csrc/psdr_plan.h
--- a/psdr-cuda_amd/csrc/psdr_plan.h
+++ b/psdr-cuda_amd/csrc/psdr_plan.h
@@ -125,6 +125,46 @@
     const long long fit = n / ((long long) kBlock * h->num_cus * 2);
     return (int) std::max(16LL, std::min(64LL, fit));
 }
+inline TaperPlan taper_one_segment(long long nb, int grid) {
+    TaperPlan p{};
+    p.nseg = 1; p.grid = grid;
+    p.seg[0] = TaperSeg{0, grid, (int32_t) ((nb + grid - 1) / grid), 0, grid};
+    return p;
+}
+inline TaperPlan plan_camera_taper(long long nb, int places, int waves, int per_cu, int taper) {
+    const long long cus = std::max(1, places / std::max(1, waves));
+    const int grid0 = (int) std::max(1LL, std::min(nb, cus * per_cu));
+    const long long trips0 = (nb + grid0 - 1) / grid0;
+    if (taper <= 0 || places <= 0 || nb < 2LL * places || nb > (1LL << 30) || trips0 < 2) return taper_one_segment(nb, grid0);
+    const long long tier_wgs = (long long) places * taper;
+    int tier_trips[kTaperSegs - 1], ntiers = 0;
+    for (long long t = std::min(trips0 / 2, 1LL << (kTaperSegs - 2)); t >= 1; t /= 2) tier_trips[ntiers++] = (int) t;
+    for (int first = 0; first < ntiers; ++first) {
+        long long tail = 0;
+        for (int i = first; i < ntiers; ++i) tail += tier_wgs * tier_trips[i];
+        const long long lead = nb - tail;
+        if (lead < tail) continue;
+        const long long lead_wgs = std::max(1LL, std::min(lead, (grid0 * lead + nb / 2) / nb));
+        if (lead / lead_wgs < tier_trips[first]) continue;
+        TaperPlan p{};
+        p.seg[0] = TaperSeg{0, (int32_t) lead_wgs, (int32_t) ((lead + lead_wgs - 1) / lead_wgs), 0, (int32_t) lead_wgs};
+        long long wg = lead_wgs, block = lead;
+        p.nseg = 1;
+        for (int i = first; i < ntiers; ++i) {
+            p.seg[p.nseg++] = TaperSeg{(int32_t) wg, (int32_t) tier_wgs, tier_trips[i], (int32_t) block, (int32_t) tier_wgs};
+            wg += tier_wgs; block += tier_wgs * tier_trips[i];
+        }
+        p.grid = (int32_t) wg;
+        return p;
+    }
+    return taper_one_segment(nb, grid0);
+}
+inline TaperPlan plan_camera_launch(const psdr_scene_s *h, long long n, int waves) {
+    const long long nb = (n + kBlock - 1) / kBlock;
+    const int per_cu = h->opt.blocks_per_cu ? h->opt.blocks_per_cu : camera_blocks_per_cu(h, n);
+    const bool on = h->opt.taper > 0;
+    return plan_camera_taper(nb, on && h->opt.taper_places > 0 ? h->opt.taper_places : h->num_cus * waves, waves, per_cu, on ? h->opt.taper : 0);
+}
 inline int big_launch_per_cu(const psdr_scene_s *h, long long n) { return (int) std::max(16LL, std::min(40LL, n / ((long long) kBlock * h->num_cus * 8))); }
 inline long long launch_chunk(const psdr_scene_s *h, int log2_default) { return 1ll << (h->opt.chunk_log2 > 0 ? h->opt.chunk_log2 : log2_default); }
 inline bool probe_direct(const psdr_scene_s *h, const psdr_render_opts *o, long long n) {
diff --git a/psdr-cuda_amd/psdr_cuda/_abi.py b/psdr-cuda_amd/psdr_cuda/_abi.py
--- a/psdr-cuda_amd/psdr_cuda/_abi.py
+++ b/psdr-cuda_amd/psdr_cuda/_abi.py
@@ -89,7 +89,7 @@
 HIP_SYMBOLS = (
     "psdr_last_error", "psdr_version", "psdr_abi_struct_sizes", "psdr_scene_create", "psdr_scene_destroy", "psdr_scene_set_option", "psdr_scene_set_tables",
     "psdr_bvh_build", "psdr_bvh_stats", "psdr_scene_info", "psdr_trace", "psdr_render_c", "psdr_render_d_fwd", "psdr_render_d_rev",
-    "psdr_guide_build", "psdr_scene_set_point_light", "psdr_scene_set_point_lights", "psdr_scene_set_light", "psdr_scene_set_lights", "psdr_scene_set_path_guide", "psdr_path_guide_build", "psdr_get_counters", "psdr_scene_rev_layout", "psdr_scene_seed_info", "psdr_scene_logd_info",
+    "psdr_guide_build", "psdr_scene_set_point_light", "psdr_scene_set_point_lights", "psdr_scene_set_light", "psdr_scene_set_lights", "psdr_scene_set_path_guide", "psdr_path_guide_build", "psdr_get_counters", "psdr_scene_rev_layout", "psdr_scene_seed_info", "psdr_scene_logd_info", "psdr_scene_taper_info",
     "psdr_geo_world_vertices_fwd", "psdr_geo_world_vertices_rev", "psdr_geo_tri_rows_fwd", "psdr_geo_tri_rows_rev", "psdr_geo_sec_edges_fwd", "psdr_geo_sec_edges_rev", "psdr_geo_prim_edges_fwd", "psdr_geo_prim_edges_rev",
     "psdr_geo_compact_edges_fwd", "psdr_geo_compact_edges_rev", "psdr_geo_emitter_tables",
     "psdr_geo_world_vertices_jvp", "psdr_geo_tri_rows_jvp", "psdr_geo_sec_edges_jvp", "psdr_geo_prim_edges_jvp", "psdr_geo_compact_edges_jvp",
@@ -142,6 +142,7 @@
     lib.psdr_scene_rev_layout.argtypes = [vp, C.POINTER(i32)]
     lib.psdr_scene_seed_info.argtypes = [vp, C.POINTER(C.c_int64)]
     lib.psdr_scene_logd_info.argtypes = [vp, C.POINTER(C.c_int64)]
+    lib.psdr_scene_taper_info.argtypes = [vp, i32, C.POINTER(i32)]
     lib.psdr_geo_world_vertices_fwd.argtypes = [i32, vp, vp, vp, vp, vp]
     lib.psdr_geo_world_vertices_rev.argtypes = [i32, vp, vp, vp, vp, vp, vp, vp]
     lib.psdr_geo_tri_rows_fwd.argtypes = [i32, i32, vp, vp, vp, vp, i32, vp]
@@ -215,7 +216,17 @@
     lib = load_hip()
     out = (C.c_int64 * 4)()
     check(lib, lib.psdr_scene_logd_info(handle, out))
-    return {"launches": int(out[0]), "lean": int(out[1]), "lean_seeded": int(out[2]), "lean_lds_bytes": int(out[3])}
+    return {"launches": int(out[0]), "lean": int(out[1]), "lean_seeded": int(out[2]), "lean_lds_bytes": int(out[3]), "taper_segments": taper_info(handle, 1)["nseg"]}
+
+
+TAPER_SEGS = 8
+
+
+def taper_info(handle, which):
+    lib = load_hip()
+    out = (C.c_int32 * (2 + 5 * TAPER_SEGS))()
+    check(lib, lib.psdr_scene_taper_info(handle, which, out))
+    return {"nseg": int(out[0]), "grid": int(out[1]), "segments": [tuple(int(v) for v in out[2 + 5 * s: 7 + 5 * s]) for s in range(out[0])]}
 
 
 def make_opts(integrator=INTEGRATOR_DIRECT, bsdf_samples=1, light_samples=1, max_depth=1, hide_emitters=False,
```

Result: no change. 21050 Mpath-samples/s (median of 6 runs) (+0.9%).
